# eladb3/SViT

Measured on AMD Instinct MI355X. Metric: clips/sec (fwd+bwd) SViT 16x224^2 bf16, higher is better.
Workload: dtype bf16; 1 GPU; SViT 16x224^2, 8 clips/GPU, 4 object tokens/frame, fwd+CE+bwd+clip+AdamW; global_batch=8, parallelism=dp1, ranks_seen=1, forced_dp=False, launch=hip-graph replay, input=fp32 clips, resident in the replayed step's input buffers, hip_library=svit_amd/lib/libsvit_hip.so

## Files before the change

### include/svit_hip.h

```cpp
#ifndef SVIT_HIP_H
#define SVIT_HIP_H
#include <stdint.h>
#ifdef __cplusplus
extern "C" {
#endif

#define SVIT_HEAD_DIM 96

int svit_version(void);
const char* svit_arch(void);

enum {
  SVIT_EPI_BF16 = 0,
  SVIT_EPI_GELU = 1,
  SVIT_EPI_RESID = 2,
  SVIT_EPI_F32 = 3,
  SVIT_EPI_DGELU = 4,
  SVIT_EPI_RELQ = 5
};
typedef struct {
  const void* A; int32_t lda;
  const void* W; int32_t ldw;
  const float* bias;
  void* out; int32_t ldo;
  void* out2; int32_t ldo2;
  const void* aux; int32_t ldaux;
  const float* row_scale; int32_t rows_per_sample;
  int32_t M, N, K;
  int32_t epilogue; int32_t accumulate;
  int32_t remap_L, remap_N, remap_off;
  const int32_t* relq_map;
  void* relq_out; int32_t relq_ld;
  int32_t relq_extra, relq_rows;
  float relq_scale;
} svit_gemm_args;
int svit_gemm_nt(const svit_gemm_args* args, void* stream);
int svit_gemm_tn(const void* A, int lda, const void* B, int ldb, float* dW, int lddw,
                 int M, int N, int K, int splits, float* dbias ,
                 void* stream);
#define SVIT_TN_GROUP_MAX 16
typedef struct {
  const void* A; const void* B; float* dW; float* dbias;
  int32_t lda, ldb, lddw, M, N, K;
} svit_tn_problem;
int svit_gemm_tn_grouped(const svit_tn_problem* probs, int count, void* stream);
int svit_gemm_tn_grouped_ex(const svit_tn_problem* probs, int count, int ordered, void* stream);
int svit_gemm_tn_grouped_slab(const svit_tn_problem* probs, int count, float* workspace,
                              int64_t workspace_floats, void* stream);
int64_t svit_gemm_tn_grouped_workspace(const svit_tn_problem* probs, int count);
int svit_gemm_tn_grouped_slab_lead(const svit_tn_problem* probs, int count, int launch_count, float* workspace,
                                   int64_t workspace_floats, void* stream);
int svit_colsum_bf16(const void* A, int lda, float* out, int M, int N, void* stream);

int svit_cast_f32_bf16(const float* src, void* dst, int64_t n, void* stream);
int svit_table_interp(const float* M, int rows, int J, const float* tables, float* out32, void* out16, void* stream);
typedef struct svit_table_interp_job {
  const float* M;
  const float* tables;
  float* out32;
  void* out16;
  int32_t rows, J;
} svit_table_interp_job;
int svit_table_interp_batched(const svit_table_interp_job* jobs_dev, int n_jobs, int max_rows, void* stream);
int svit_transpose_cast_batched(const float* src_base, void* dst_base, const int64_t* table,
                                int n_mats, int max_tiles, void* stream);
int svit_transpose_bf16_batched(const void* src_base, void* dst_base, const int64_t* table,
                                int n_mats, int max_tiles, void* stream);
int svit_pad_cast_rows(const float* src, void* dst, int R, int C, int ldd, void* stream);
int svit_scale_cast(const float* src, void* dst, const float* row_scale, int rows_per_sample,
                    int64_t rows, int cols, int gather_L, int gather_N, int gather_off,
                    void* stream);

int svit_reduce_defer(int on, void* stream);
int svit_reduce_flush(void* stream);
int svit_reduce_reset(void* stream);

int svit_layernorm_fwd(const float* x, const float* gamma, const float* beta, void* y_bf16,
                       float* y_f32, float* mean, float* rstd, int64_t rows, int C, float eps,
                       void* stream);
int svit_layernorm_bwd(const void* dy , int dy_is_bf16,
                       const float* x, const float* gamma, const float* mean,
                       const float* rstd, const float* dres, float* dx, void* dx_bf16,
                       const float* row_scale, int rows_per_sample, float* dgamma,
                       float* dbeta, int64_t rows, int C, float* workspace,
                       int64_t workspace_floats, void* stream);

int svit_im2col_patch(const float* video, void* cols, int B, int T, int H, int W, void* stream);
int svit_im2col_patch_u8(const uint8_t* frames, int64_t frames_bytes, const void* lut,
                         const int32_t* crops, void* cols, int B, int T, int Hs, int Ws, int S,
                         void* stream);
int svit_mixup_clips(float* x, const void* mix, int B, int planes, int H, int W, void* stream);
int svit_im2col_patch_u8_mix(const uint8_t* frames, int64_t frames_bytes, const float* lut_f32,
                             const int32_t* crops, const void* mix, void* cols, int B, int T, int Hs,
                             int Ws, int S, void* stream);
int svit_im2col_patch_u8_aug(const uint8_t* frames, int64_t frames_bytes, const float* lut_f32, const void* aug,
                             const void* mix, void* cols, int B, int T, int Hs, int Ws, int S, void* stream);
int svit_im2col_patch_u8_aug_frames(const uint8_t* frames, int64_t frames_bytes, const float* lut_f32, const void* aug,
                                    const void* mix, void* cols, int B, int T, int Hs, int Ws, int S, void* stream);
int svit_u8_clips_render(const uint8_t* frames, int64_t frames_bytes, const float* lut_f32, const void* aug,
                         float* out_f32, int B, int T, int Hs, int Ws, int S, void* stream);
int svit_im2col_patch_u8_aug_ext(const uint8_t* frames, int64_t frames_bytes, const float* lut_f32, const void* aug,
                                 const int32_t* extents, const void* mix, void* cols, int B, int T, int Hs, int Ws, int S,
                                 void* stream);
int svit_im2col_patch_u8_aug_frames_ext(const uint8_t* frames, int64_t frames_bytes, const float* lut_f32, const void* aug,
                                        const int32_t* extents, const void* mix, void* cols, int B, int T, int Hs, int Ws,
                                        int S, void* stream);
int svit_u8_clips_render_ext(const uint8_t* frames, int64_t frames_bytes, const float* lut_f32, const void* aug,
                             const int32_t* extents, float* out_f32, int B, int T, int Hs, int Ws, int S, void* stream);
typedef struct SvitRandAugOp {
  int32_t op, arg_i;
  float arg_f;
  uint32_t bicubic_mask;
  double m[6];
} SvitRandAugOp;
int svit_randaug_stats(const uint8_t* frames, const void* records, int layer, void* workspace, int V, int T, int Hs,
                       int Ws, int N, void* stream);
int svit_randaug_apply(const uint8_t* src, uint8_t* dst, const void* records, int layer, const void* workspace, int V,
                       int T, int Hs, int Ws, int N, void* stream);
int svit_randaug_stats_ext(const uint8_t* frames, const void* records, const int32_t* extents, int layer, void* workspace,
                           int V, int T, int Hs, int Ws, int N, void* stream);
int svit_randaug_apply_ext(const uint8_t* src, uint8_t* dst, const void* records, const int32_t* extents, int layer,
                           const void* workspace, int V, int T, int Hs, int Ws, int N, void* stream);
typedef struct { int64_t src_off; void* dst; int64_t bytes; } svit_feed_seg;
typedef struct {
  const uint8_t* slot; int64_t slot_bytes;
  const int64_t* offsets;
  const int32_t* extents;
  uint8_t* frames;
  int V, T, Hs, Ws, fill, swap_rb, n_seg;
  svit_feed_seg seg[8];
} svit_feed_args;
int svit_feed_unpack(const svit_feed_args* a, void* stream);
int svit_fill_special_tokens(float* x, const float* cls, const float* objq, const float* pos_t,
                             int B, int N, int L, int Tx, int O, int C, int add_pos, void* stream);
int svit_special_token_grads(const float* dx, float* g_cls, float* g_obj, float* g_pos, int B, int N,
                             int L, int Tx, int O, int C, int add_pos, void* stream);

typedef struct {
  const void* qkv; int32_t which;
  const float* conv_w;
  const float* gamma; const float* beta;
  void* out; int32_t ld_out;
  void* pre; float* mean; float* rstd;
  int32_t B, heads, T, H, W, n_obj;
  int32_t stride_hw;
  int32_t mode;
  float eps;
  float out_scale;
  const void* relq_R; const int32_t* relq_map; int32_t relq_lpad; float relq_scale;
} svit_pool_args;
int svit_pool_ln_fwd(const svit_pool_args* a, void* stream);

typedef struct {
  const void* d_main; int32_t main_is_f32; int32_t ld_main;
  const void* d_res; const void* d_extra;
  const void* pre; const float* mean; const float* rstd; const float* gamma;
  void* dpre; float* dgamma; float* dbeta;
  int32_t B, heads, Nout;
  float* workspace; int64_t workspace_floats;
  int32_t main_parts; int64_t main_part_stride;
  int32_t extra_is_bf16;
} svit_pool_ln_bwd_args;
int svit_pool_ln_bwd(const svit_pool_ln_bwd_args* a, void* stream);
typedef struct {
  const void* dpre; const float* conv_w; void* dqkv; int32_t which;
  int32_t B, heads, T, H, W, n_obj, stride_hw;
} svit_pool_dgrad_args;
typedef struct {
  const void* dpre; const void* qkv; int32_t which; float* dw;
  int32_t B, heads, T, H, W, n_obj, stride_hw;
  float* workspace; int64_t workspace_floats;
} svit_pool_wgrad_args;
int svit_pool_ln_fwd_qkv(const svit_pool_args* args3, void* stream);
int svit_pool_weight_sel(const float* src_base, const int64_t* src_off, uint32_t* dst, int n_tables,
                         void* stream);
int svit_pool_ln_fwd_qkv_sel(const svit_pool_args* args3, const uint32_t* const* sel3, void* stream);
int svit_pool_ln_bwd_qkv(const svit_pool_ln_bwd_args* args3, void* stream);
#ifdef SVIT_DIAG_POOL_STREAMING
int svit_pool_conv_dgrad(const svit_pool_dgrad_args* a, void* stream);
int svit_pool_conv_wgrad(const svit_pool_wgrad_args* a, void* stream);
int svit_pool_conv_dgrad_qkv(const svit_pool_dgrad_args* args3, void* stream);
int svit_pool_conv_wgrad_qkv(const svit_pool_wgrad_args* args3, void* stream);
#endif
int svit_pool_conv_bwd_qkv(const svit_pool_dgrad_args* dgrad3, const svit_pool_wgrad_args* wgrad3,
                           void* stream);
int64_t svit_pool_conv_bwd_workspace(const svit_pool_dgrad_args* dgrad3);

typedef struct {
  void* qa; int32_t ld;
  const float* rel_h; const float* rel_w; const float* rel_t;
  const int32_t* idx_h; const int32_t* idx_w; const int32_t* idx_t;
  int32_t B, heads, qt, qh, qw, kt, kh, kw, n_obj;
  float inv_scale;
} svit_relq_args;
int svit_relpos_q_fwd(const svit_relq_args* a, void* stream);
typedef struct {
  const void* qa; const void* dqa; int32_t ld;
  const float* rel_h; const float* rel_w; const float* rel_t;
  const int32_t* idx_h; const int32_t* idx_w; const int32_t* idx_t;
  float* dq_extra;
  float* drel_h; float* drel_w; float* drel_t;
  int32_t rows_h, rows_w, rows_t;
  int32_t B, heads, qt, qh, qw, kt, kh, kw, n_obj;
  float inv_scale;
  float* workspace; int64_t workspace_floats;
} svit_relq_bwd_args;
int svit_relpos_q_bwd(const svit_relq_bwd_args* a, void* stream);
typedef struct {
  const void* P; int32_t ldp; void* qa; int32_t ld;
  const int32_t* idx_h; const int32_t* idx_w; const int32_t* idx_t;
  int32_t row_h, row_w, row_t;
  int32_t B, heads, qt, qh, qw, kt, kh, kw, n_obj;
  float inv_scale;
} svit_relq_gather_args;
int svit_relpos_gather(const svit_relq_gather_args* a, void* stream);
typedef struct {
  const void* dqa; int32_t ld; void* D; int32_t ldd;
  const int32_t* idx_h; const int32_t* idx_w; const int32_t* idx_t;
  int32_t off_h, off_w, off_t;
  int32_t B, heads, qt, qh, qw, kt, kh, kw, n_obj;
  float inv_scale;
} svit_relq_scatter_args;
int svit_relpos_scatter(const svit_relq_scatter_args* a, void* stream);

typedef struct {
  const void* qa; const void* ka; const void* v; void* ctx; float* lse2;
  int32_t B, heads, Nq, Nk, DA; float scale; int32_t bias_cols;
} svit_attn_fwd_args;
int svit_attn_fwd(const svit_attn_fwd_args* a, void* stream);
typedef struct {
  const void* qa; const void* ka; const void* v; const void* ctx; const void* dctx;
  const float* lse2; float* delta;
  void* dqa;
  float* dk; float* dv;
  int32_t B, heads, Nq, Nk, DA, q_splits; float scale;
  int32_t bias_cols;
  void* relD; int32_t relD_ld; const int32_t* relD_map; float relD_scale;
  const void* relR; float* relX;
} svit_attn_bwd_args;
int svit_attn_bwd(const svit_attn_bwd_args* a, void* stream);
int svit_attn_bwd_parts(const svit_attn_bwd_args* a);

int svit_maxpool_fwd(const float* x, float* y, uint8_t* idx, int B, int T, int H, int W,
                     int n_obj, int C, void* stream);
int svit_maxpool_bwd(const float* dy, const uint8_t* idx, float* dx, int B, int T, int H, int W,
                     int n_obj, int C, void* stream);
int svit_maxpool_bwd_bf16(const float* dy, const uint8_t* idx, void* dx_bf16, int B, int T, int H, int W,
                          int n_obj, int C, void* stream);

int svit_sumsq(const float* g, int64_t n, float* sumsq, float* workspace,
               int64_t workspace_floats, void* stream);
int svit_adamw_step(float* p, const float* g, float* m, float* v, int64_t n, const float* sumsq,
                    float max_norm, float lr, float beta1, float beta2, float eps, float wd,
                    int step, float grad_scale, void* stream);

typedef struct {
  float lr[2], weight_decay[2];
  float max_norm, clip_value, grad_scale, reserved;
} svit_step_host;
typedef struct {
  int64_t applied, skipped;
  int32_t consecutive, apply;
  float coef, bc1, bc2_sqrt, sumsq, grad_norm, reserved;
} svit_step_dev;

int svit_tensor_stats_window(void);
int svit_tensor_table_check(const int64_t* table, int64_t Tn, int64_t n);
int64_t svit_tensor_stats_workspace(int64_t n, int64_t Tn);
int svit_tensor_stats(const float* g, const float* p, int64_t n, const int64_t* table_dev, const int64_t* table_host,
                      int64_t Tn, const int64_t* segs, int64_t S, const svit_step_dev* dev_rec, void* ring, int64_t R,
                      int64_t every, void* workspace, int64_t workspace_bytes, void* stream);

#define SVIT_ACT_MAX_SITES 96
#define SVIT_ACT_HEADER_BYTES 48
typedef struct {
  const float* a;
  const float* b;
  int32_t rows, first_window;
} svit_act_site;
int svit_act_stats_window(void);
int64_t svit_act_stats_workspace(int64_t total_windows);
int svit_act_sites_check(const svit_act_site* sites, const int32_t* slots, int64_t n_sites, int64_t n_slots,
                         int64_t* total_windows);
int svit_act_stats(const svit_act_site* sites, const int32_t* slots, int64_t n_sites, int64_t n_slots,
                   const int32_t* geom, const svit_step_dev* dev_rec, void* ring, int64_t R, int64_t* state,
                   void* workspace, int64_t workspace_bytes, void* stream);

int svit_adamw_bias_table(float beta1, float beta2, float* table, int64_t capacity, int64_t* n_entries);

int svit_step_guard(const float* g, int64_t n, const svit_step_host* host_rec, svit_step_dev* dev_rec,
                    const float* bias_table, int64_t table_entries, float* workspace, int64_t workspace_floats,
                    void* stream);
int svit_adamw_step_guarded(float* p, const float* g, float* m, float* v, int64_t n, int64_t n_decay,
                            const svit_step_host* host_rec, const svit_step_dev* dev_rec, float beta1, float beta2,
                            float eps, void* stream);

#define SVIT_MAX_SEGS 64
int svit_step_guard_seg(const float* g, int64_t n, const int64_t* segs, int64_t S, const svit_step_host* host_rec,
                        svit_step_dev* dev_rec, const float* bias_table, int64_t table_entries, float* workspace,
                        int64_t workspace_floats, void* stream);
int svit_adamw_step_guarded_seg(float* p, const float* g, float* m, float* v, int64_t n, int64_t n_decay,
                                const int64_t* segs, int64_t S, const svit_step_host* host_rec,
                                const svit_step_dev* dev_rec, float beta1, float beta2, float eps, void* stream);

int svit_adamw_step_guarded_lr(float* p, const float* g, float* m, float* v, int64_t n, int64_t n_decay,
                               const int64_t* segs, const float* scales, int64_t S, const svit_step_host* host_rec,
                               const svit_step_dev* dev_rec, float beta1, float beta2, float eps, void* stream);

int svit_sgd_step_guarded(float* p, const float* g, float* buf, int64_t n, int64_t n_decay, const int64_t* segs,
                          const float* scales, int64_t S, const svit_step_host* host_rec, const svit_step_dev* dev_rec,
                          float momentum, float dampening, int nesterov, void* stream);
int svit_adam_step_guarded(float* p, const float* g, float* m, float* v, int64_t n, int64_t n_decay,
                           const int64_t* segs, const float* scales, int64_t S, const svit_step_host* host_rec,
                           const svit_step_dev* dev_rec, float beta1, float beta2, float eps, void* stream);

int svit_ema_decay_table(float decay, float* table, int64_t capacity, int64_t* n_entries);
int svit_ema_step_guarded(float* ema, const float* p, int64_t n, const int64_t* segs, int64_t S,
                          const float* decay_table, int64_t table_entries, float decay, const int64_t* ema_rec,
                          const svit_step_dev* dev_rec, void* stream);

typedef struct {
  const float* tokens; int32_t B, N, C, T, O;
  const float* keep;
  const float* w_proj; const float* b_proj; int32_t n_cls;
  const float* w_box; const float* b_box;
  const float* w_bce; const float* b_bce;
  const float* w_con; const float* b_con;
  float* logits; float* boxes; float* contact; float* xobj;
} svit_head_args;
int svit_head_fwd(const svit_head_args* a, void* stream);
typedef struct {
  svit_head_args f;
  const float* dlogits; const float* dboxes; const float* dcontact; const float* dxobj;
  float* dtokens;
  float* gw_proj; float* gb_proj; float* gw_box; float* gb_box; float* gw_bce; float* gb_bce; float* gw_con; float* gb_con;
  int32_t ordered;
} svit_head_bwd_args;
int svit_head_bwd(const svit_head_bwd_args* g, void* stream);
int svit_head_eval(const svit_head_args* a, int act, void* stream);

int svit_haog_loss(const float* pred, const float* tar, const float* contact,
                   const int64_t* contact_tar, float* losses, float* g_l1, float* g_bce,
                   float* g_giou, float* g_contact, int R, int Rc, void* stream);
int svit_haog_loss_bwd(const float* upstream, const float* g_l1, const float* g_bce,
                       const float* g_giou, const float* g_contact, float* dpred,
                       float* dcontact, int R, int Rc, void* stream);

int svit_ce_loss(const float* logits, const int64_t* labels, int B, int C, float* loss, float* dlogits, void* stream);
int svit_ce_loss_soft(const float* logits, const float* target, const int64_t* labels, const void* mix, float on,
                      float off, int B, int C, float* loss, float* dlogits, void* stream);
int svit_step_draws(uint64_t* state, const float* keep, int n_blocks, int per_block, float* scales,
                    int n_drop, float p_drop, float* drop, void* stream);

int svit_ensemble_update(const float* preds, const int64_t* labels, const int64_t* clip_ids,
                         int N, int C, int num_clips, int num_videos, int mode, int repeat,
                         float* video_preds, int64_t* video_labels, int64_t* clip_count,
                         int* err, void* stream);
int svit_topk_correct(const float* video_preds, const int64_t* video_labels, int V, int C,
                      const int* ks, int nk, int* counts, int* err, void* stream);
#define SVIT_METER_MAX_SCALARS 16
int svit_meter_push(float* ring, int W, int K, int64_t* state, const float* const* scalars, int n_scalars,
                    const float* logits, const int64_t* labels, int N, int C, int k0, int k1, void* stream);
int svit_debug_set(int key, int val);
int svit_debug_gemm_nt_plan(int M, int N, int K, int epilogue, int32_t* out, int n_out);
int svit_debug_set_tn(int step_us_x100, int atomic_tbs_x100);
int svit_debug_set_tn_tile(int mode);
int svit_debug_gemm_tn_plan(const svit_tn_problem* probs, int count, int form, int arg, int64_t* out, int n_out);
int svit_debug_set_pool(int key, int val);
int svit_debug_pool_bwd_path(void);
int svit_debug_pool_plan(int kind, int B, int heads, int T, int H, int W, int n_obj, int sq, int sk, int sv, int save_mask,
                         int sel, int relq_lpad, int32_t* out, int n_out);
int svit_attn_debug_set(int key, int val);
int svit_debug_reset(void);
#ifdef __cplusplus
}
#endif
#endif
```

### svit_amd/csrc/common.h

```cpp
#pragma once
#include <hip/hip_runtime.h>
#include <stdint.h>

typedef uint16_t bf16_t;
typedef __bf16 bf16x8_t __attribute__((ext_vector_type(8)));
typedef __bf16 bf16x4_t __attribute__((ext_vector_type(4)));
typedef short s16x4_t __attribute__((ext_vector_type(4)));
typedef short s16x8_t __attribute__((ext_vector_type(8)));
typedef float f32x16_t __attribute__((ext_vector_type(16)));
typedef float f32x4_t __attribute__((ext_vector_type(4)));

#define SVIT_OK 0
#define SVIT_ERR_SHAPE (-2)
#define SVIT_ERR_ALIGN (-3)
#define SVIT_ERR_ARG (-4)

struct SvitOnce {
  unsigned long long mask;
};
static inline int svit_max_lds_once(SvitOnce& once, const void* fn, size_t bytes) {
  int dev = 0;
  if (hipGetDevice(&dev) != hipSuccess) dev = 0;
  const unsigned long long bit = 1ull << (dev & 63);
  if (__atomic_load_n(&once.mask, __ATOMIC_ACQUIRE) & bit) return 0;
  hipError_t e = hipFuncSetAttribute(fn, hipFuncAttributeMaxDynamicSharedMemorySize, (int)bytes);
  if (e != hipSuccess) return (int)e;
  __atomic_fetch_or(&once.mask, bit, __ATOMIC_RELEASE);
  return 0;
}

enum SvitKnob {
  SVIT_K_NT_STAGES = 0,
  SVIT_K_NT_CFG,
  SVIT_K_NT_BK,
  SVIT_K_TN_STEP_US_X100,
  SVIT_K_TN_ATOMIC_TBS_X100,
  SVIT_K_TN_TILE,
  SVIT_K_POOL_FWD,
  SVIT_K_POOL_BWD,
  SVIT_K_POOL_FWD_LARGE,
  SVIT_K_ATTN_DKV_FORM,
  SVIT_K_ATTN_FWD_SHORT,
  SVIT_K_POOL_FRAME,
  SVIT_K_COUNT
};
int svit_knob(int k);
int svit_knob_set(int k, int v);
void svit_knob_reset();

#define SVIT_LAUNCH_CHECK()                       \
  do {                                            \
    hipError_t e__ = hipGetLastError();           \
    if (e__ != hipSuccess) return (int)e__;       \
  } while (0)

__device__ __forceinline__ float bf16_to_f32(bf16_t v) {
  return __uint_as_float(((uint32_t)v) << 16);
}
__device__ __forceinline__ bf16_t f32_to_bf16(float f) {
  __bf16 b = (__bf16)f;
  return __builtin_bit_cast(bf16_t, b);
}
__device__ __forceinline__ uint32_t pack_bf16x2(float lo, float hi) {
  return (uint32_t)f32_to_bf16(lo) | ((uint32_t)f32_to_bf16(hi) << 16);
}
__device__ __forceinline__ float lo_bf16(uint32_t w) { return __uint_as_float(w << 16); }
__device__ __forceinline__ float hi_bf16(uint32_t w) { return __uint_as_float(w & 0xffff0000u); }

__device__ __forceinline__ float wave_sum(float v) {
#pragma unroll
  for (int o = 32; o > 0; o >>= 1) v += __shfl_xor(v, o, 64);
  return v;
}
__device__ __forceinline__ float wave_max(float v) {
#pragma unroll
  for (int o = 32; o > 0; o >>= 1) v = fmaxf(v, __shfl_xor(v, o, 64));
  return v;
}

__device__ __forceinline__ float fast_exp2(float x) { return __builtin_amdgcn_exp2f(x); }

__device__ __forceinline__ f32x16_t mfma32(bf16x8_t a, bf16x8_t b, f32x16_t c) {
  return __builtin_amdgcn_mfma_f32_32x32x16_bf16(a, b, c, 0, 0, 0);
}
__device__ __forceinline__ int acc_row(int r, int lane) {
  return (r & 3) + 8 * (r >> 2) + 4 * (lane >> 5);
}

typedef __attribute__((address_space(3))) s16x4_t lds_s16x4_t;
__device__ __forceinline__ s16x4_t lds_read_tr16(const void* p) {
  return __builtin_amdgcn_ds_read_tr16_b64_v4i16(
      (lds_s16x4_t*)(__attribute__((address_space(3))) void*)p);
}

__device__ __forceinline__ bf16x8_t make_bf16x8(s16x4_t lo, s16x4_t hi) {
  s16x8_t v = {lo[0], lo[1], lo[2], lo[3], hi[0], hi[1], hi[2], hi[3]};
  return __builtin_bit_cast(bf16x8_t, v);
}

__device__ __forceinline__ void gelu_parts(float x, float* cdf, float* pdf_scaled) {
  const float ax = fabsf(x) * 0.70710678118654752f;
  const float e = __expf(-ax * ax);
  const float t = __builtin_amdgcn_rcpf(1.0f + 0.3275911f * ax);
  const float poly = t * (0.254829592f + t * (-0.284496736f + t * (1.421413741f +
                     t * (-1.453152027f + t * 1.061405429f))));
  const float erf_abs = 1.0f - poly * e;
  const float erfv = x < 0.f ? -erf_abs : erf_abs;
  *cdf = 0.5f * (1.0f + erfv);
  *pdf_scaled = 0.39894228040143268f * e;
}
__device__ __forceinline__ float gelu_erf(float x) {
  float cdf, pdf;
  gelu_parts(x, &cdf, &pdf);
  return x * cdf;
}
__device__ __forceinline__ void gelu_fwd_grad(float x, float* y, float* dydx) {
#ifdef SVIT_DIAG_GELU_FREE
  *y = 0.5f * x; *dydx = 0.5f;
  return;
#endif
  float cdf, pdf;
  gelu_parts(x, &cdf, &pdf);
  *y = x * cdf;
  *dydx = cdf + x * pdf;
}
__device__ __forceinline__ float gelu_erf_grad(float x) {
  float cdf, pdf;
  gelu_parts(x, &cdf, &pdf);
  return cdf + x * pdf;
}

__device__ __forceinline__ void philox_round(uint32_t (&c)[4], uint32_t k0, uint32_t k1) {
  const uint64_t p0 = (uint64_t)0xD2511F53u * c[0], p1 = (uint64_t)0xCD9E8D57u * c[2];
  const uint32_t n0 = (uint32_t)(p1 >> 32) ^ c[1] ^ k0, n2 = (uint32_t)(p0 >> 32) ^ c[3] ^ k1;
  c[1] = (uint32_t)p1; c[3] = (uint32_t)p0; c[0] = n0; c[2] = n2;
}
__device__ __forceinline__ void philox4(uint64_t seed, uint64_t draw, uint32_t idx, float (&u)[4]) {
  uint32_t c[4] = {idx, 0u, (uint32_t)draw, (uint32_t)(draw >> 32)};
  uint32_t k0 = (uint32_t)seed, k1 = (uint32_t)(seed >> 32);
#pragma unroll
  for (int r = 0; r < 10; ++r) {
    philox_round(c, k0, k1);
    k0 += 0x9E3779B9u; k1 += 0xBB67AE85u;
  }
#pragma unroll
  for (int i = 0; i < 4; ++i) u[i] = (float)(c[i] >> 8) * (1.0f / 16777216.0f);
}

struct SvitReduceDst {
  float* ptr[6];
  int end[6];
};
void svit_launch_reduce(const float* partial, int nblocks, int n, SvitReduceDst dst, hipStream_t st);

static __global__ void svit_zero_kernel(uint4* __restrict__ p, size_t n16) {
  const size_t stride = (size_t)gridDim.x * blockDim.x;
  for (size_t i = (size_t)blockIdx.x * blockDim.x + threadIdx.x; i < n16; i += stride)
    p[i] = make_uint4(0u, 0u, 0u, 0u);
}
static inline void svit_launch_zero(void* p, size_t bytes, hipStream_t st) {
  const size_t n16 = bytes / 16;
  size_t blocks = (n16 + 255) / 256;
  if (blocks > 2048) blocks = 2048;
  if (blocks == 0) return;
  hipLaunchKernelGGL(svit_zero_kernel, dim3((unsigned)blocks), dim3(256), 0, st, (uint4*)p, n16);
}
```

### svit_amd/csrc/gemm_tn.hip

```cpp
#include <algorithm>
#include <type_traits>
#include <vector>
#include "common.h"
#include "../../include/svit_hip.h"

namespace {

template <int B, int E, typename F>
__device__ __forceinline__ void tn_static_for(F&& f) {
  if constexpr (B < E) {
    f(std::integral_constant<int, B>{});
    tn_static_for<B + 1, E>(f);
  }
}

template <int RB_, int WN_, int WK_, int BM_, int NS_>
struct TnDma {
  static constexpr int RB = RB_, WN = WN_, WK = WK_, BM = BM_, NS = NS_;
  static constexpr int TN = 32 * RB * WN, TK = 96 * WK;
  static constexpr int ROWA = TN * 2, ROWB = TK * 2;
  static constexpr int A_BYTES = BM * ROWA, B_BYTES = BM * ROWB, STAGE = A_BYTES + B_BYTES;
  static constexpr int A_INSTR = A_BYTES / 1024, B_INSTR = B_BYTES / 1024;
  static constexpr int NW = WN * WK, NT = NW * 64;
  static constexpr int PER = (A_INSTR + B_INSTR) / NW;
  static_assert((A_INSTR + B_INSTR) % NW == 0, "every wave issues the same number of pieces");
  __host__ __device__ static constexpr int swz_a(int row) { return row & 3; }
  __host__ __device__ static constexpr int swz_b(int row) { return ROWB == 384 ? ((row >> 1) & 1) : (ROWB % 256 == 0 ? (row & 3) : 0); }
};
using TnSmallD = TnDma<1, 4, 1, 64, 2>;
#ifndef SVIT_TN_BIG_NS
#define SVIT_TN_BIG_NS 3
#endif
#ifndef SVIT_TN_BIG_BM
#define SVIT_TN_BIG_BM 32
#endif
using TnBigD = TnDma<2, 2, 2, SVIT_TN_BIG_BM, SVIT_TN_BIG_NS>;
constexpr int TN_DMA_LDS = 2 * TnSmallD::STAGE > SVIT_TN_BIG_NS * TnBigD::STAGE ? 2 * TnSmallD::STAGE : SVIT_TN_BIG_NS * TnBigD::STAGE;

template <int OFF>
__device__ __forceinline__ void tn_read_tr(s16x4_t& d, unsigned addr) {
  asm volatile("ds_read_b64_tr_b16 %0, %1 offset:%2" : "=&v"(d) : "v"(addr), "i"(OFF) : "memory");
}

template <class C, bool SLAB>
__device__ __forceinline__ void tn_tile_dma(unsigned char* lds, const bf16_t* __restrict__ A, int lda,
                                            const bf16_t* __restrict__ B, int ldb,
                                            float* __restrict__ dW, int lddw, int M, int N, int K, int n0,
                                            int k0, int m_begin, int m_end,
                                            float* __restrict__ dbias, bool bias_tile) {
#if __HIP_DEVICE_COMPILE__
  constexpr int RB = C::RB, BM = C::BM, NS = C::NS, PER = C::PER;
  const int tid = threadIdx.x, lane = tid & 63, wave = __builtin_amdgcn_readfirstlane(tid >> 6);
  const int wn = wave / C::WK, wk = wave % C::WK;
  if (m_begin >= m_end) return;
  constexpr int NW = C::NW, NT = C::NT;
  constexpr int PA = C::A_INSTR / NW;
  static_assert(C::A_INSTR % NW == 0 && C::B_INSTR % NW == 0, "pieces split evenly over the waves");
  unsigned voff[PER];
  const int na8 = (N - n0 + 7) / 8, nb8 = (K - k0 + 7) / 8;
  auto piece = [&](int i, bool a) { return wave + NW * (a ? i : i - PA); };
#pragma unroll
  for (int i = 0; i < PER; ++i) {
    const bool a = i < PA;
    const int o = piece(i, a) * 1024 + lane * 16;
    const int rowb = a ? C::ROWA : C::ROWB;
    const int row = o / rowb, inrow = o % rowb;
    const int pb = inrow >> 6, c16 = (inrow >> 4) & 3;
    const int lb = pb ^ (a ? C::swz_a(row) : C::swz_b(row));
    const int ch = min(lb * 4 + c16, (a ? na8 : nb8) - 1);
    voff[i] = (unsigned)(row * (a ? lda : ldb) + (a ? n0 : k0) + ch * 8) * 2u;
  }
  const auto ars = __builtin_amdgcn_make_buffer_rsrc((void*)A, 0, (int)std::min<size_t>((size_t)M * lda * 2, 0x7fffffffu), 0x00020000);
  const auto brs = __builtin_amdgcn_make_buffer_rsrc((void*)B, 0, (int)std::min<size_t>((size_t)M * ldb * 2, 0x7fffffffu), 0x00020000);
  const int nsteps = (m_end - m_begin + BM - 1) / BM;
  auto issue = [&](int s) {
    unsigned char* st = lds + (s % NS) * C::STAGE;
    const int m0 = m_begin + s * BM;
    const int valid = m_end - m0;
#pragma unroll
    for (int i = 0; i < PER; ++i) {
      const bool a = i < PA;
      unsigned vo = voff[i];
      if (valid < BM) {
        const int row = (piece(i, a) * 1024 + lane * 16) / (a ? C::ROWA : C::ROWB);
        vo -= (unsigned)(row - min(row, valid - 1)) * (a ? lda : ldb) * 2u;
      }
      unsigned char* dst = st + (a ? 0 : C::A_BYTES) + piece(i, a) * 1024;
      if (a)
        __builtin_amdgcn_raw_ptr_buffer_load_lds(ars, (__attribute__((address_space(3))) void*)dst, 16, vo,
                                                 (unsigned)m0 * lda * 2u, 0, 0);
      else
        __builtin_amdgcn_raw_ptr_buffer_load_lds(brs, (__attribute__((address_space(3))) void*)dst, 16, vo,
                                                 (unsigned)m0 * ldb * 2u, 0, 0);
    }
  };
#pragma unroll
  for (int s = 0; s < NS - 1; ++s)
    if (s < nsteps) issue(s);

  f32x16_t acc[RB][3];
#pragma unroll
  for (int i = 0; i < RB; ++i)
#pragma unroll
    for (int j = 0; j < 3; ++j)
#pragma unroll
      for (int r = 0; r < 16; ++r) acc[i][j][r] = 0.f;
  const bool do_bias = (dbias != nullptr) && bias_tile;
  float bsum[8] = {0.f, 0.f, 0.f, 0.f, 0.f, 0.f, 0.f, 0.f};

  const int hh = lane >> 5, cg = (lane >> 4) & 1, ii = lane & 15, q = ii >> 2, pp = ii & 3;
  const unsigned lds0 = (unsigned)(size_t)lds;
  unsigned a_addr[RB], b_addr[3];
#pragma unroll
  for (int i = 0; i < RB; ++i) {
    const int col = wn * 32 * RB + i * 32 + 16 * cg + 4 * pp;
    a_addr[i] = lds0 + (8 * hh + q) * C::ROWA + (((col >> 5) ^ C::swz_a(q)) << 6) + (col & 31) * 2;
  }
#pragma unroll
  for (int j = 0; j < 3; ++j) {
    const int col = wk * 96 + j * 32 + 16 * cg + 4 * pp;
    b_addr[j] = lds0 + C::A_BYTES + (8 * hh + q) * C::ROWB + (((col >> 5) ^ C::swz_b(q)) << 6) + (col & 31) * 2;
  }
  constexpr int KS = BM / 16;
  for (int s = 0; s < nsteps; ++s) {
    if (s + NS - 2 < nsteps - 0 && NS > 2 && s + 1 < nsteps) asm volatile("s_waitcnt vmcnt(%0)" ::"n"((NS - 2) * PER) : "memory");
    else asm volatile("s_waitcnt vmcnt(0)" ::: "memory");
    __builtin_amdgcn_s_barrier();
    if (s + NS - 1 < nsteps) issue(s + NS - 1);
    const unsigned so = (unsigned)((s % NS) * C::STAGE);
    if (m_begin + (s + 1) * BM > m_end) {
      const int valid = m_end - (m_begin + s * BM);
      for (int c = tid; c < (BM - valid) * (C::ROWA / 16); c += NT)
        *(uint4*)(lds + so + valid * C::ROWA + c * 16) = make_uint4(0, 0, 0, 0);
      __syncthreads();
    }
    if (do_bias) {
      constexpr int CPR = C::TN / 8, RP = NT / CPR;
#pragma unroll
      for (int r0 = 0; r0 < BM; r0 += RP) {
        const int row = r0 + tid / CPR, lc = tid % CPR;
        uint4 u;
        asm volatile("ds_read_b128 %0, %1\n\ts_waitcnt lgkmcnt(0)" : "=&v"(u)
                     : "v"(lds0 + so + row * C::ROWA + ((((lc >> 2) ^ C::swz_a(row))) << 6) + (lc & 3) * 16) : "memory");
        bsum[0] += lo_bf16(u.x); bsum[1] += hi_bf16(u.x);
        bsum[2] += lo_bf16(u.y); bsum[3] += hi_bf16(u.y);
        bsum[4] += lo_bf16(u.z); bsum[5] += hi_bf16(u.z);
        bsum[6] += lo_bf16(u.w); bsum[7] += hi_bf16(u.w);
      }
    }
    s16x4_t fl[2][RB + 3], fh[2][RB + 3];
    auto rd = [&](auto KS_, auto BUF_) {
      constexpr int ks = decltype(KS_)::value, buf = decltype(BUF_)::value;
#pragma unroll
      for (int i = 0; i < RB; ++i) {
        tn_read_tr<ks * 16 * C::ROWA>(fl[buf][i], a_addr[i] + so);
        tn_read_tr<(ks * 16 + 4) * C::ROWA>(fh[buf][i], a_addr[i] + so);
      }
#pragma unroll
      for (int j = 0; j < 3; ++j) {
        tn_read_tr<ks * 16 * C::ROWB>(fl[buf][RB + j], b_addr[j] + so);
        tn_read_tr<(ks * 16 + 4) * C::ROWB>(fh[buf][RB + j], b_addr[j] + so);
      }
    };
    rd(std::integral_constant<int, 0>{}, std::integral_constant<int, 0>{});
    tn_static_for<0, KS>([&](auto KS_) {
      constexpr int ks = decltype(KS_)::value, cur = ks & 1;
      if constexpr (ks + 1 < KS) {
        rd(std::integral_constant<int, ks + 1>{}, std::integral_constant<int, (cur ^ 1)>{});
        asm volatile("s_waitcnt lgkmcnt(%0)" ::"n"(2 * (RB + 3)) : "memory");
      } else {
        asm volatile("s_waitcnt lgkmcnt(0)" ::: "memory");
      }
#pragma unroll
      for (int f = 0; f < RB + 3; ++f) asm volatile("" : "+v"(fl[cur][f]), "+v"(fh[cur][f]));
#pragma unroll
      for (int j = 0; j < 3; ++j)
#pragma unroll
        for (int i = 0; i < RB; ++i)
          acc[i][j] = mfma32(make_bf16x8(fl[cur][i], fh[cur][i]), make_bf16x8(fl[cur][RB + j], fh[cur][RB + j]), acc[i][j]);
      __builtin_amdgcn_sched_barrier(0);
    });
  }
  if constexpr (SLAB) {
#pragma unroll
    for (int i = 0; i < RB; ++i)
#pragma unroll
      for (int j = 0; j < 3; ++j) {
        const int tcol = wk * 96 + j * 32 + (lane & 31);
        if (k0 + tcol >= K) continue;
#pragma unroll
        for (int r4 = 0; r4 < 4; ++r4) {
          const int trow = wn * 32 * RB + i * 32 + acc_row(4 * r4, lane);
          if (n0 + trow < N)
            *(float4*)(dW + ((size_t)(trow >> 2) * lddw + tcol) * 4) =
                make_float4(acc[i][j][4 * r4], acc[i][j][4 * r4 + 1], acc[i][j][4 * r4 + 2], acc[i][j][4 * r4 + 3]);
        }
      }
  } else {
#pragma unroll
  for (int i = 0; i < RB; ++i)
#pragma unroll
    for (int j = 0; j < 3; ++j) {
      const int col = k0 + wk * 96 + j * 32 + (lane & 31);
      if (col >= K) continue;
#pragma unroll
      for (int r = 0; r < 16; ++r) {
        const int row = n0 + wn * 32 * RB + i * 32 + acc_row(r, lane);
#ifdef SVIT_TN_FLUSH_PLAIN
        if (row < N) dW[(size_t)row * lddw + col] = acc[i][j][r];
#else
        if (row < N) atomicAdd(dW + (size_t)row * lddw + col, acc[i][j][r]);
#endif
      }
    }
  }
  if (do_bias) {
    constexpr int CPR = C::TN / 8, RP = NT / CPR;
    static_assert(BM % RP == 0, "whole passes over a stage");
    __syncthreads();
    float* red = (float*)lds;
#pragma unroll
    for (int e = 0; e < 8; ++e) red[(tid / CPR) * C::TN + (tid % CPR) * 8 + e] = bsum[e];
    __syncthreads();
    if (tid < C::TN && n0 + tid < N) {
      float sum = 0.f;
#pragma unroll
      for (int g = 0; g < RP; ++g) sum += red[g * C::TN + tid];
      if constexpr (SLAB) dbias[tid] = sum;
      else atomicAdd(dbias + n0 + tid, sum);
    }
  }
#endif
}


__global__ __launch_bounds__(256) void gemm_tn_kernel(const bf16_t* __restrict__ A, int lda,
                                                      const bf16_t* __restrict__ B, int ldb,
                                                      float* __restrict__ dW, int lddw, int M,
                                                      int N, int K, int rows_per_split,
                                                      float* __restrict__ dbias) {
  __shared__ __attribute__((aligned(16))) unsigned char lds[TN_DMA_LDS];
  const int m_begin = blockIdx.z * rows_per_split;
  tn_tile_dma<TnSmallD, false>(lds, A, lda, B, ldb, dW, lddw, M, N, K, blockIdx.x * TnSmallD::TN, blockIdx.y * TnSmallD::TK,
                               m_begin, min(M, m_begin + rows_per_split), dbias, blockIdx.y == 0);
}

struct TnGroup {
  svit_tn_problem p[SVIT_TN_GROUP_MAX];
  int first_block[SVIT_TN_GROUP_MAX + 1];
  int tiles_n[SVIT_TN_GROUP_MAX];
  int tiles[SVIT_TN_GROUP_MAX];
  int rows_per_split[SVIT_TN_GROUP_MAX];
  int big[SVIT_TN_GROUP_MAX];
  int count;
};

struct TnSlabs {
  long long tile_off[SVIT_TN_GROUP_MAX];
  long long bias_off[SVIT_TN_GROUP_MAX];
  int red_first[SVIT_TN_GROUP_MAX + 1];
  int w[SVIT_TN_GROUP_MAX];
};
constexpr int TN_RED_THREADS = 128;
static_assert(TnSmallD::TN == 128 && TnBigD::TN == 128, "slabs and bias partials are 128 rows");

template <bool SLAB>
__device__ __forceinline__ void tn_grouped_workgroup(unsigned char* lds, const TnGroup& g, const TnSlabs* sl, float* ws) {
  const int nwg = gridDim.x, lin = blockIdx.x;
  const int xq = nwg >> 3, xr = nwg & 7, xcd = lin & 7;
  int pi = 0;
  const int bid = (xcd < xr ? xcd * (xq + 1) : xr * (xq + 1) + (xcd - xr) * xq) + (lin >> 3);
#pragma unroll
  for (int i = 1; i < SVIT_TN_GROUP_MAX; ++i)
    if (i < g.count && bid >= g.first_block[i]) pi = i;
  const int local = bid - g.first_block[pi];
  const int tile = local % g.tiles[pi], split = local / g.tiles[pi];
  const svit_tn_problem& p = g.p[pi];
  const int tn = tile % g.tiles_n[pi], tk = tile / g.tiles_n[pi];
  const int m_begin = split * g.rows_per_split[pi];
  float *out, *bias;
  int ld;
  if constexpr (SLAB) {
    ld = sl->w[pi];
    out = ws + sl->tile_off[pi] + (long long)local * (128 * ld);
    bias = p.dbias ? ws + sl->bias_off[pi] + (long long)(split * g.tiles_n[pi] + tn) * 128 : nullptr;
  } else {
    out = p.dW, ld = p.lddw, bias = p.dbias;
  }
  if (g.big[pi])
    tn_tile_dma<TnBigD, SLAB>(lds, (const bf16_t*)p.A, p.lda, (const bf16_t*)p.B, p.ldb, out, ld, p.M, p.N, p.K,
                              tn * TnBigD::TN, tk * TnBigD::TK, m_begin, min(p.M, m_begin + g.rows_per_split[pi]),
                              bias, tk == 0);
  else
    tn_tile_dma<TnSmallD, SLAB>(lds, (const bf16_t*)p.A, p.lda, (const bf16_t*)p.B, p.ldb, out, ld, p.M, p.N, p.K,
                                tn * TnSmallD::TN, tk * TnSmallD::TK, m_begin, min(p.M, m_begin + g.rows_per_split[pi]),
                                bias, tk == 0);
}

#ifndef SVIT_TN_WPE
#define SVIT_TN_WPE 2
#endif
__global__ __launch_bounds__(256, SVIT_TN_WPE) void gemm_tn_grouped_kernel(const TnGroup g) {
  __shared__ __attribute__((aligned(16))) unsigned char lds[TN_DMA_LDS];
  tn_grouped_workgroup<false>(lds, g, nullptr, nullptr);
}

__global__ __launch_bounds__(256, SVIT_TN_WPE) void gemm_tn_grouped_slab_kernel(const TnGroup g, const TnSlabs sl,
                                                                               float* __restrict__ ws) {
  __shared__ __attribute__((aligned(16))) unsigned char lds[TN_DMA_LDS];
  tn_grouped_workgroup<true>(lds, g, &sl, ws);
}

__global__ __launch_bounds__(TN_RED_THREADS) void tn_slab_reduce_kernel(const TnGroup g, const TnSlabs sl,
                                                                        const float* __restrict__ ws) {
#pragma clang fp reassociate(off)
  int pi = 0;
  const int blk = blockIdx.x;
#pragma unroll
  for (int i = 1; i < SVIT_TN_GROUP_MAX; ++i)
    if (i < g.count && blk >= sl.red_first[i]) pi = i;
  const svit_tn_problem& p = g.p[pi];
  const int N = p.N, K = p.K, rg_n = (N + 3) >> 2;
  const int tiles = g.tiles[pi], tiles_n = g.tiles_n[pi];
  const int S = (g.first_block[pi + 1] - g.first_block[pi]) / tiles;
  const long long e = (long long)(blk - sl.red_first[pi]) * TN_RED_THREADS + threadIdx.x;
  const long long nmat = (long long)rg_n * K;
  const float* src;
  long long stride;
  if (e < nmat) {
    const int rg = (int)(e / K), col = (int)(e - (long long)rg * K);
    const int tk_w = g.big[pi] ? TnBigD::TK : TnSmallD::TK, w = sl.w[pi];
    const int tile = (col / tk_w) * tiles_n + rg / 32;
    stride = (long long)tiles * (128 * w);
    src = ws + sl.tile_off[pi] + (long long)tile * (128 * w) + ((long long)(rg % 32) * w + col % tk_w) * 4;
  } else if (p.dbias && e < nmat + rg_n) {
    const int n = (int)(e - nmat) * 4;
    stride = (long long)tiles_n * 128;
    src = ws + sl.bias_off[pi] + (long long)(n / 128) * 128 + n % 128;
  } else {
    return;
  }
  float a0 = 0.f, a1 = 0.f, a2 = 0.f, a3 = 0.f;
  int s = 0;
  for (; s + 8 <= S; s += 8) {
    float4 v[8];
#pragma unroll
    for (int u = 0; u < 8; ++u) v[u] = *(const float4*)(src + (s + u) * stride);
#pragma unroll
    for (int u = 0; u < 8; ++u) { a0 += v[u].x; a1 += v[u].y; a2 += v[u].z; a3 += v[u].w; }
  }
  for (; s < S; ++s) {
    const float4 v = *(const float4*)(src + s * stride);
    a0 += v.x; a1 += v.y; a2 += v.z; a3 += v.w;
  }
  if (e < nmat) {
    const int rg = (int)(e / K), col = (int)(e - (long long)rg * K), row = rg * 4;
    float* d = p.dW + (size_t)row * p.lddw + col;
    d[0] += a0;
    if (row + 1 < N) d[p.lddw] += a1;
    if (row + 2 < N) d[2 * (size_t)p.lddw] += a2;
    if (row + 3 < N) d[3 * (size_t)p.lddw] += a3;
  } else {
    const int n = (int)(e - nmat) * 4;
    float* d = p.dbias + n;
    d[0] += a0;
    if (n + 1 < N) d[1] += a1;
    if (n + 2 < N) d[2] += a2;
    if (n + 3 < N) d[3] += a3;
  }
}

__global__ void colsum_kernel(const bf16_t* __restrict__ A, int lda, float* __restrict__ out,
                              int M, int N, int rows_per_block) {
  const int col = (blockIdx.x * 64 + threadIdx.x) * 2;
  const int r0 = blockIdx.y * rows_per_block;
  const int r1 = min(M, r0 + rows_per_block);
  float s0 = 0.f, s1 = 0.f;
  if (col < N) {
    for (int r = r0 + threadIdx.y; r < r1; r += 4) {
      const uint32_t w = *(const uint32_t*)(A + (size_t)r * lda + col);
      s0 += lo_bf16(w);
      s1 += hi_bf16(w);
    }
  }
  __shared__ float red[4][64][2];
  red[threadIdx.y][threadIdx.x][0] = s0;
  red[threadIdx.y][threadIdx.x][1] = s1;
  __syncthreads();
  if (threadIdx.y == 0 && col < N) {
    for (int k = 1; k < 4; ++k) {
      s0 += red[k][threadIdx.x][0];
      s1 += red[k][threadIdx.x][1];
    }
    atomicAdd(out + col, s0);
    if (col + 1 < N) atomicAdd(out + col + 1, s1);
  }
}

}

struct TnTileDims { int tn, tk, bm; };
static constexpr TnTileDims tn_dims(int big) {
  return big ? TnTileDims{TnBigD::TN, TnBigD::TK, TnBigD::BM} : TnTileDims{TnSmallD::TN, TnSmallD::TK, TnSmallD::BM};
}
static constexpr int tn_ceil(long a, long b) { return (int)((a + b - 1) / b); }

static int tn_check(const svit_tn_problem& p) {
  if (!p.A || !p.B || !p.dW) return SVIT_ERR_ARG;
  if (p.M <= 0 || p.N <= 0 || p.K <= 0) return SVIT_ERR_SHAPE;
  if (p.lda % 8 != 0 || p.ldb % 8 != 0 || p.lda < p.N || p.ldb < p.K || p.lddw < p.K)
    return SVIT_ERR_ALIGN;
  if (((uintptr_t)p.A | (uintptr_t)p.B) & 15) return SVIT_ERR_ALIGN;
  return SVIT_OK;
}
static int tn_check_all(const svit_tn_problem* probs, int count) {
  if (!probs || count <= 0) return SVIT_ERR_ARG;
  for (int i = 0; i < count; ++i) {
    const int rc = tn_check(probs[i]);
    if (rc) return rc;
  }
  return SVIT_OK;
}

struct TnSingle { int tiles_n, tiles_k, splits, rows_per_split; };
static int tn_single_splits(int M, int N, int K) {
  constexpr TnTileDims t = tn_dims(0);
  const int tiles = tn_ceil(N, t.tn) * tn_ceil(K, t.tk);
  const double atom_us = (double)N * K * 4.0 / 0.75e6;
  double best = 1e30;
  int splits = 1;
  static const int cand[] = {1, 2, 3, 4, 6, 8, 12, 16, 24, 32, 48, 64, 96, 128, 192, 256, 384, 512};
  for (int ci = 0; ci < (int)(sizeof(cand) / sizeof(cand[0])); ++ci) {
    const int s = cand[ci];
    const long steps = ((M + s - 1) / s + t.bm - 1) / t.bm;
    if (steps < 2 && s > 1) break;
    const long rounds = ((long)tiles * s + 511) / 512;
    const double time = (double)rounds * steps * 0.85 + s * atom_us;
    if (time < best) { best = time; splits = s; }
  }
  return splits;
}
static TnSingle tn_single_plan(int M, int N, int K, int splits) {
  constexpr TnTileDims t = tn_dims(0);
  if (splits <= 0) splits = tn_single_splits(M, N, K);
  const int rows_per_split = tn_ceil(tn_ceil(M, splits), t.bm) * t.bm;
  return {tn_ceil(N, t.tn), tn_ceil(K, t.tk), tn_ceil(M, rows_per_split), rows_per_split};
}

extern "C" int svit_gemm_tn(const void* A, int lda, const void* B, int ldb, float* dW, int lddw,
                            int M, int N, int K, int splits, float* dbias, void* stream) {
  const svit_tn_problem p = {A, B, dW, dbias, lda, ldb, lddw, M, N, K};
  const int rc = tn_check(p);
  if (rc) return rc;
  const TnSingle s = tn_single_plan(M, N, K, splits);
  hipLaunchKernelGGL(gemm_tn_kernel, dim3(s.tiles_n, s.tiles_k, s.splits), dim3(256), 0, (hipStream_t)stream,
                     (const bf16_t*)A, lda, (const bf16_t*)B, ldb, dW, lddw, M, N, K, s.rows_per_split, dbias);
  SVIT_LAUNCH_CHECK();
  return SVIT_OK;
}


static int tn_tile_rule(const svit_tn_problem& p, int mode) {
  const bool whole = p.K % TnBigD::TK == 0 && p.N >= 128;
  return mode == 1 ? (whole && (p.M <= 4096 || (p.M >= 32768 && p.M < 131072))) : mode == 3 ? whole : (mode == 2);
}

static long tn_chunk_steps(const TnGroup& g, int ordered, double step_us, double atomic_tbs) {
  constexpr long slots = 512;
  long st[SVIT_TN_GROUP_MAX], max_steps = 1;
  for (int i = 0; i < g.count; ++i) {
    st[i] = tn_ceil(g.p[i].M, tn_dims(g.big[i]).bm);
    if (st[i] > max_steps) max_steps = st[i];
  }
  if (ordered) return max_steps;
  double best = 1e30;
  long best_steps = max_steps;
  for (long steps = 2; steps <= max_steps; steps += (steps < 32 ? 1 : steps / 16)) {
    long blocks = 0;
    double flush = 0.0;
    for (int i = 0; i < g.count; ++i) {
      const TnTileDims t = tn_dims(g.big[i]);
      const long nb = (long)g.tiles[i] * ((st[i] + steps - 1) / steps);
      blocks += nb;
      flush += (double)nb * ((double)t.tn * t.tk * 4.0);
    }
    const double time = (double)((blocks + slots - 1) / slots) * steps * step_us + flush / (atomic_tbs * 1e6);
    if (time < best) { best = time; best_steps = steps; }
  }
  return best_steps;
}

static int tn_plan(const svit_tn_problem* probs, int n, int ordered, TnGroup& g) {
  const int mode = svit_knob(SVIT_K_TN_TILE);
  g.count = n;
  for (int i = 0; i < n; ++i) {
    g.p[i] = probs[i];
    g.big[i] = tn_tile_rule(probs[i], mode);
    const TnTileDims t = tn_dims(g.big[i]);
    g.tiles_n[i] = tn_ceil(probs[i].N, t.tn);
    g.tiles[i] = g.tiles_n[i] * tn_ceil(probs[i].K, t.tk);
  }
  const long steps = tn_chunk_steps(g, ordered, svit_knob(SVIT_K_TN_STEP_US_X100) * 0.01,
                                    svit_knob(SVIT_K_TN_ATOMIC_TBS_X100) * 0.01);
  int total = 0;
  for (int i = 0; i < n; ++i) {
    g.rows_per_split[i] = (int)steps * tn_dims(g.big[i]).bm;
    g.first_block[i] = total;
    total += g.tiles[i] * tn_ceil(g.p[i].M, g.rows_per_split[i]);
  }
  for (int i = n; i <= SVIT_TN_GROUP_MAX; ++i) g.first_block[i] = total;
  return total;
}

static int64_t tn_slab_layout(const TnGroup& g, TnSlabs& sl) {
  long long off = 0;
  int red = 0;
  for (int i = 0; i < g.count; ++i) {
    const int tk = tn_dims(g.big[i]).tk, k32 = (g.p[i].K + 31) / 32 * 32;
    sl.w[i] = k32 < tk ? k32 : tk;
    sl.tile_off[i] = off;
    off += (long long)(g.first_block[i + 1] - g.first_block[i]) * (128 * sl.w[i]);
  }
  for (int i = 0; i < g.count; ++i) {
    sl.bias_off[i] = off;
    const int splits = (g.first_block[i + 1] - g.first_block[i]) / g.tiles[i];
    if (g.p[i].dbias) off += (long long)splits * g.tiles_n[i] * 128;
    const long long rg_n = (g.p[i].N + 3) / 4, thr = rg_n * g.p[i].K + (g.p[i].dbias ? rg_n : 0);
    sl.red_first[i] = red;
    red += (int)((thr + TN_RED_THREADS - 1) / TN_RED_THREADS);
  }
  for (int i = g.count; i < SVIT_TN_GROUP_MAX; ++i) sl.tile_off[i] = sl.bias_off[i] = 0, sl.w[i] = 0;
  for (int i = g.count; i <= SVIT_TN_GROUP_MAX; ++i) sl.red_first[i] = red;
  return off;
}

struct TnChunk {
  TnGroup g;
  TnSlabs sl;
  int grid;
  int64_t slab_floats;
};
static int tn_chunks(const svit_tn_problem* probs, int count, int ordered, bool slabs, std::vector<TnChunk>& chunks) {
  const int rc = tn_check_all(probs, count);
  if (rc) return rc;
  chunks.resize((count + SVIT_TN_GROUP_MAX - 1) / SVIT_TN_GROUP_MAX);
  for (size_t c = 0; c < chunks.size(); ++c) {
    const int base = (int)c * SVIT_TN_GROUP_MAX;
    chunks[c].grid = tn_plan(probs + base, std::min(count - base, SVIT_TN_GROUP_MAX), ordered, chunks[c].g);
    chunks[c].slab_floats = slabs ? tn_slab_layout(chunks[c].g, chunks[c].sl) : 0;
  }
  return SVIT_OK;
}
static int64_t tn_slab_need(const std::vector<TnChunk>& chunks) {
  int64_t need = 0;
  for (const TnChunk& c : chunks) need = std::max(need, c.slab_floats);
  return need;
}

extern "C" int svit_gemm_tn_grouped_ex(const svit_tn_problem* probs, int count, int ordered, void* stream) {
  std::vector<TnChunk> chunks;
  const int rc = tn_chunks(probs, count, ordered, false, chunks);
  if (rc) return rc;
  for (const TnChunk& c : chunks) {
    hipLaunchKernelGGL(gemm_tn_grouped_kernel, dim3(c.grid), dim3(256), 0, (hipStream_t)stream, c.g);
    SVIT_LAUNCH_CHECK();
  }
  return SVIT_OK;
}
extern "C" int svit_gemm_tn_grouped(const svit_tn_problem* probs, int count, void* stream) {
  return svit_gemm_tn_grouped_ex(probs, count, 0, stream);
}

extern "C" int64_t svit_gemm_tn_grouped_workspace(const svit_tn_problem* probs, int count) {
  std::vector<TnChunk> chunks;
  const int rc = tn_chunks(probs, count, 0, true, chunks);
  return rc ? rc : tn_slab_need(chunks);
}

extern "C" int svit_gemm_tn_grouped_slab(const svit_tn_problem* probs, int count, float* workspace,
                                         int64_t workspace_floats, void* stream) {
  std::vector<TnChunk> chunks;
  const int rc = tn_chunks(probs, count, 0, true, chunks);
  if (rc) return rc;
  if (!workspace || workspace_floats < tn_slab_need(chunks)) return SVIT_ERR_ARG;
  if ((uintptr_t)workspace & 15) return SVIT_ERR_ALIGN;
  for (const TnChunk& c : chunks) {
    hipLaunchKernelGGL(gemm_tn_grouped_slab_kernel, dim3(c.grid), dim3(256), 0, (hipStream_t)stream, c.g, c.sl, workspace);
    SVIT_LAUNCH_CHECK();
    hipLaunchKernelGGL(tn_slab_reduce_kernel, dim3(c.sl.red_first[SVIT_TN_GROUP_MAX]), dim3(TN_RED_THREADS), 0,
                       (hipStream_t)stream, c.g, c.sl, (const float*)workspace);
    SVIT_LAUNCH_CHECK();
  }
  return SVIT_OK;
}

extern "C" int svit_gemm_tn_grouped_slab_lead(const svit_tn_problem* probs, int count, int launch_count,
                                              float* workspace, int64_t workspace_floats, void* stream) {
  if (launch_count < 1 || launch_count > count) return SVIT_ERR_ARG;
  std::vector<TnChunk> chunks;
  const int rc = tn_chunks(probs, count, 0, true, chunks);
  if (rc) return rc;
  if (!workspace || workspace_floats < tn_slab_need(chunks)) return SVIT_ERR_ARG;
  if ((uintptr_t)workspace & 15) return SVIT_ERR_ALIGN;
  for (size_t i = 0; i < chunks.size(); ++i) {
    const TnChunk& c = chunks[i];
    const int lead = std::min(launch_count - (int)i * SVIT_TN_GROUP_MAX, c.g.count);
    if (lead <= 0) break;
    hipLaunchKernelGGL(gemm_tn_grouped_slab_kernel, dim3(c.g.first_block[lead]), dim3(256), 0, (hipStream_t)stream, c.g,
                       c.sl, workspace);
    SVIT_LAUNCH_CHECK();
    hipLaunchKernelGGL(tn_slab_reduce_kernel, dim3(c.sl.red_first[lead]), dim3(TN_RED_THREADS), 0, (hipStream_t)stream,
                       c.g, c.sl, (const float*)workspace);
    SVIT_LAUNCH_CHECK();
  }
  return SVIT_OK;
}

extern "C" int svit_debug_gemm_tn_plan(const svit_tn_problem* probs, int count, int form, int arg, int64_t* out,
                                       int n_out) {
  if (form < 0 || form > 3 || !out || (form == 3 && count != 1)) return SVIT_ERR_ARG;
  std::vector<TnChunk> chunks;
  const int rc = form == 3 ? tn_check_all(probs, count) : tn_chunks(probs, count, form == 1, form == 2, chunks);
  if (rc) return rc;
  const int groups = form == 3 ? 1 : (int)chunks.size(), n = 2 + 3 * groups + 10 * count;
  if (n_out < n) return SVIT_ERR_ARG;
  int64_t* o = out;
  *o++ = groups;
  *o++ = tn_slab_need(chunks);
  if (form == 3) {
    const TnSingle s = tn_single_plan(probs[0].M, probs[0].N, probs[0].K, arg);
    const int64_t v[13] = {1, (int64_t)s.tiles_n * s.tiles_k * s.splits, 0,
                           0, s.tiles_n, s.tiles_k, s.rows_per_split, s.splits, 0, 0, 0, 0, 0};
    o = std::copy(v, v + 13, o);
  }
  for (const TnChunk& c : chunks) {
    const TnGroup& g = c.g;
    const bool slab = form == 2;
    const int64_t head[3] = {g.count, c.grid, slab ? c.sl.red_first[SVIT_TN_GROUP_MAX] : 0};
    o = std::copy(head, head + 3, o);
    for (int i = 0; i < g.count; ++i) {
      const int64_t v[10] = {g.big[i], g.tiles_n[i], g.tiles[i] / g.tiles_n[i], g.rows_per_split[i],
                             (g.first_block[i + 1] - g.first_block[i]) / g.tiles[i], g.first_block[i],
                             slab ? c.sl.w[i] : 0, slab ? c.sl.tile_off[i] : 0, slab ? c.sl.bias_off[i] : 0,
                             slab ? c.sl.red_first[i] : 0};
      o = std::copy(v, v + 10, o);
    }
  }
  return (int)(o - out);
}

extern "C" int svit_colsum_bf16(const void* A, int lda, float* out, int M, int N, void* stream) {
  if (!A || !out || M <= 0 || N <= 0 || (N & 1) || (lda & 1)) return SVIT_ERR_ARG;
  const int col_groups = (N + 127) / 128;
  int row_chunks = 2048 / col_groups;
  if (row_chunks < 1) row_chunks = 1;
  int rows_per_block = (M + row_chunks - 1) / row_chunks;
  if (rows_per_block < 64) rows_per_block = 64;
  row_chunks = (M + rows_per_block - 1) / rows_per_block;
  hipLaunchKernelGGL(colsum_kernel, dim3(col_groups, row_chunks), dim3(64, 4), 0,
                     (hipStream_t)stream, (const bf16_t*)A, lda, out, M, N, rows_per_block);
  SVIT_LAUNCH_CHECK();
  return SVIT_OK;
}
```

### svit_amd/csrc/misc.hip

```cpp
#include <cstring>
#include <mutex>
#include <unordered_map>
#include "common.h"
#include "../../include/svit_hip.h"

namespace {

__global__ void cast_kernel(const float* __restrict__ src, bf16_t* __restrict__ dst, int64_t n) {
  const int64_t stride = (int64_t)gridDim.x * blockDim.x * 8;
  for (int64_t i = ((int64_t)blockIdx.x * blockDim.x + threadIdx.x) * 8; i < n; i += stride) {
    if (i + 8 <= n) {
      const float4 a = *(const float4*)(src + i), b = *(const float4*)(src + i + 4);
      uint4 o;
      o.x = pack_bf16x2(a.x, a.y); o.y = pack_bf16x2(a.z, a.w);
      o.z = pack_bf16x2(b.x, b.y); o.w = pack_bf16x2(b.z, b.w);
      *(uint4*)(dst + i) = o;
    } else {
      for (int64_t j = i; j < n; ++j) dst[j] = f32_to_bf16(src[j]);
    }
  }
}

__global__ void transpose_cast_kernel(const float* __restrict__ src_base,
                                      bf16_t* __restrict__ dst_base,
// ... 383 lines not shown
}
__global__ void sumsq_final_kernel(const float* __restrict__ partial, int nblocks,
                                   float* __restrict__ out) {
  float s = 0.f;
  for (int i = threadIdx.x; i < nblocks; i += 64) s += partial[i];
  s = wave_sum(s);
  if (threadIdx.x == 0) *out += s;
}

__global__ void adamw_kernel(float* __restrict__ p, const float* __restrict__ g,
                             float* __restrict__ m, float* __restrict__ v, int64_t n,
                             const float* __restrict__ sumsq, float max_norm, float lr, float b1,
                             float b2, float eps, float wd, float bc1, float bc2_sqrt,
                             float grad_scale) {
  float coef = grad_scale;
  if (sumsq && max_norm > 0.f) {
    const float total = sqrtf(*sumsq) * grad_scale;
    coef *= fminf(max_norm / (total + 1e-6f), 1.0f);
  }
  const int64_t stride = (int64_t)gridDim.x * blockDim.x;
  for (int64_t i = (int64_t)blockIdx.x * blockDim.x + threadIdx.x; i < n; i += stride) {
    const float gi = g[i] * coef;
    float w = p[i] * (1.f - lr * wd);
    const float mi = m[i] * b1 + gi * (1.f - b1);
    const float vi = v[i] * b2 + gi * gi * (1.f - b2);
    const float denom = sqrtf(vi) / bc2_sqrt + eps;
    w -= (lr / bc1) * (mi / denom);
    p[i] = w; m[i] = mi; v[i] = vi;
  }
}

__global__ void step_guard_final_kernel(const float* __restrict__ partial, int nblocks,
                                        const svit_step_host* __restrict__ h, svit_step_dev* __restrict__ d,
                                        const float2* __restrict__ table, int64_t entries) {
  float s = 0.f;
  for (int i = threadIdx.x; i < nblocks; i += 64) s += partial[i];
  s = wave_sum(s);
  if (threadIdx.x != 0) return;
  const float max_norm = h->max_norm, grad_scale = h->grad_scale;
  const float total = sqrtf(s) * grad_scale;
  if ((__float_as_uint(total) & 0x7f800000u) != 0x7f800000u) {
    const int64_t step = d->applied + 1;
    float coef = grad_scale;
    if (max_norm > 0.f && !(h->clip_value > 0.f))
      coef *= fminf(max_norm / __builtin_fmaf(sqrtf(s), grad_scale, 1e-6f), 1.0f);
    float2 bc = make_float2(1.f, 1.f);
    if (step >= 1 && step <= entries) bc = table[step - 1];
    d->applied = step;
    d->consecutive = 0;
    d->apply = 1;
    d->coef = coef;
    d->bc1 = bc.x;
    d->bc2_sqrt = bc.y;
    d->sumsq = s;
    d->grad_norm = total;
  } else {
    d->skipped += 1;
    d->consecutive += 1;
    d->apply = 0;
  }
}

template <bool CLAMP>
__device__ __forceinline__ void adamw_guarded_update(float& pw, float gr, float& mo, float& va, float coef, float cv,
                                                     float lr, float wd, float b1, float b2, float eps, float bc1,
                                                     float bc2_sqrt) {
  float gi = gr * coef;
  if (CLAMP) gi = fminf(fmaxf(gi, -cv), cv);
  float w = pw * (1.f - lr * wd);
  const float mi = mo * b1 + gi * (1.f - b1);
  const float vi = va * b2 + gi * gi * (1.f - b2);
  const float denom = sqrtf(vi) / bc2_sqrt + eps;
  w -= (lr / bc1) * (mi / denom);
  pw = w; mo = mi; va = vi;
}

template <bool CLAMP>
__device__ __forceinline__ void adamw_guarded_range(float* __restrict__ p, const float* __restrict__ g,
                                                    float* __restrict__ m, float* __restrict__ v, int64_t n,
                                                    int64_t n_decay, const svit_step_host* __restrict__ h, float coef,
                                                    float bc1, float bc2_sqrt, float b1, float b2, float eps) {
  const float cv = h->clip_value;
  const float lr0 = h->lr[0], lr1 = h->lr[1], wd0 = h->weight_decay[0], wd1 = h->weight_decay[1];
  const int64_t n4 = n >> 2;
  const int64_t stride = (int64_t)gridDim.x * blockDim.x;
  for (int64_t q = (int64_t)blockIdx.x * blockDim.x + threadIdx.x; q < n4; q += stride) {
    const int64_t i = q * 4;
    float4 P = ((const float4*)p)[q], M = ((const float4*)m)[q], V = ((const float4*)v)[q];
    const float4 G = ((const float4*)g)[q];
    const bool d0 = i < n_decay, d1 = i + 1 < n_decay, d2 = i + 2 < n_decay, d3 = i + 3 < n_decay;
    adamw_guarded_update<CLAMP>(P.x, G.x, M.x, V.x, coef, cv, d0 ? lr0 : lr1, d0 ? wd0 : wd1, b1, b2, eps, bc1, bc2_sqrt);
    adamw_guarded_update<CLAMP>(P.y, G.y, M.y, V.y, coef, cv, d1 ? lr0 : lr1, d1 ? wd0 : wd1, b1, b2, eps, bc1, bc2_sqrt);
    adamw_guarded_update<CLAMP>(P.z, G.z, M.z, V.z, coef, cv, d2 ? lr0 : lr1, d2 ? wd0 : wd1, b1, b2, eps, bc1, bc2_sqrt);
    adamw_guarded_update<CLAMP>(P.w, G.w, M.w, V.w, coef, cv, d3 ? lr0 : lr1, d3 ? wd0 : wd1, b1, b2, eps, bc1, bc2_sqrt);
    ((float4*)p)[q] = P; ((float4*)m)[q] = M; ((float4*)v)[q] = V;
  }
  const int64_t i = n4 * 4 + threadIdx.x;
  if (blockIdx.x == 0 && i < n) {
    const bool dec = i < n_decay;
    float pw = p[i], mo = m[i], va = v[i];
    adamw_guarded_update<CLAMP>(pw, g[i], mo, va, coef, cv, dec ? lr0 : lr1, dec ? wd0 : wd1, b1, b2, eps, bc1, bc2_sqrt);
    p[i] = pw; m[i] = mo; v[i] = va;
  }
}

__global__ __launch_bounds__(256) void adamw_guarded_kernel(float* __restrict__ p, const float* __restrict__ g,
                                                            float* __restrict__ m, float* __restrict__ v, int64_t n,
                                                            int64_t n_decay, const svit_step_host* __restrict__ h,
                                                            const svit_step_dev* __restrict__ d, float b1, float b2,
                                                            float eps) {
  if (d->apply == 0) return;
  const float coef = d->coef, bc1 = d->bc1, bc2_sqrt = d->bc2_sqrt;
  if (h->clip_value > 0.f) adamw_guarded_range<true>(p, g, m, v, n, n_decay, h, coef, bc1, bc2_sqrt, b1, b2, eps);
  else adamw_guarded_range<false>(p, g, m, v, n, n_decay, h, coef, bc1, bc2_sqrt, b1, b2, eps);
}

struct SegTable {
  int64_t v[SVIT_MAX_SEGS][2];
  int32_t S;
};
__device__ __forceinline__ bool seg_inside(const SegTable& t, int& k, int64_t lo, int64_t hi, int64_t i) {
  while (k < t.S && t.v[k][1] <= lo) ++k;
  bool in = false;
  for (int j = k; j < t.S && t.v[j][0] < hi; ++j) in |= (i >= t.v[j][0]) & (i < t.v[j][1]);
  return in;
}

__global__ void sumsq_seg_kernel(const float* __restrict__ g, int64_t n, float* __restrict__ partial, const SegTable t) {
  float s = 0.f;
  const int64_t window = (int64_t)blockDim.x * 4, stride = (int64_t)gridDim.x * window;
  int k = 0;
  for (int64_t lo = (int64_t)blockIdx.x * window; lo < n; lo += stride) {
    const int64_t i = lo + (int64_t)threadIdx.x * 4;
    if (seg_inside(t, k, lo, lo + window, i)) {
      const float4 v = *(const float4*)(g + i);
      s += v.x * v.x + v.y * v.y + v.z * v.z + v.w * v.w;
    }
  }
  s = wave_sum(s);
  __shared__ float red[4];
  if ((threadIdx.x & 63) == 0) red[threadIdx.x >> 6] = s;
  __syncthreads();
  if (threadIdx.x == 0) partial[blockIdx.x] = (red[0] + red[1]) + (red[2] + red[3]);
}

template <bool CLAMP>
__device__ __forceinline__ void adamw_guarded_seg_range(float* __restrict__ p, const float* __restrict__ g,
                                                        float* __restrict__ m, float* __restrict__ v, int64_t n,
                                                        int64_t n_decay, const svit_step_host* __restrict__ h,
                                                        float coef, float bc1, float bc2_sqrt, float b1, float b2,
                                                        float eps, const SegTable& t) {
  const float cv = h->clip_value;
  const float lr0 = h->lr[0], lr1 = h->lr[1], wd0 = h->weight_decay[0], wd1 = h->weight_decay[1];
  const int64_t window = (int64_t)blockDim.x * 4, stride = (int64_t)gridDim.x * window;
  int k = 0;
  for (int64_t lo = (int64_t)blockIdx.x * window; lo < n; lo += stride) {
    const int64_t i = lo + (int64_t)threadIdx.x * 4;
    if (!seg_inside(t, k, lo, lo + window, i)) continue;
    const int64_t q = i >> 2;
    float4 P = ((const float4*)p)[q], M = ((const float4*)m)[q], V = ((const float4*)v)[q];
    const float4 G = ((const float4*)g)[q];
    const bool d0 = i < n_decay, d1 = i + 1 < n_decay, d2 = i + 2 < n_decay, d3 = i + 3 < n_decay;
    adamw_guarded_update<CLAMP>(P.x, G.x, M.x, V.x, coef, cv, d0 ? lr0 : lr1, d0 ? wd0 : wd1, b1, b2, eps, bc1, bc2_sqrt);
    adamw_guarded_update<CLAMP>(P.y, G.y, M.y, V.y, coef, cv, d1 ? lr0 : lr1, d1 ? wd0 : wd1, b1, b2, eps, bc1, bc2_sqrt);
    adamw_guarded_update<CLAMP>(P.z, G.z, M.z, V.z, coef, cv, d2 ? lr0 : lr1, d2 ? wd0 : wd1, b1, b2, eps, bc1, bc2_sqrt);
    adamw_guarded_update<CLAMP>(P.w, G.w, M.w, V.w, coef, cv, d3 ? lr0 : lr1, d3 ? wd0 : wd1, b1, b2, eps, bc1, bc2_sqrt);
    ((float4*)p)[q] = P; ((float4*)m)[q] = M; ((float4*)v)[q] = V;
  }
}

__global__ __launch_bounds__(256) void adamw_guarded_seg_kernel(float* __restrict__ p, const float* __restrict__ g,
                                                                float* __restrict__ m, float* __restrict__ v, int64_t n,
                                                                int64_t n_decay, const svit_step_host* __restrict__ h,
                                                                const svit_step_dev* __restrict__ d, float b1, float b2,
                                                                float eps, const SegTable t) {
  if (d->apply == 0) return;
  const float coef = d->coef, bc1 = d->bc1, bc2_sqrt = d->bc2_sqrt;
  if (h->clip_value > 0.f) adamw_guarded_seg_range<true>(p, g, m, v, n, n_decay, h, coef, bc1, bc2_sqrt, b1, b2, eps, t);
  else adamw_guarded_seg_range<false>(p, g, m, v, n, n_decay, h, coef, bc1, bc2_sqrt, b1, b2, eps, t);
}

struct LrTable {
  SegTable t;
  float scale[SVIT_MAX_SEGS];
};
__device__ __forceinline__ float lr_times_scale(float lr, float scale) {
  return __uint_as_float(__builtin_amdgcn_readfirstlane(__float_as_uint(lr * scale)));
}

template <bool CLAMP>
__device__ __forceinline__ void adamw_guarded_lr_range(float* __restrict__ p, const float* __restrict__ g,
                                                       float* __restrict__ m, float* __restrict__ v, int64_t n,
                                                       int64_t n_decay, const svit_step_host* __restrict__ h,
                                                       float coef, float bc1, float bc2_sqrt, float b1, float b2,
                                                       float eps, const LrTable& T) {
  const SegTable& t = T.t;
  const float cv = h->clip_value;
  const float lr0 = h->lr[0], lr1 = h->lr[1], wd0 = h->weight_decay[0], wd1 = h->weight_decay[1];
  const int64_t window = (int64_t)blockDim.x * 4, stride = (int64_t)gridDim.x * window;
  int k = 0;
  for (int64_t lo = (int64_t)blockIdx.x * window; lo < n; lo += stride) {
    const int64_t i = lo + (int64_t)threadIdx.x * 4, hi = lo + window;
    while (k < t.S && t.v[k][1] <= lo) ++k;
    bool in = false;
    float lr = 0.f, wd = 0.f;
    for (int j = k; j < t.S && t.v[j][0] < hi; ++j) {
      const bool dec = t.v[j][0] < n_decay;
      const float le = lr_times_scale(dec ? lr0 : lr1, T.scale[j]);
      const bool here = (i >= t.v[j][0]) & (i < t.v[j][1]);
      in |= here;
      lr = here ? le : lr;
      wd = here ? (dec ? wd0 : wd1) : wd;
    }
    if (!in) continue;
    const int64_t q = i >> 2;
    float4 P = ((const float4*)p)[q], M = ((const float4*)m)[q], V = ((const float4*)v)[q];
    const float4 G = ((const float4*)g)[q];
    adamw_guarded_update<CLAMP>(P.x, G.x, M.x, V.x, coef, cv, lr, wd, b1, b2, eps, bc1, bc2_sqrt);
    adamw_guarded_update<CLAMP>(P.y, G.y, M.y, V.y, coef, cv, lr, wd, b1, b2, eps, bc1, bc2_sqrt);
    adamw_guarded_update<CLAMP>(P.z, G.z, M.z, V.z, coef, cv, lr, wd, b1, b2, eps, bc1, bc2_sqrt);
    adamw_guarded_update<CLAMP>(P.w, G.w, M.w, V.w, coef, cv, lr, wd, b1, b2, eps, bc1, bc2_sqrt);
    ((float4*)p)[q] = P; ((float4*)m)[q] = M; ((float4*)v)[q] = V;
  }
}

__global__ __launch_bounds__(256) void adamw_guarded_lr_kernel(float* __restrict__ p, const float* __restrict__ g,
                                                               float* __restrict__ m, float* __restrict__ v, int64_t n,
                                                               int64_t n_decay, const svit_step_host* __restrict__ h,
                                                               const svit_step_dev* __restrict__ d, float b1, float b2,
                                                               float eps, const LrTable T) {
  if (d->apply == 0) return;
  const float coef = d->coef, bc1 = d->bc1, bc2_sqrt = d->bc2_sqrt;
  if (h->clip_value > 0.f) adamw_guarded_lr_range<true>(p, g, m, v, n, n_decay, h, coef, bc1, bc2_sqrt, b1, b2, eps, T);
  else adamw_guarded_lr_range<false>(p, g, m, v, n, n_decay, h, coef, bc1, bc2_sqrt, b1, b2, eps, T);
}

static int seg_table_take(const int64_t* segs, int64_t S, int64_t n, int64_t n_decay, SegTable* out) {
  if (!segs || S < 1 || S > SVIT_MAX_SEGS) return SVIT_ERR_ARG;
  int64_t prev = 0;
  for (int64_t s = 0; s < S; ++s) {
    const int64_t b = segs[2 * s], e = segs[2 * s + 1];
    if (b < prev || e <= b || e > n) return SVIT_ERR_ARG;
    if (n_decay >= 0 && b < n_decay && e > n_decay) return SVIT_ERR_ARG;
    prev = e;
  }
  for (int64_t s = 0; s < 2 * S; ++s)
    if (segs[s] & 3) return SVIT_ERR_ALIGN;
  for (int64_t s = 0; s < SVIT_MAX_SEGS; ++s) {
    out->v[s][0] = s < S ? segs[2 * s] : 0;
    out->v[s][1] = s < S ? segs[2 * s + 1] : 0;
  }
  out->S = (int32_t)S;
  return SVIT_OK;
}

inline unsigned grid_for(int64_t work_items, int block, unsigned cap = 8192) {
  int64_t b = (work_items + block - 1) / block;
  if (b < 1) b = 1;
  if (b > cap) b = cap;
  return (unsigned)b;
}
__global__ __launch_bounds__(128) void table_interp_kernel(const float* __restrict__ M, int J, const float* __restrict__ T,
                                                           float* __restrict__ out32, bf16_t* __restrict__ out16) {
  const int r = blockIdx.x, c = threadIdx.x;
  if (c >= 96) return;
  const float* m = M + (size_t)r * J;
  float acc = 0.f;
#pragma unroll 8
  for (int j = 0; j < J; ++j) acc += m[j] * T[(size_t)j * 96 + c];
  if (out32) out32[(size_t)r * 96 + c] = acc;
  if (out16) out16[(size_t)r * 96 + c] = f32_to_bf16(acc);
}
__global__ __launch_bounds__(128) void table_interp_batched_kernel(const svit_table_interp_job* __restrict__ jobs) {
  const svit_table_interp_job j = jobs[blockIdx.y];
  const int r = blockIdx.x, c = threadIdx.x;
  if (r >= j.rows || c >= 96) return;
  const float* m = j.M + (size_t)r * j.J;
  float acc = 0.f;
#pragma unroll 8
  for (int k = 0; k < j.J; ++k) acc += m[k] * j.tables[(size_t)k * 96 + c];
  if (j.out32) j.out32[(size_t)r * 96 + c] = acc;
  if (j.out16) ((bf16_t*)j.out16)[(size_t)r * 96 + c] = f32_to_bf16(acc);
}
}

extern "C" int svit_version(void) { return 1; }

extern "C" int svit_table_interp_batched(const svit_table_interp_job* jobs_dev, int n_jobs, int max_rows, void* stream) {
  if (!jobs_dev || n_jobs <= 0 || n_jobs > 65535 || max_rows <= 0) return SVIT_ERR_ARG;
  hipLaunchKernelGGL(table_interp_batched_kernel, dim3(max_rows, n_jobs), dim3(128), 0, (hipStream_t)stream, jobs_dev);
  SVIT_LAUNCH_CHECK();
  return SVIT_OK;
}

extern "C" int svit_table_interp(const float* M, int rows, int J, const float* tables, float* out32, void* out16, void* stream) {
  if (!M || !tables || (!out32 && !out16) || rows <= 0 || J <= 0) return SVIT_ERR_ARG;
  hipLaunchKernelGGL(table_interp_kernel, dim3(rows), dim3(128), 0, (hipStream_t)stream, M, J, tables, out32, (bf16_t*)out16);
  SVIT_LAUNCH_CHECK();
  return SVIT_OK;
}

static const int k_knob_default[SVIT_K_COUNT] = {
     0,  -1,  0,  85,  75,  2,
     2,  1,  1,  0,  1,  2};
static int g_knob[SVIT_K_COUNT] = {0, -1, 0, 85, 75, 2, 2, 1, 1, 0, 1, 2};
int svit_knob(int k) { return __atomic_load_n(&g_knob[k], __ATOMIC_RELAXED); }
int svit_knob_set(int k, int v) {
  if (k < 0 || k >= SVIT_K_COUNT) return SVIT_ERR_ARG;
  __atomic_store_n(&g_knob[k], v, __ATOMIC_RELAXED);
  return SVIT_OK;
}
void svit_knob_reset() {
  for (int k = 0; k < SVIT_K_COUNT; ++k) __atomic_store_n(&g_knob[k], k_knob_default[k], __ATOMIC_RELAXED);
}
extern "C" int svit_debug_set(int key, int val) {
  if (key == 0) return (val == 0 || (val >= 2 && val <= 4)) ? svit_knob_set(SVIT_K_NT_STAGES, val) : SVIT_ERR_ARG;
  if (key == 1) return (val >= -1 && val <= 10) ? svit_knob_set(SVIT_K_NT_CFG, val) : SVIT_ERR_ARG;
  if (key == 2) return (val == 0 || val == 32 || val == 64) ? svit_knob_set(SVIT_K_NT_BK, val) : SVIT_ERR_ARG;
  return SVIT_ERR_ARG;
}
extern "C" int svit_debug_set_tn(int step_us_x100, int atomic_tbs_x100) {
  if (step_us_x100 > 0) svit_knob_set(SVIT_K_TN_STEP_US_X100, step_us_x100);
  if (atomic_tbs_x100 > 0) svit_knob_set(SVIT_K_TN_ATOMIC_TBS_X100, atomic_tbs_x100);
  return SVIT_OK;
}
extern "C" int svit_debug_set_tn_tile(int mode) {
  return (mode >= 0 && mode <= 3) ? svit_knob_set(SVIT_K_TN_TILE, mode) : SVIT_ERR_ARG;
}
extern "C" int svit_debug_set_pool(int key, int val) {
  if (key == 0) return (val >= 0 && val <= 3) ? svit_knob_set(SVIT_K_POOL_FWD, val) : SVIT_ERR_ARG;
  if (key == 1) return (val == 0 || val == 1) ? svit_knob_set(SVIT_K_POOL_BWD, val) : SVIT_ERR_ARG;
  if (key == 2) return (val == 0 || val == 1) ? svit_knob_set(SVIT_K_POOL_FWD_LARGE, val) : SVIT_ERR_ARG;
  if (key == 3) return (val >= 0 && val <= 2) ? svit_knob_set(SVIT_K_POOL_FRAME, val) : SVIT_ERR_ARG;
  return SVIT_ERR_ARG;
}
extern "C" int svit_attn_debug_set(int key, int val) {
  if (key == 0) return (val >= 0 && val <= 2) ? svit_knob_set(SVIT_K_ATTN_DKV_FORM, val) : SVIT_ERR_ARG;
  if (key == 3) return (val == 0 || val == 1) ? svit_knob_set(SVIT_K_ATTN_FWD_SHORT, val) : SVIT_ERR_ARG;
  return SVIT_ERR_ARG;
}
extern "C" int svit_debug_reset(void) { svit_knob_reset(); return SVIT_OK; }
extern "C" const char* svit_arch(void) { return "gfx950"; }

extern "C" int svit_cast_f32_bf16(const float* src, void* dst, int64_t n, void* stream) {
  if (!src || !dst || n <= 0) return SVIT_ERR_ARG;
  if (((uintptr_t)src | (uintptr_t)dst) & 15) return SVIT_ERR_ALIGN;
  hipLaunchKernelGGL(cast_kernel, dim3(grid_for((n + 7) / 8, 256)), dim3(256), 0,
                     (hipStream_t)stream, src, (bf16_t*)dst, n);
  SVIT_LAUNCH_CHECK();
  return SVIT_OK;
}

extern "C" int svit_transpose_cast_batched(const float* src_base, void* dst_base,
                                           const int64_t* table, int n_mats, int max_tiles,
                                           void* stream) {
  if (!src_base || !dst_base || !table || n_mats <= 0) return SVIT_ERR_ARG;
  int gx = max_tiles < 1 ? 1 : (max_tiles > 256 ? 256 : max_tiles);
  hipLaunchKernelGGL(transpose_cast_kernel, dim3(gx, n_mats), dim3(256), 0, (hipStream_t)stream,
                     src_base, (bf16_t*)dst_base, table, n_mats);
  SVIT_LAUNCH_CHECK();
  return SVIT_OK;
}


extern "C" int svit_transpose_bf16_batched(const void* src_base, void* dst_base, const int64_t* table,
                                           int n_mats, int max_tiles, void* stream) {
  if (!src_base || !dst_base || !table || n_mats <= 0) return SVIT_ERR_ARG;
  if (((uintptr_t)src_base | (uintptr_t)dst_base) & 15) return SVIT_ERR_ALIGN;
  int gx = max_tiles < 1 ? 1 : (max_tiles > 256 ? 256 : max_tiles);
  hipLaunchKernelGGL(transpose_bf16_kernel, dim3(gx, n_mats), dim3(256), 0, (hipStream_t)stream,
                     (const bf16_t*)src_base, (bf16_t*)dst_base, table, n_mats);
  SVIT_LAUNCH_CHECK();
  return SVIT_OK;
}

extern "C" int svit_scale_cast(const float* src, void* dst, const float* row_scale,
                               int rows_per_sample, int64_t rows, int cols, int gather_L,
                               int gather_N, int gather_off, void* stream) {
  if (!src || !dst || rows <= 0 || cols <= 0 || cols % 4 != 0) return SVIT_ERR_ARG;
  if (row_scale && rows_per_sample <= 0) return SVIT_ERR_ARG;
  if (gather_L < 0 || (gather_L > 0 && (gather_N < gather_L || gather_off < 0))) return SVIT_ERR_ARG;
  hipLaunchKernelGGL(scale_cast_kernel, dim3(grid_for(rows * (cols / 4), 256)), dim3(256), 0,
                     (hipStream_t)stream, src, (bf16_t*)dst, row_scale, rows_per_sample, rows,
                     cols, gather_L, gather_N, gather_off);
  SVIT_LAUNCH_CHECK();
  return SVIT_OK;
}

extern "C" int svit_pad_cast_rows(const float* src, void* dst, int R, int C, int ldd, void* stream) {
  if (!src || !dst || R <= 0 || C <= 0 || ldd < C) return SVIT_ERR_ARG;
  hipLaunchKernelGGL(pad_cast_rows_kernel, dim3(grid_for((int64_t)R * ldd, 256)), dim3(256), 0,
                     (hipStream_t)stream, src, (bf16_t*)dst, R, C, ldd);
  SVIT_LAUNCH_CHECK();
  return SVIT_OK;
}

extern "C" int svit_im2col_patch(const float* video, void* cols, int B, int T, int H, int W,
                                 void* stream) {
  if (!video || !cols || B <= 0 || T <= 0 || H <= 0 || W <= 0) return SVIT_ERR_ARG;
  const int To = (T + 2 - 3) / 2 + 1, Ho = (H + 6 - 7) / 4 + 1, Wo = (W + 6 - 7) / 4 + 1;
  hipLaunchKernelGGL(im2col_patch_kernel, dim3((unsigned)(B * To * Ho)), dim3(256), 0,
                     (hipStream_t)stream, video, (bf16_t*)cols, B, T, H, W, To, Ho, Wo);
  SVIT_LAUNCH_CHECK();
  return SVIT_OK;
}

extern "C" int svit_fill_special_tokens(float* x, const float* cls, const float* objq,
                                        const float* pos_t, int B, int N, int L, int Tx, int O,
                                        int C, int add_pos, void* stream) {
  if (!x || !cls || !objq || (add_pos && !pos_t)) return SVIT_ERR_ARG;
  if (N != 1 + L + Tx * O) return SVIT_ERR_SHAPE;
  const int64_t total = (int64_t)B * (1 + Tx * O) * C;
  hipLaunchKernelGGL(fill_special_kernel, dim3(grid_for(total, 256)), dim3(256), 0,
                     (hipStream_t)stream, x, cls, objq, pos_t, B, N, L, Tx, O, C, add_pos);
  SVIT_LAUNCH_CHECK();
  return SVIT_OK;
}

extern "C" int svit_special_token_grads(const float* dx, float* g_cls, float* g_obj, float* g_pos, int B, int N,
                                        int L, int Tx, int O, int C, int add_pos, void* stream) {
  if (!dx || !g_cls || !g_obj || (add_pos && !g_pos)) return SVIT_ERR_ARG;
  if (N != 1 + L + Tx * O || B <= 0 || C <= 0) return SVIT_ERR_SHAPE;
  const int n_out = C + O * C + (add_pos ? Tx * C : 0);
  hipLaunchKernelGGL(special_grads_kernel, dim3((n_out * 8 + 255) / 256), dim3(256), 0, (hipStream_t)stream, dx, g_cls,
                     g_obj, g_pos, B, N, L, Tx, O, C, add_pos);
  SVIT_LAUNCH_CHECK();
  return SVIT_OK;
}

extern "C" int svit_maxpool_fwd(const float* x, float* y, uint8_t* idx, int B, int T, int H, int W,
                                int n_obj, int C, void* stream) {
  if (!x || !y || !idx || C % 4 != 0) return SVIT_ERR_ARG;
  const int Ho = (H - 1) / 2 + 1, Wo = (W - 1) / 2 + 1;
  const int64_t per = (int64_t)(1 + T * Ho * Wo + n_obj) * (C / 4);
  if (per >= (1ll << 31) || B > 65535) return SVIT_ERR_SHAPE;
  hipLaunchKernelGGL(maxpool_fwd_kernel, dim3(grid_for(per, 256, 2048), B), dim3(256), 0,
                     (hipStream_t)stream, x, y, idx, B, T, H, W, Ho, Wo, n_obj, C);
  SVIT_LAUNCH_CHECK();
  return SVIT_OK;
}

extern "C" int svit_maxpool_bwd(const float* dy, const uint8_t* idx, float* dx, int B, int T, int H,
                                int W, int n_obj, int C, void* stream) {
  if (!dy || !dx || !idx || C % 4 != 0) return SVIT_ERR_ARG;
  const int Ho = (H - 1) / 2 + 1, Wo = (W - 1) / 2 + 1;
  const int64_t per = (int64_t)(1 + T * H * W + n_obj) * (C / 4);
  if (per >= (1ll << 31) || B > 65535) return SVIT_ERR_SHAPE;
  hipLaunchKernelGGL(maxpool_bwd_kernel<false>, dim3(grid_for(per, 256, 2048), B), dim3(256), 0,
                     (hipStream_t)stream, dy, idx, (void*)dx, B, T, H, W, Ho, Wo, n_obj, C);
  SVIT_LAUNCH_CHECK();
  return SVIT_OK;
}
extern "C" int svit_maxpool_bwd_bf16(const float* dy, const uint8_t* idx, void* dx_bf16, int B, int T, int H,
                                     int W, int n_obj, int C, void* stream) {
  if (!dy || !dx_bf16 || !idx || C % 4 != 0) return SVIT_ERR_ARG;
  const int Ho = (H - 1) / 2 + 1, Wo = (W - 1) / 2 + 1;
  const int64_t per = (int64_t)(1 + T * H * W + n_obj) * (C / 4);
  if (per >= (1ll << 31) || B > 65535) return SVIT_ERR_SHAPE;
  hipLaunchKernelGGL(maxpool_bwd_kernel<true>, dim3(grid_for(per, 256, 2048), B), dim3(256), 0,
                     (hipStream_t)stream, dy, idx, dx_bf16, B, T, H, W, Ho, Wo, n_obj, C);
  SVIT_LAUNCH_CHECK();
  return SVIT_OK;
}

struct ReduceQueue {
  SvitReduceBatch batch;
  bool defer = false;
  ReduceQueue() { batch.count = 0; }
};
static std::mutex g_reduce_mu;
static std::unordered_map<hipStream_t, ReduceQueue> g_reduce_q;

static void reduce_launch(const SvitReduceBatch& b, hipStream_t st) {
  int max_n = 0;
  for (int i = 0; i < b.count; ++i)
    if (b.job[i].n > max_n) max_n = b.job[i].n;
  hipLaunchKernelGGL(svit_reduce_partials_kernel, dim3((max_n + 31) / 32, b.count), dim3(32, 32),
                     0, st, b);
}

void svit_launch_reduce(const float* partial, int nblocks, int n, SvitReduceDst dst, hipStream_t st) {
  SvitReduceJob job = {partial, nblocks, n, dst};
  SvitReduceBatch run;
  run.count = 0;
  {
    std::lock_guard<std::mutex> lk(g_reduce_mu);
    auto it = g_reduce_q.find(st);
    if (it != g_reduce_q.end() && it->second.defer) {
      ReduceQueue& q = it->second;
      if (q.batch.count == SVIT_REDUCE_MAX_JOBS) {
        run = q.batch;
        q.batch.count = 0;
      }
      q.batch.job[q.batch.count++] = job;
      job.partial = nullptr;
    }
  }
  if (run.count) reduce_launch(run, st);
  if (job.partial) {
    SvitReduceBatch one;
    one.job[0] = job;
    one.count = 1;
    reduce_launch(one, st);
  }
}

static void reduce_take(hipStream_t st, int set_defer , bool drop, SvitReduceBatch* out) {
  out->count = 0;
  std::lock_guard<std::mutex> lk(g_reduce_mu);
  auto it = g_reduce_q.find(st);
  if (it == g_reduce_q.end()) {
    if (set_defer != 1) return;
    it = g_reduce_q.emplace(st, ReduceQueue()).first;
  }
  ReduceQueue& q = it->second;
  if (!drop) *out = q.batch;
  q.batch.count = 0;
  if (set_defer >= 0) q.defer = set_defer != 0;
  if (!q.defer) g_reduce_q.erase(it);
}

extern "C" int svit_reduce_defer(int on, void* stream) {
  SvitReduceBatch run;
  reduce_take((hipStream_t)stream, on ? 1 : 0, on != 0, &run);
  if (run.count) reduce_launch(run, (hipStream_t)stream);
  SVIT_LAUNCH_CHECK();
  return SVIT_OK;
}

extern "C" int svit_reduce_flush(void* stream) {
  SvitReduceBatch run;
  reduce_take((hipStream_t)stream, -1, false, &run);
  if (run.count) reduce_launch(run, (hipStream_t)stream);
  SVIT_LAUNCH_CHECK();
  return SVIT_OK;
}

extern "C" int svit_reduce_reset(void* stream) {
  SvitReduceBatch run;
  reduce_take((hipStream_t)stream, 0, true, &run);
  return SVIT_OK;
}

extern "C" int svit_sumsq(const float* g, int64_t n, float* sumsq, float* workspace,
                          int64_t workspace_floats, void* stream) {
  if (!g || !sumsq || !workspace || n <= 0) return SVIT_ERR_ARG;
  unsigned blocks = grid_for((n + 3) / 4, 256, 1024);
  if ((int64_t)blocks > workspace_floats) blocks = (unsigned)workspace_floats;
  if (blocks < 1) return SVIT_ERR_ARG;
  hipLaunchKernelGGL(sumsq_kernel, dim3(blocks), dim3(256), 0, (hipStream_t)stream, g, n, workspace);
  SVIT_LAUNCH_CHECK();
  hipLaunchKernelGGL(sumsq_final_kernel, dim3(1), dim3(64), 0, (hipStream_t)stream, workspace,
                     (int)blocks, sumsq);
  SVIT_LAUNCH_CHECK();
  return SVIT_OK;
}

static inline void adamw_bias_corrections(float beta1, float beta2, int step, float* bc1, float* bc2_sqrt) {
#pragma float_control(precise, on)
  *bc1 = 1.f - powf(beta1, (float)step);
  *bc2_sqrt = sqrtf(1.f - powf(beta2, (float)step));
}

extern "C" int svit_adamw_step(float* p, const float* g, float* m, float* v, int64_t n,
                               const float* sumsq, float max_norm, float lr, float beta1,
                               float beta2, float eps, float wd, int step, float grad_scale,
                               void* stream) {
  if (!p || !g || !m || !v || n <= 0 || step < 1) return SVIT_ERR_ARG;
  float bc1, bc2s;
  adamw_bias_corrections(beta1, beta2, step, &bc1, &bc2s);
  hipLaunchKernelGGL(adamw_kernel, dim3(grid_for(n, 256, 4096)), dim3(256), 0, (hipStream_t)stream,
                     p, g, m, v, n, sumsq, max_norm, lr, beta1, beta2, eps, wd, bc1, bc2s,
                     grad_scale);
  SVIT_LAUNCH_CHECK();
  return SVIT_OK;
}

extern "C" int svit_adamw_bias_table(float beta1, float beta2, float* table, int64_t capacity, int64_t* n_entries) {
  if (!n_entries || (table && capacity < 0)) return SVIT_ERR_ARG;
  constexpr int64_t kMax = 1ll << 20;
  for (int64_t k = 1; k <= kMax; ++k) {
    float bc1, bc2s;
    adamw_bias_corrections(beta1, beta2, (int)k, &bc1, &bc2s);
    if (table) {
      if (k > capacity) return SVIT_ERR_ARG;
      table[2 * (k - 1)] = bc1;
      table[2 * (k - 1) + 1] = bc2s;
    }
    if (bc1 == 1.0f && bc2s == 1.0f) {
      *n_entries = k;
      return SVIT_OK;
    }
  }
  return SVIT_ERR_ARG;
}

extern "C" int svit_step_guard(const float* g, int64_t n, const svit_step_host* host_rec, svit_step_dev* dev_rec,
                               const float* bias_table, int64_t table_entries, float* workspace,
                               int64_t workspace_floats, void* stream) {
  if (!g || !host_rec || !dev_rec || !workspace || n <= 0 || table_entries < 0 || (table_entries > 0 && !bias_table))
    return SVIT_ERR_ARG;
  if (((uintptr_t)host_rec | (uintptr_t)dev_rec | (uintptr_t)bias_table) & 7) return SVIT_ERR_ALIGN;
  unsigned blocks = grid_for((n + 3) / 4, 256, 1024);
  if ((int64_t)blocks > workspace_floats) blocks = (unsigned)workspace_floats;
  if (blocks < 1) return SVIT_ERR_ARG;
  hipLaunchKernelGGL(sumsq_kernel, dim3(blocks), dim3(256), 0, (hipStream_t)stream, g, n, workspace);
  SVIT_LAUNCH_CHECK();
  hipLaunchKernelGGL(step_guard_final_kernel, dim3(1), dim3(64), 0, (hipStream_t)stream, workspace, (int)blocks,
                     host_rec, dev_rec, (const float2*)bias_table, table_entries);
  SVIT_LAUNCH_CHECK();
  return SVIT_OK;
}

extern "C" int svit_adamw_step_guarded(float* p, const float* g, float* m, float* v, int64_t n, int64_t n_decay,
                                       const svit_step_host* host_rec, const svit_step_dev* dev_rec, float beta1,
                                       float beta2, float eps, void* stream) {
  if (!p || !g || !m || !v || !host_rec || !dev_rec || n <= 0 || n_decay < 0 || n_decay > n) return SVIT_ERR_ARG;
  if (((uintptr_t)p | (uintptr_t)g | (uintptr_t)m | (uintptr_t)v) & 15) return SVIT_ERR_ALIGN;
  if (((uintptr_t)host_rec | (uintptr_t)dev_rec) & 7) return SVIT_ERR_ALIGN;
  hipLaunchKernelGGL(adamw_guarded_kernel, dim3(grid_for(n >> 2, 256, 4096)), dim3(256), 0, (hipStream_t)stream,
                     p, g, m, v, n, n_decay, host_rec, dev_rec, beta1, beta2, eps);
  SVIT_LAUNCH_CHECK();
  return SVIT_OK;
}

extern "C" int svit_step_guard_seg(const float* g, int64_t n, const int64_t* segs, int64_t S,
                                   const svit_step_host* host_rec, svit_step_dev* dev_rec, const float* bias_table,
                                   int64_t table_entries, float* workspace, int64_t workspace_floats, void* stream) {
  if (!g || !host_rec || !dev_rec || !workspace || n <= 0 || table_entries < 0 || (table_entries > 0 && !bias_table))
    return SVIT_ERR_ARG;
// ... 54 lines not shown
```

### svit_amd/engine.py

```python
import math

import torch

from . import arch, hip, ops
from .augment import AugClips
from .input import FramesView, U8Clips

HD = arch.HEAD_DIM
F32, BF16 = torch.float32, torch.bfloat16
SCALE = HD ** -0.5
LOG2E = 1.4426950408889634
K_SCALE = SCALE * LOG2E


def _align(n, a=8):
    return (n + a - 1) // a * a


class FlatParams:

    @staticmethod
    def layout(shapes, decay_of, rank_of):
        names = list(shapes)
        depth = 1 + max([int(n.split(".")[1]) for n in names if n.startswith("blocks.")] or [0])
# ... 197 lines not shown
                q_thw = (cur[0], arch.pooled(cur[1], sq), arch.pooled(cur[2], sq))
                k_thw = (cur[0], arch.pooled(cur[1], skv), arch.pooled(cur[2], skv))
                _, _, mcat, _ = self._rel(blk, q_thw, k_thw)
                if mcat is not None:
                    r32 = torch.empty((mcat.shape[0], HD), device=self.dev, dtype=F32) if save else None
                    r16 = torch.empty((mcat.shape[0], HD), device=self.dev, dtype=BF16)
                    entries.append((mcat, self.flat.rel_tables32("blocks.%d." % blk.index), r32, r16))
                    outs[blk.index] = (r32, r16)
                cur = q_thw
            jobs = ops.table_interp_jobs(entries, self.dev) if entries else None
            ent = (jobs, max((e[0].shape[0] for e in entries), default=0), outs, entries)
            self._interp_cache[key] = ent
        jobs, max_rows, outs, _ = ent
        if jobs is not None:
            ops.table_interp_batched(jobs, max_rows)
        self._interp_out = outs

    def _relq_map(self, blk, q_thw, k_thw, idx, rows_off, n_obj, extra):
        key = (blk.index, q_thw, k_thw, tuple(rows_off), n_obj, extra)
        m = self._relq_cache.get(key)
        if m is None:
            qt, qh, qw = q_thw
            kt, kh, kw = k_thw
            ih, iw, it = (t.cpu().view(n, k) for t, n, k in zip(idx, (qh, qw, qt), (kh, kw, kt)))
            Lq = qt * qh * qw
            body = torch.full((qt, qh, qw, extra), -1, dtype=torch.int32)
            body[..., :kh] = (rows_off[0] + ih).view(1, qh, 1, kh)
            body[..., kh:kh + kw] = (rows_off[1] + iw).view(1, 1, qw, kw)
            body[..., kh + kw:kh + kw + kt] = (rows_off[2] + it).view(qt, 1, 1, kt)
            m = torch.full((1 + Lq + n_obj, extra), -1, dtype=torch.int32)
            m[1:1 + Lq] = body.view(Lq, extra)
            m = m.contiguous().to(self.dev)
            self._relq_cache[key] = m
        return m

    def _tables(self, pre, mats):
        names = (pre + "attn.rel_pos_h", pre + "attn.rel_pos_w", pre + "attn.rel_pos_t")
        out = []
        for n, m in zip(names, mats):
            t = self.flat.p(n)
            out.append(t if m is None else (m @ t).contiguous())
        return out

    def forward(self, video, drop_scales=None, save=True, cut=0):
        plan, f = self.plan, self.flat
        if isinstance(video, U8Clips):
            cols, (To, Ho, Wo) = ops.im2col_patch_u8(video)
        elif isinstance(video, AugClips):
            cols, (To, Ho, Wo) = ops.im2col_patch_u8_aug(video)
        elif isinstance(video, FramesView):
            cols, (To, Ho, Wo) = ops.im2col_patch_u8_aug_frames(video)
        else:
            if video.dim() == 4:
                video = video.unsqueeze(2)
            video = video.contiguous().to(F32)
            cols, (To, Ho, Wo) = ops.im2col_patch(video)
        B, _, Tx = video.shape[:3]
        T = plan.num_frames // plan.patch_stride[0] if Tx > 1 else Tx
        if To != T:
            raise hip.SvitHipError("clip has %d frames but cfg.DATA.NUM_FRAMES=%d" % (Tx, plan.num_frames))
        L, n_obj, C = To * Ho * Wo, Tx * plan.objects, plan.embed_dim
        N = 1 + L + n_obj
        x = torch.empty((B, N, C), device=self.dev, dtype=F32)
        ops.gemm_nt(cols, self.patch_w16, f.p("patch_embed.proj.bias"), hip.EPI_F32,
                    out=x.view(B * N, C), remap=(L, N, 1))
        ops.fill_special_tokens(x, f.p("cls_token"), f.p("object_queries"),
                                f.p("pos_embed_temporal"), L, Tx, plan.objects, Tx > 1)
        st = {"B": B, "Tx": Tx, "n_obj": n_obj, "L0": L, "cols": cols if save and cut == 0 else None,
              "blocks": [], "cut": cut}
        thw = (T, Ho, Wo)
        self._interp_tables(thw, save)
        hip.mark("stem")
        for blk in plan.blocks:
            ds = drop_scales[blk.index] if drop_scales is not None else None
            keep = save and 1 + blk.index >= cut
            shapes = (self._tn_shapes(blk, x.shape[0], x.shape[1], thw, n_obj)
                      if save and not keep and self.reproducible and not self.deterministic else None)
            x, thw, sv = self._block_fwd(blk, x, thw, n_obj, ds, keep)
            if shapes is not None:
                sv = {"tn_shapes": shapes}
            st["blocks"].append(sv)
            hip.mark("fwd%d" % blk.index)
        y16, y32, mean, rstd = ops.layernorm_fwd(x, f.p("norm.weight"), f.p("norm.bias"),
                                                 want_f32=True, want_bf16=False, save_stats=save)
        st.update(x_last=x if save else None, mean=mean, rstd=rstd, thw=thw, thw0=(T, Ho, Wo))
        if save and self.act_monitor is not None:
            self.act_monitor.enqueue(st)
        self._interp_out = {}
        return y32, st

    def _tn_shapes(self, blk, B, N, thw, n_obj):
        f = self.flat
        pre = "blocks.%d." % blk.index
        sq, skv = blk.stride_q[1], blk.stride_kv[1]
        q_thw = (thw[0], arch.pooled(thw[1], sq), arch.pooled(thw[2], sq))
        k_thw = (thw[0], arch.pooled(thw[1], skv), arch.pooled(thw[2], skv))
        Nq = 1 + q_thw[0] * q_thw[1] * q_thw[2] + n_obj
        hid, Co = f.slots[pre + "mlp.fc1.weight"][2]
        C = f.slots[pre + "attn.qkv.weight"][2][1]
        M, Mq = B * N, B * Nq
        out = [(Mq, Co, hid, True), (Mq, hid, Co, True), (Mq, Co, Co, True)]
        for a, m in zip("hwt", self._rel(blk, q_thw, k_thw)[1]):
            if m is None:
                out.append((B * blk.heads * Nq, f.slots[pre + "attn.rel_pos_" + a][2][0], HD, False))
        out.append((M, 3 * Co, C, True))
        if blk.has_proj:
            out.append((M, Co, C, True))
        return out

    def _block_fwd(self, blk, x, thw, n_obj, ds, save):
        f = self.flat
        pre = "blocks.%d." % blk.index
        B, N, C = x.shape
        Co, h = blk.dim_out, blk.heads
        sq, skv = blk.stride_q[1], blk.stride_kv[1]
        q_thw = (thw[0], arch.pooled(thw[1], sq), arch.pooled(thw[2], sq))
        k_thw = (thw[0], arch.pooled(thw[1], skv), arch.pooled(thw[2], skv))
        Nq = 1 + q_thw[0] * q_thw[1] * q_thw[2] + n_obj
        J = k_thw[0] + k_thw[1] + k_thw[2]
        DA = HD + 32 if J <= 32 else HD + 64
        if J > 64:
            raise hip.SvitHipError("key grid %s too large for the in-MFMA rel-pos bias" % (k_thw,))
        xn, _, mean1, rstd1 = ops.layernorm_fwd(x, f.p(pre + "norm1.weight"), f.p(pre + "norm1.bias"),
                                                save_stats=save)
        xn2d = xn.view(B * N, C)
        qkv = ops.gemm_nt(xn2d, f.w(pre + "attn.qkv.weight"), f.p(pre + "attn.qkv.bias"), hip.EPI_BF16)
        idx, mats, mcat, need = self._rel(blk, q_thw, k_thw)
        if mcat is None:
            tabs = self._tables(pre, mats)
            rcat, rows_off = f.rel_cat(pre)
        else:
            if blk.index in self._interp_out:
                r32, rcat = self._interp_out[blk.index]
            else:
                r32, rcat = ops.table_interp(mcat, f.rel_tables32(pre), want_f32=save)
            rows_off = (0, need[0], need[0] + need[1])
            tabs = None if r32 is None else [r32[rows_off[0]:rows_off[0] + need[0]], r32[rows_off[1]:rows_off[1] + need[1]],
                                             r32[rows_off[2]:rows_off[2] + need[2]]]
        pools = ops.pool_ln_fwd_qkv(
            qkv, [f.p(pre + "attn.pool_%s.weight" % r).view(HD, 27) for r in "qkv"],
            [f.p(pre + "attn.norm_%s.weight" % r) for r in "qkv"],
            [f.p(pre + "attn.norm_%s.bias" % r) for r in "qkv"],
            B, h, thw, n_obj, (sq, skv, skv), (DA, DA, HD), (0, 1, 0), save=save, out_scales=(1.0, K_SCALE, 1.0),
            sels=f.sels(pre) if (thw[1] * thw[2] >= f.TILED_MIN_PLANE or thw[1] * thw[2] <= f.SLAB_MAX_PLANE)
            else None,
            relq=(rcat.contiguous(), self._relq_map(blk, q_thw, k_thw, idx, rows_off, n_obj, DA - HD), LOG2E))
        qa, ka, v = pools[0][0], pools[1][0], pools[2][0]
        ctx, lse2 = ops.attn_fwd(qa, ka, v, SCALE, bias_cols=J)
        pool_idx = None
        if blk.has_proj:
            skip = ops.gemm_nt(xn2d, f.w(pre + "proj.weight"), f.p(pre + "proj.bias"), hip.EPI_F32)
            skip = skip.view(B, N, Co)
        else:
            skip = x
        if blk.pools_q:
            skip, pool_idx = ops.maxpool_fwd(skip, thw, n_obj)
        dpa, dpm = ds if ds is not None else (None, None)
        x1 = ops.gemm_nt(ctx.view(B * Nq, Co), f.w(pre + "attn.proj.weight"), f.p(pre + "attn.proj.bias"),
                         hip.EPI_RESID, aux=skip.view(B * Nq, Co), row_scale=dpa, rows_per_sample=Nq)
        x1 = x1.view(B, Nq, Co)
        xn2, _, mean2, rstd2 = ops.layernorm_fwd(x1, f.p(pre + "norm2.weight"), f.p(pre + "norm2.bias"),
                                                 save_stats=save)
        act, dact = ops.gemm_nt(xn2.view(B * Nq, Co), f.w(pre + "mlp.fc1.weight"),
                                f.p(pre + "mlp.fc1.bias"), hip.EPI_GELU, save=save)
        x2 = ops.gemm_nt(act, f.w(pre + "mlp.fc2.weight"), f.p(pre + "mlp.fc2.bias"), hip.EPI_RESID,
                         aux=x1.view(B * Nq, Co), row_scale=dpm, rows_per_sample=Nq).view(B, Nq, Co)
        sv = None
        if save:
            sv = dict(x=x, thw=thw, q_thw=q_thw, k_thw=k_thw, mean1=mean1, rstd1=rstd1, xn=xn2d,
                      qkv=qkv, pools=pools, tabs=tabs, idx=idx, mats=mats, ctx=ctx, lse2=lse2,
                      pool_idx=pool_idx, x1=x1, mean2=mean2, rstd2=rstd2, xn2=xn2, act=act,
                      dact=dact, dpa=dpa, dpm=dpm, Nq=Nq)
        return x2, q_thw, sv

    def backward(self, st, dy, on_ready=None, ready_ranks=None):
        def ready(rank):
            if on_ready is not None:
                if ready_ranks is None or rank in ready_ranks:
                    ops.reduce_flush()
                    self._flush_tn()
                    self._join()
                on_ready(rank)
        plan, f = self.plan, self.flat
        depth = len(plan.blocks)
        cut = st.get("cut", 0)
        lo = max(cut - 1, 0)
        if cut > depth:
            if cut == depth + 1:
                ops.layernorm_bwd(dy.contiguous(), st["x_last"], f.p("norm.weight"), st["mean"], st["rstd"],
                                  f.g("norm.weight"), f.g("norm.bias"), want_bf16=False,
                                  rows_per_sample=st["x_last"].shape[1])
            for rank in range(depth + 2):
                ready(rank)
            return
        last = st["blocks"][depth - 1]
        dx, dx16 = ops.layernorm_bwd(dy.contiguous(), st["x_last"], f.p("norm.weight"), st["mean"],
                                     st["rstd"], f.g("norm.weight"), f.g("norm.bias"),
                                     want_bf16=True, row_scale=last["dpm"],
                                     rows_per_sample=st["x_last"].shape[1])
        ready(0)
        hip.mark("bwd_norm")
        for blk in reversed(plan.blocks[lo:]):
            below = st["blocks"][blk.index - 1] if blk.index > lo else None
            try:
                G = self.RED_GROUP
                dx, dx16 = self._block_bwd(blk, st["blocks"][blk.index], dx, dx16, st["n_obj"], below,
                                           red_begin=blk.index % G == G - 1 or blk.index == depth - 1,
                                           red_end=blk.index % G == 0 or blk.index == lo, red_slot=blk.index % G)
            except BaseException:
                ops.reduce_reset()
                self._tn = []
                raise
            hip.mark("bwd%d" % blk.index)
            ready(1 + (depth - 1 - blk.index))
        if cut > 0:
            behind = []
            if self._tn and self.reproducible and not self.deterministic:
                for j in range(lo - 1, -1, -1):
                    behind += st["blocks"][j]["tn_shapes"]
                    if len(self._tn) + len(behind) > 8:
                        break
            self._flush_tn(behind=behind)
            self._join()
            for rank in range(1 + (depth - lo), depth + 2):
                ready(rank)
            return
        B, Tx, L, O, C = st["B"], st["Tx"], st["L0"], plan.objects, plan.embed_dim
        ops.special_token_grads(dx, f.g("cls_token"), f.g("object_queries"),
                                f.g("pos_embed_temporal") if Tx > 1 else None, L, Tx, O, Tx > 1)
        dtok = ops.scale_cast(dx, gather=(L, 1))
        self._gemm_tn(dtok, st["cols"], f.g("patch_embed.proj.weight").view(C, 441), f.g("patch_embed.proj.bias"))
        self._flush_tn()
        self._join()
        ready(depth + 1)

    def _rws(self, key):
        a, b = self._red_regions[key]
        o = self._red_slot * 18 * 1024 * 1024
        return self._red_ws[o + a:o + b]

    def _wgrad_ws(self, B, h, thw, n_obj, strides):
        key = (B, h, tuple(thw), n_obj, tuple(strides))
        need = self._wgrad_need.get(key)
        if need is None:
            need = self._wgrad_need[key] = ops.pool_conv_bwd_workspace(B, h, thw, n_obj, strides)
        ws = self._rws("wgrad")
        if need <= ws.numel():
            return ws
        big = self._wgrad_big.get(self._red_slot)
        if big is None or big.numel() < need:
            big = self._wgrad_big[self._red_slot] = torch.empty(need, device=self.dev, dtype=F32)
        return big

    def _fork(self, fn, keep):
        if not self.overlap_wgrad:
            fn()
            return
        if self._capture_fork is not None:
            self._capture_fork(fn)
            self._side_active = True
            return
        main = torch.cuda.current_stream(self.dev)
        if self._side is None:
            self._side = torch.cuda.Stream(device=self.dev)
        self._side.wait_stream(main)
        with torch.cuda.stream(self._side):
            fn()
        self._side_keep.append(keep)
        self._side_active = True

    def _join(self):
        if self._side_active and self._capture_join is not None:
            self._capture_join()
            self._side_active = False
            return
        if self._side_active:
            torch.cuda.current_stream(self.dev).wait_stream(self._side)
            self._side_keep.clear()
            self._side_active = False

    def _flush_tn(self, force=True, behind=()):
        if not force and len(self._tn) <= 8:
            return
        q, self._tn = self._tn, []
        if not q:
            return
        det = self.deterministic
        if self.reproducible and not det:
            if behind:
                self._fork(lambda: ops.gemm_tn_grouped_slab_lead(q, behind, tag="tn_slab_queue"), q)
            else:
                self._fork(lambda: ops.gemm_tn_grouped_slab(q, tag="tn_slab_queue"), q)
            return
        self._fork(lambda: ops.gemm_tn_grouped(q, ordered=det), q)

    def _gemm_tn(self, a, b, dw, dbias=None):
        if self.deterministic:
            ops.gemm_tn(a, b, dw, splits=1, dbias=dbias)
        elif self.reproducible:
            ops.gemm_tn_grouped_slab([(a, b, dw, dbias)], tag="tn_slab_main")
        else:
            ops.gemm_tn(a, b, dw, splits=0, dbias=dbias)

    def _linear_bwd(self, dy16, x16, wname, bname, need_dx, out=None, accumulate=False,
                    epilogue=hip.EPI_F32, aux=None):
        f = self.flat
        self._tn.append((dy16, x16, f.g(wname), f.g(bname)))
        if not need_dx:
            return None
        return ops.gemm_nt(dy16, f.wt(wname), None, epilogue, out=out, aux=aux, accumulate=accumulate)

    def _block_bwd(self, blk, sv, dx2, dy, n_obj, below, red_begin=True, red_end=True, red_slot=0):
        f = self.flat
        pre = "blocks.%d." % blk.index
        B, Nq, Co = dx2.shape
        x = sv["x"]
        N, C, h = x.shape[1], x.shape[2], blk.heads
        M, Mq = B * N, B * Nq
        sq, skv = blk.stride_q[1], blk.stride_kv[1]
        thw, q_thw, k_thw = sv["thw"], sv["q_thw"], sv["k_thw"]
        self._red_slot = red_slot
        if red_begin:
            ops.reduce_defer(True)
        dy = dy.view(Mq, Co)
        dh = self._linear_bwd(dy, sv["act"], pre + "mlp.fc2.weight", pre + "mlp.fc2.bias", True,
                              epilogue=hip.EPI_DGELU, aux=sv["dact"])
        dxn2 = self._linear_bwd(dh, sv["xn2"].view(Mq, Co), pre + "mlp.fc1.weight",
                                pre + "mlp.fc1.bias", True, epilogue=hip.EPI_BF16)
        dx1, dy = ops.layernorm_bwd(dxn2, sv["x1"], f.p(pre + "norm2.weight"), sv["mean2"],
                                    sv["rstd2"], f.g(pre + "norm2.weight"), f.g(pre + "norm2.bias"),
                                    dres=dx2, want_bf16=True, row_scale=sv["dpa"], rows_per_sample=Nq,
                                    ws=self._rws("ln2"))
        dy = dy.view(Mq, Co)
        dctx = self._linear_bwd(dy, sv["ctx"].view(Mq, Co), pre + "attn.proj.weight",
                                pre + "attn.proj.bias", True, epilogue=hip.EPI_BF16)
        (qa, preq, mq, rq), (ka, prek, mk, rk), (v, prev, mv, rv) = sv["pools"]
        tabs, mats = sv["tabs"], sv["mats"]
        names = (pre + "attn.rel_pos_h", pre + "attn.rel_pos_w", pre + "attn.rel_pos_t")
        if all(m is None for m in mats):
            rcat_t, lpad, offs = f.rel_cat_t(pre)
        else:
            offs, lpad = rel_sections([t.shape[0] for t in tabs])
            rcat = torch.zeros((lpad, HD), device=self.dev, dtype=F32)
            for o, t in zip(offs, tabs):
                rcat[o:o + t.shape[0]] = t
            rcat_t = rcat.t().contiguous().to(BF16)
        if self.fused_scatter:
            dmap = self._relq_map(blk, q_thw, k_thw, sv["idx"], offs, n_obj, qa.shape[-1] - HD)
            dqa, dk, dv, D, dq_extra = ops.attn_bwd(
                qa, ka, v, sv["ctx"], dctx.view(B, Nq, Co), sv["lse2"], SCALE,
                q_splits=1 if self.deterministic else self.attn_q_splits, bias_cols=sum(sv["k_thw"]),
                reld=(dmap, lpad, LOG2E, rcat_t if rcat_t.is_contiguous() else None, "fold"))
        else:
            dqa, dk, dv = ops.attn_bwd(qa, ka, v, sv["ctx"], dctx.view(B, Nq, Co), sv["lse2"], SCALE,
                                       q_splits=1 if self.deterministic else self.attn_q_splits,
                                       bias_cols=sum(sv["k_thw"]))
            D = ops.relpos_scatter(dqa, sv["idx"], offs, lpad, B, h, q_thw, k_thw, n_obj, LOG2E)
            dq_extra = None
        qa2 = qa.view(B * h * Nq, qa.shape[-1])
        for n, m, t, o in zip(names, mats, tabs, offs):
            rows = t.shape[0]
            if m is None:
                self._tn.append((D[:, o:o + rows], qa2[:, :HD], f.g(n), None))
            else:
                d = torch.zeros_like(t)
                self._gemm_tn(D[:, o:o + rows], qa2[:, :HD], d)
                f.g(n).add_(m.t() @ d)
        if dq_extra is None:
            dq_extra = ops.gemm_nt(D, rcat_t, None, hip.EPI_BF16)
        elif isinstance(dq_extra, str):
            dq_extra = None
        Nk = ka.shape[2]
        dqkv = torch.empty_like(sv["qkv"])
        entries = []
        for r, pre_t, mean, rstd, nout, kw in (
                ("q", preq, mq, rq, Nq, dict(d_main=dqa, ld_main=qa.shape[-1], d_res=dctx,
                                             d_extra=dq_extra)),
                ("k", prek, mk, rk, Nk, dict(d_main=dk, ld_main=HD)),
                ("v", prev, mv, rv, Nk, dict(d_main=dv, ld_main=HD))):
            entries.append(((pre_t, mean, rstd, f.p(pre + "attn.norm_%s.weight" % r),
                             f.g(pre + "attn.norm_%s.weight" % r),
                             f.g(pre + "attn.norm_%s.bias" % r), B, h, nout), kw))
        dpres = ops.pool_ln_bwd_qkv(entries, ws=self._rws("pln"))
        strides = (sq, skv, skv)
        ops.pool_conv_bwd_qkv(dpres, [f.p(pre + "attn.pool_%s.weight" % r).view(HD, 27) for r in "qkv"],
                              dqkv, sv["qkv"],
                              [f.g(pre + "attn.pool_%s.weight" % r).view(HD, 27) for r in "qkv"],
                              B, h, thw, n_obj, strides, ws=self._wgrad_ws(B, h, thw, n_obj, strides))
        dxn = self._linear_bwd(dqkv, sv["xn"], pre + "attn.qkv.weight", pre + "attn.qkv.bias", True,
                               epilogue=hip.EPI_F32 if blk.has_proj else hip.EPI_BF16)
        dskip = dx1
        if blk.pools_q:
            dskip = ops.maxpool_bwd(dskip, sv["pool_idx"], thw, n_obj, bf16=blk.has_proj)
        if blk.has_proj:
            ds16 = dskip.view(M, Co) if blk.pools_q else ops.scale_cast(dskip.view(M, Co))
            self._linear_bwd(ds16, sv["xn"], pre + "proj.weight", pre + "proj.bias", True, out=dxn,
                             accumulate=True)
            dskip = None
        res = ops.layernorm_bwd(dxn, x, f.p(pre + "norm1.weight"), sv["mean1"], sv["rstd1"],
                                f.g(pre + "norm1.weight"), f.g(pre + "norm1.bias"), dres=dskip,
                                want_bf16=below is not None,
                                row_scale=below["dpm"] if below is not None else None,
                                rows_per_sample=N, ws=self._rws("ln1"))
        if red_end:
            ops.reduce_defer(False)
        self._flush_tn(force=False)
        if below is None:
            return res.view(B, N, C), None
        return res[0].view(B, N, C), res[1]
```

### svit_amd/hip.py

```python
import ctypes as C
import os

import torch

_HERE = os.path.dirname(os.path.abspath(__file__))
LIB_PATH = os.environ.get("SVIT_HIP_LIB") or os.path.join(_HERE, "lib", "libsvit_hip.so")
_lib = None

vp, i32, i64, f32 = C.c_void_p, C.c_int32, C.c_int64, C.c_float

EPI_BF16, EPI_GELU, EPI_RESID, EPI_F32, EPI_DGELU, EPI_RELQ = 0, 1, 2, 3, 4, 5


class TnProblem(C.Structure):
    _fields_ = [("A", vp), ("B", vp), ("dW", vp), ("dbias", vp), ("lda", i32), ("ldb", i32),
                ("lddw", i32), ("M", i32), ("N", i32), ("K", i32)]


class GemmArgs(C.Structure):
    _fields_ = [("A", vp), ("lda", i32), ("W", vp), ("ldw", i32), ("bias", vp), ("out", vp),
                ("ldo", i32), ("out2", vp), ("ldo2", i32), ("aux", vp), ("ldaux", i32),
                ("row_scale", vp), ("rows_per_sample", i32), ("M", i32), ("N", i32), ("K", i32),
                ("epilogue", i32), ("accumulate", i32), ("remap_L", i32), ("remap_N", i32),
                ("remap_off", i32), ("relq_map", vp), ("relq_out", vp), ("relq_ld", i32),
                ("relq_extra", i32), ("relq_rows", i32), ("relq_scale", f32)]


class PoolArgs(C.Structure):
    _fields_ = [("qkv", vp), ("which", i32), ("conv_w", vp), ("gamma", vp), ("beta", vp),
                ("out", vp), ("ld_out", i32), ("pre", vp), ("mean", vp), ("rstd", vp),
                ("B", i32), ("heads", i32), ("T", i32), ("H", i32), ("W", i32), ("n_obj", i32),
                ("stride_hw", i32), ("mode", i32), ("eps", f32), ("out_scale", f32),
                ("relq_R", vp), ("relq_map", vp), ("relq_lpad", i32), ("relq_scale", f32)]


class PoolLnBwdArgs(C.Structure):
    _fields_ = [("d_main", vp), ("main_is_f32", i32), ("ld_main", i32), ("d_res", vp),
                ("d_extra", vp), ("pre", vp), ("mean", vp), ("rstd", vp), ("gamma", vp),
                ("dpre", vp), ("dgamma", vp), ("dbeta", vp), ("B", i32), ("heads", i32),
                ("Nout", i32), ("workspace", vp), ("workspace_floats", i64), ("main_parts", i32),
                ("main_part_stride", i64), ("extra_is_bf16", i32)]


class PoolDgradArgs(C.Structure):
    _fields_ = [("dpre", vp), ("conv_w", vp), ("dqkv", vp), ("which", i32), ("B", i32),
                ("heads", i32), ("T", i32), ("H", i32), ("W", i32), ("n_obj", i32),
                ("stride_hw", i32)]


class PoolWgradArgs(C.Structure):
    _fields_ = [("dpre", vp), ("qkv", vp), ("which", i32), ("dw", vp), ("B", i32), ("heads", i32),
                ("T", i32), ("H", i32), ("W", i32), ("n_obj", i32), ("stride_hw", i32),
                ("workspace", vp), ("workspace_floats", i64)]


class RelqArgs(C.Structure):
    _fields_ = [("qa", vp), ("ld", i32), ("rel_h", vp), ("rel_w", vp), ("rel_t", vp),
                ("idx_h", vp), ("idx_w", vp), ("idx_t", vp), ("B", i32), ("heads", i32),
                ("qt", i32), ("qh", i32), ("qw", i32), ("kt", i32), ("kh", i32), ("kw", i32),
                ("n_obj", i32), ("inv_scale", f32)]


class RelqBwdArgs(C.Structure):
    _fields_ = [("qa", vp), ("dqa", vp), ("ld", i32), ("rel_h", vp), ("rel_w", vp), ("rel_t", vp),
                ("idx_h", vp), ("idx_w", vp), ("idx_t", vp), ("dq_extra", vp), ("drel_h", vp),
                ("drel_w", vp), ("drel_t", vp), ("rows_h", i32), ("rows_w", i32), ("rows_t", i32),
                ("B", i32), ("heads", i32), ("qt", i32), ("qh", i32), ("qw", i32), ("kt", i32),
                ("kh", i32), ("kw", i32), ("n_obj", i32), ("inv_scale", f32),
                ("workspace", vp), ("workspace_floats", i64)]


class RelqGatherArgs(C.Structure):
    _fields_ = [("P", vp), ("ldp", i32), ("qa", vp), ("ld", i32), ("idx_h", vp), ("idx_w", vp),
                ("idx_t", vp), ("row_h", i32), ("row_w", i32), ("row_t", i32), ("B", i32),
                ("heads", i32), ("qt", i32), ("qh", i32), ("qw", i32), ("kt", i32), ("kh", i32),
                ("kw", i32), ("n_obj", i32), ("inv_scale", f32)]


class RelqScatterArgs(C.Structure):
    _fields_ = [("dqa", vp), ("ld", i32), ("D", vp), ("ldd", i32), ("idx_h", vp), ("idx_w", vp),
                ("idx_t", vp), ("off_h", i32), ("off_w", i32), ("off_t", i32), ("B", i32),
                ("heads", i32), ("qt", i32), ("qh", i32), ("qw", i32), ("kt", i32), ("kh", i32),
                ("kw", i32), ("n_obj", i32), ("inv_scale", f32)]


class AttnFwdArgs(C.Structure):
    _fields_ = [("qa", vp), ("ka", vp), ("v", vp), ("ctx", vp), ("lse2", vp), ("B", i32),
                ("heads", i32), ("Nq", i32), ("Nk", i32), ("DA", i32), ("scale", f32),
                ("bias_cols", i32)]


class AttnBwdArgs(C.Structure):
    _fields_ = [("qa", vp), ("ka", vp), ("v", vp), ("ctx", vp), ("dctx", vp), ("lse2", vp),
                ("delta", vp), ("dqa", vp), ("dk", vp), ("dv", vp), ("B", i32), ("heads", i32),
                ("Nq", i32), ("Nk", i32), ("DA", i32), ("q_splits", i32), ("scale", f32),
                ("bias_cols", i32), ("relD", vp), ("relD_ld", i32), ("relD_map", vp), ("relD_scale", f32),
                ("relR", vp), ("relX", vp)]


class HeadArgs(C.Structure):
    _fields_ = [("tokens", vp), ("B", i32), ("N", i32), ("C", i32), ("T", i32), ("O", i32), ("keep", vp),
                ("w_proj", vp), ("b_proj", vp), ("n_cls", i32), ("w_box", vp), ("b_box", vp),
                ("w_bce", vp), ("b_bce", vp), ("w_con", vp), ("b_con", vp),
                ("logits", vp), ("boxes", vp), ("contact", vp), ("xobj", vp)]


class HeadBwdArgs(C.Structure):
    _fields_ = [("f", HeadArgs), ("dlogits", vp), ("dboxes", vp), ("dcontact", vp), ("dxobj", vp), ("dtokens", vp),
                ("gw_proj", vp), ("gb_proj", vp), ("gw_box", vp), ("gb_box", vp), ("gw_bce", vp), ("gb_bce", vp),
                ("gw_con", vp), ("gb_con", vp), ("ordered", i32)]


class FeedSeg(C.Structure):
    _fields_ = [("src_off", i64), ("dst", vp), ("bytes", i64)]


class FeedArgs(C.Structure):
    _fields_ = [("slot", vp), ("slot_bytes", i64), ("offsets", vp), ("extents", vp), ("frames", vp),
                ("V", i32), ("T", i32), ("Hs", i32), ("Ws", i32), ("fill", i32), ("swap_rb", i32), ("n_seg", i32),
                ("seg", FeedSeg * 8)]


class ActSite(C.Structure):
    _fields_ = [("a", vp), ("b", vp), ("rows", i32), ("first_window", i32)]


class StepHost(C.Structure):
    _fields_ = [("lr", f32 * 2), ("weight_decay", f32 * 2), ("max_norm", f32), ("clip_value", f32),
                ("grad_scale", f32), ("reserved", f32)]


class StepDev(C.Structure):
    _fields_ = [("applied", i64), ("skipped", i64), ("consecutive", i32), ("apply", i32), ("coef", f32),
                ("bc1", f32), ("bc2_sqrt", f32), ("sumsq", f32), ("grad_norm", f32), ("reserved", f32)]


_SIGS = {
    "svit_version": (i32, []),
    "svit_arch": (C.c_char_p, []),
    "svit_gemm_nt": (i32, [C.POINTER(GemmArgs), vp]),
    "svit_gemm_tn": (i32, [vp, i32, vp, i32, vp, i32, i32, i32, i32, i32, vp, vp]),
    "svit_gemm_tn_grouped": (i32, [C.POINTER(TnProblem), i32, vp]),
    "svit_gemm_tn_grouped_ex": (i32, [C.POINTER(TnProblem), i32, i32, vp]),
    "svit_gemm_tn_grouped_slab": (i32, [C.POINTER(TnProblem), i32, vp, i64, vp]),
    "svit_gemm_tn_grouped_workspace": (i64, [C.POINTER(TnProblem), i32]),
    "svit_gemm_tn_grouped_slab_lead": (i32, [C.POINTER(TnProblem), i32, i32, vp, i64, vp]),
    "svit_colsum_bf16": (i32, [vp, i32, vp, i32, i32, vp]),
    "svit_cast_f32_bf16": (i32, [vp, vp, i64, vp]),
    "svit_table_interp": (i32, [vp, i32, i32, vp, vp, vp, vp]),
    "svit_table_interp_batched": (i32, [vp, i32, i32, vp]),
    "svit_transpose_cast_batched": (i32, [vp, vp, vp, i32, i32, vp]),
    "svit_transpose_bf16_batched": (i32, [vp, vp, vp, i32, i32, vp]),
    "svit_scale_cast": (i32, [vp, vp, vp, i32, i64, i32, i32, i32, i32, vp]),
    "svit_pad_cast_rows": (i32, [vp, vp, i32, i32, i32, vp]),
    "svit_reduce_defer": (i32, [i32, vp]),
    "svit_reduce_flush": (i32, [vp]),
    "svit_reduce_reset": (i32, [vp]),
    "svit_layernorm_fwd": (i32, [vp, vp, vp, vp, vp, vp, vp, i64, i32, f32, vp]),
    "svit_layernorm_bwd": (i32, [vp, i32, vp, vp, vp, vp, vp, vp, vp, vp, i32, vp, vp, i64, i32, vp,
                                 i64, vp]),
    "svit_im2col_patch": (i32, [vp, vp, i32, i32, i32, i32, vp]),
    "svit_im2col_patch_u8": (i32, [vp, i64, vp, vp, vp, i32, i32, i32, i32, i32, vp]),
    "svit_im2col_patch_u8_mix": (i32, [vp, i64, vp, vp, vp, vp, i32, i32, i32, i32, i32, vp]),
    "svit_im2col_patch_u8_aug": (i32, [vp, i64, vp, vp, vp, vp, i32, i32, i32, i32, i32, vp]),
    "svit_im2col_patch_u8_aug_frames": (i32, [vp, i64, vp, vp, vp, vp, i32, i32, i32, i32, i32, vp]),
    "svit_u8_clips_render": (i32, [vp, i64, vp, vp, vp, i32, i32, i32, i32, i32, vp]),
    "svit_im2col_patch_u8_aug_ext": (i32, [vp, i64, vp, vp, vp, vp, vp, i32, i32, i32, i32, i32, vp]),
    "svit_im2col_patch_u8_aug_frames_ext": (i32, [vp, i64, vp, vp, vp, vp, vp, i32, i32, i32, i32, i32, vp]),
    "svit_u8_clips_render_ext": (i32, [vp, i64, vp, vp, vp, vp, i32, i32, i32, i32, i32, vp]),
    "svit_mixup_clips": (i32, [vp, vp, i32, i32, i32, i32, vp]),
    "svit_randaug_stats": (i32, [vp, vp, i32, vp, i32, i32, i32, i32, i32, vp]),
    "svit_randaug_apply": (i32, [vp, vp, vp, i32, vp, i32, i32, i32, i32, i32, vp]),
    "svit_randaug_stats_ext": (i32, [vp, vp, vp, i32, vp, i32, i32, i32, i32, i32, vp]),
    "svit_randaug_apply_ext": (i32, [vp, vp, vp, vp, i32, vp, i32, i32, i32, i32, i32, vp]),
    "svit_feed_unpack": (i32, [C.POINTER(FeedArgs), vp]),
    "svit_fill_special_tokens": (i32, [vp, vp, vp, vp, i32, i32, i32, i32, i32, i32, i32, vp]),
    "svit_special_token_grads": (i32, [vp, vp, vp, vp, i32, i32, i32, i32, i32, i32, i32, vp]),
    "svit_pool_ln_fwd": (i32, [C.POINTER(PoolArgs), vp]),
    "svit_pool_ln_bwd": (i32, [C.POINTER(PoolLnBwdArgs), vp]),
    "svit_pool_ln_fwd_qkv": (i32, [C.POINTER(PoolArgs), vp]),
    "svit_pool_ln_fwd_qkv_sel": (i32, [C.POINTER(PoolArgs), C.POINTER(vp), vp]),
    "svit_pool_weight_sel": (i32, [vp, vp, vp, i32, vp]),
    "svit_pool_ln_bwd_qkv": (i32, [C.POINTER(PoolLnBwdArgs), vp]),
    "svit_pool_conv_bwd_qkv": (i32, [C.POINTER(PoolDgradArgs), C.POINTER(PoolWgradArgs), vp]),
    "svit_pool_conv_bwd_workspace": (i64, [C.POINTER(PoolDgradArgs)]),
    "svit_relpos_q_fwd": (i32, [C.POINTER(RelqArgs), vp]),
    "svit_relpos_q_bwd": (i32, [C.POINTER(RelqBwdArgs), vp]),
    "svit_relpos_scatter": (i32, [C.POINTER(RelqScatterArgs), vp]),
    "svit_relpos_gather": (i32, [C.POINTER(RelqGatherArgs), vp]),
    "svit_attn_fwd": (i32, [C.POINTER(AttnFwdArgs), vp]),
    "svit_attn_bwd": (i32, [C.POINTER(AttnBwdArgs), vp]),
    "svit_attn_bwd_parts": (i32, [C.POINTER(AttnBwdArgs)]),
    "svit_maxpool_fwd": (i32, [vp, vp, vp, i32, i32, i32, i32, i32, i32, vp]),
    "svit_maxpool_bwd": (i32, [vp, vp, vp, i32, i32, i32, i32, i32, i32, vp]),
    "svit_maxpool_bwd_bf16": (i32, [vp, vp, vp, i32, i32, i32, i32, i32, i32, vp]),
    "svit_sumsq": (i32, [vp, i64, vp, vp, i64, vp]),
    "svit_adamw_step": (i32, [vp, vp, vp, vp, i64, vp, f32, f32, f32, f32, f32, f32, i32, f32, vp]),
    "svit_adamw_bias_table": (i32, [f32, f32, vp, i64, C.POINTER(i64)]),
    "svit_step_guard": (i32, [vp, i64, vp, vp, vp, i64, vp, i64, vp]),
    "svit_adamw_step_guarded": (i32, [vp, vp, vp, vp, i64, i64, vp, vp, f32, f32, f32, vp]),
    "svit_step_guard_seg": (i32, [vp, i64, vp, i64, vp, vp, vp, i64, vp, i64, vp]),
    "svit_adamw_step_guarded_seg": (i32, [vp, vp, vp, vp, i64, i64, vp, i64, vp, vp, f32, f32, f32, vp]),
    "svit_adamw_step_guarded_lr": (i32, [vp, vp, vp, vp, i64, i64, vp, vp, i64, vp, vp, f32, f32, f32, vp]),
    "svit_sgd_step_guarded": (i32, [vp, vp, vp, i64, i64, vp, vp, i64, vp, vp, f32, f32, i32, vp]),
    "svit_adam_step_guarded": (i32, [vp, vp, vp, vp, i64, i64, vp, vp, i64, vp, vp, f32, f32, f32, vp]),
    "svit_ema_decay_table": (i32, [f32, vp, i64, C.POINTER(i64)]),
    "svit_ema_step_guarded": (i32, [vp, vp, i64, vp, i64, vp, i64, f32, vp, vp, vp]),
    "svit_tensor_stats_window": (i32, []),
    "svit_tensor_table_check": (i32, [vp, i64, i64]),
    "svit_tensor_stats_workspace": (i64, [i64, i64]),
    "svit_tensor_stats": (i32, [vp, vp, i64, vp, vp, i64, vp, i64, vp, vp, i64, i64, vp, i64, vp]),
    "svit_act_stats_window": (i32, []),
    "svit_act_stats_workspace": (i64, [i64]),
    "svit_act_sites_check": (i32, [C.POINTER(ActSite), vp, i64, i64, C.POINTER(i64)]),
    "svit_act_stats": (i32, [C.POINTER(ActSite), vp, i64, i64, vp, vp, vp, i64, vp, vp, i64, vp]),
    "svit_head_fwd": (i32, [C.POINTER(HeadArgs), vp]),
    "svit_head_bwd": (i32, [C.POINTER(HeadBwdArgs), vp]),
    "svit_head_eval": (i32, [C.POINTER(HeadArgs), i32, vp]),
    "svit_haog_loss": (i32, [vp, vp, vp, vp, vp, vp, vp, vp, vp, i32, i32, vp]),
    "svit_haog_loss_bwd": (i32, [vp, vp, vp, vp, vp, vp, vp, i32, i32, vp]),
    "svit_ce_loss": (i32, [vp, vp, i32, i32, vp, vp, vp]),
    "svit_ce_loss_soft": (i32, [vp, vp, vp, vp, f32, f32, i32, i32, vp, vp, vp]),
    "svit_step_draws": (i32, [vp, vp, i32, i32, vp, i32, C.c_float, vp, vp]),
    "svit_ensemble_update": (i32, [vp, vp, vp, i32, i32, i32, i32, i32, i32, vp, vp, vp, vp, vp]),
    "svit_topk_correct": (i32, [vp, vp, i32, i32, vp, i32, vp, vp, vp]),
    "svit_meter_push": (i32, [vp, i32, i32, vp, vp, i32, vp, vp, i32, i32, i32, i32, vp]),
    "svit_debug_set": (i32, [i32, i32]),
    "svit_debug_set_tn": (i32, [i32, i32]),
    "svit_debug_set_tn_tile": (i32, [i32]),
    "svit_debug_set_pool": (i32, [i32, i32]),
    "svit_attn_debug_set": (i32, [i32, i32]),
    "svit_debug_reset": (i32, []),
    "svit_debug_pool_bwd_path": (i32, []),
    "svit_debug_pool_plan": (i32, [i32] * 13 + [C.POINTER(C.c_int32), i32]),
    "svit_debug_gemm_nt_plan": (i32, [i32] * 4 + [C.POINTER(C.c_int32), i32]),
    "svit_debug_gemm_tn_plan": (i32, [C.POINTER(TnProblem), i32, i32, i32, C.POINTER(i64), i32]),
}
EXPORTS = tuple(sorted(_SIGS))


class SvitHipError(RuntimeError):
    pass


def load():
    global _lib
    if _lib is None:
        if not os.path.exists(LIB_PATH):
            raise SvitHipError(
                "libsvit_hip.so not found at %s -- run `python -m svit_amd.build` "
                "(the SViT HIP path has no PyTorch/CPU fallback)" % LIB_PATH)
        if os.environ.get("SVIT_HIP_LIB"):
            import warnings
            warnings.warn("SVIT_HIP_LIB is set: loading the SViT HIP library from %s instead of the "
                          "in-tree build" % LIB_PATH)
        lib = C.CDLL(LIB_PATH)
        for name, (res, args) in _SIGS.items():
            fn = getattr(lib, name)
            fn.restype, fn.argtypes = res, args
        _lib = lib
    return _lib


_raw_stream = torch._C._cuda_getCurrentRawStream
_cur_device = torch._C._cuda_getDevice


def stream():
    return C.c_void_p(_raw_stream(_cur_device()))


def ptr(t):
    if t is None:
        return None
    return t.data_ptr()


def check(rc, what):
    if rc != 0:
        kind = {-2: "bad shape", -3: "bad alignment/stride", -4: "bad argument"}.get(
            rc, "hipError_t %d" % rc)
        raise SvitHipError("%s failed: %s" % (what, kind))


_trace = None


def start_trace():
    global _trace
    _trace = []


def stop_trace():
    global _trace
    t, _trace = _trace, None
    return t


def mark(label):
    if _trace is not None:
        e = torch.cuda.Event(enable_timing=True)
        e.record()
        _trace.append(("mark:" + label, e, e, None))


def call(name, *args, meta=None):
    if _trace is None:
        rc = getattr(load(), name)(*args, stream())
        check(rc, name)
        return
    e0 = torch.cuda.Event(enable_timing=True)
    e1 = torch.cuda.Event(enable_timing=True)
    e0.record()
    rc = getattr(load(), name)(*args, stream())
    e1.record()
    check(rc, name)
    _trace.append((name, e0, e1, meta))
```

### svit_amd/ops.py

```python
import ctypes as C

import torch

from . import hip
from .hip import ptr

BF16 = torch.bfloat16
F32 = torch.float32
HD = 96
_scratch = {}


def scratch(device, floats=8 * 1024 * 1024, tag="main"):
    key = (device.index, floats, tag)
    buf = _scratch.get(key)
    if buf is None:
        buf = torch.empty(floats, device=device, dtype=F32)
        _scratch[key] = buf
    return buf


def _chk_rows(*ts):
    for t in ts:
        if not t.is_cuda or t.dim() != 2 or t.stride(1) != 1:
            raise hip.SvitHipError("svit_amd GEMM operands must be 2-D device tensors with unit inner stride")


def _chk_dev(*ts):
    for t in ts:
        if t is not None and not t.is_cuda:
            raise hip.SvitHipError("svit_amd ops need device tensors (got %s)" % t.device)
        if t is not None and not t.is_contiguous():
            raise hip.SvitHipError("svit_amd ops need contiguous tensors")


def gemm_nt(a, w, bias=None, epilogue=hip.EPI_BF16, out=None, out2=None, aux=None,
            row_scale=None, rows_per_sample=0, accumulate=False, remap=None, save=True, relq=None):
    _chk_rows(a)
    _chk_dev(w, bias, out, out2, aux, row_scale)
    M, K = a.shape
    N = w.shape[0]
    assert w.shape[1] == K and a.dtype == BF16 and w.dtype == BF16
    if epilogue == hip.EPI_RELQ:
        cmap, qa, scale = relq
        _chk_dev(cmap, qa)
        extra = qa.shape[-1] - 96
        assert cmap.dtype == torch.int32 and cmap.is_contiguous() and cmap.shape == (qa.shape[-2], extra)
        assert qa.is_contiguous() and qa.numel() == M * qa.shape[-1] and bias is None
        g = hip.GemmArgs()
        g.A, g.lda, g.W, g.ldw = ptr(a), a.stride(0), ptr(w), w.stride(0)
        g.M, g.N, g.K, g.epilogue = M, N, K, epilogue
        g.relq_map, g.relq_out, g.relq_ld = ptr(cmap), ptr(qa), qa.shape[-1]
        g.relq_extra, g.relq_rows, g.relq_scale = extra, qa.shape[-2], scale
        hip.call("svit_gemm_nt", C.byref(g), meta=("mnk", M, N, K, epilogue, 2 * M * K + 2 * N * K + 2 * M * extra))
        return qa
    if out is None:
        dt = F32 if epilogue in (hip.EPI_RESID, hip.EPI_F32) else BF16
        out = torch.empty((M, N), device=a.device, dtype=dt)
    if epilogue == hip.EPI_GELU and out2 is None and save:
        out2 = torch.empty((M, N), device=a.device, dtype=BF16)
    g = hip.GemmArgs()
    g.A, g.lda, g.W, g.ldw = ptr(a), a.stride(0), ptr(w), w.stride(0)
    g.bias = ptr(bias)
    g.out, g.ldo = ptr(out), out.stride(-2)
    g.out2, g.ldo2 = ptr(out2), (out2.stride(-2) if out2 is not None else 0)
    g.aux, g.ldaux = ptr(aux), (aux.stride(-2) if aux is not None else 0)
    g.row_scale, g.rows_per_sample = ptr(row_scale), rows_per_sample
    g.M, g.N, g.K = M, N, K
    g.epilogue, g.accumulate = epilogue, int(accumulate)
    if remap is not None:
        g.remap_L, g.remap_N, g.remap_off = remap
    osz = out.element_size()
    nbytes = 2 * M * K + 2 * N * K + M * N * osz
    if out2 is not None:
        nbytes += 2 * M * N
    if aux is not None:
        nbytes += M * N * aux.element_size()
    if accumulate:
        nbytes += M * N * osz
    hip.call("svit_gemm_nt", C.byref(g), meta=("mnk", M, N, K, epilogue, nbytes))
    return (out, out2) if epilogue == hip.EPI_GELU else out


NT_FAMILIES = ("v2", "ring")
NT_RULES = ("forced", "ring_few_long_tiles", "ring_long_k_narrow", "bk64_narrow_long_k", "one_round_160x256",
            "one_round_192x192", "square_128x128", "big_128x192", "default_128x96")
_NT_PLAN_FIELDS = ("RB", "NB", "WM", "WN", "NL", "stages", "BK", "gx", "gy", "block", "lds")


def gemm_nt_plan(M, N, K, epilogue=hip.EPI_BF16):
    out = (C.c_int32 * 13)()
    n = hip.load().svit_debug_gemm_nt_plan(M, N, K, epilogue, out, 13)
    hip.check(min(n, 0), "svit_debug_gemm_nt_plan")
    plan = dict(zip(_NT_PLAN_FIELDS, out[1:12]))
    plan.update(family=NT_FAMILIES[out[0]], rule=NT_RULES[out[12]])
    return plan


def gemm_tn(a, b, dw, splits=0, dbias=None):
    _chk_rows(a, b)
    _chk_dev(dw)
    M, N = a.shape
    K = dw.shape[-1]
    assert b.shape[0] == M and b.shape[1] >= K and dw.shape[-2] == N and dw.dtype == F32
    hip.call("svit_gemm_tn", ptr(a), a.stride(0), ptr(b), b.stride(0), ptr(dw), dw.stride(-2),
             M, N, K, splits, ptr(dbias), meta=("mnk", M, N, K))
    return dw


def _tn_problem_array(problems):
    arr = (hip.TnProblem * len(problems))()
    flop = 0.0
    for t, (a, b, dw, dbias) in zip(arr, problems):
        _chk_rows(a, b, dw)
        _chk_dev(dbias)
        M, N = a.shape
        K = dw.shape[1]
        assert b.shape[0] == M and b.shape[1] >= K and dw.shape[0] == N and dw.dtype == F32
        t.A, t.B, t.dW, t.dbias = ptr(a), ptr(b), ptr(dw), ptr(dbias)
        t.lda, t.ldb, t.lddw, t.M, t.N, t.K = a.stride(0), b.stride(0), dw.stride(0), M, N, K
        flop += 2.0 * M * N * K
    return arr, flop


def gemm_tn_grouped(problems, ordered=False):
    if not problems:
        return
    arr, flop = _tn_problem_array(problems)
    if ordered:
        hip.call("svit_gemm_tn_grouped_ex", arr, len(problems), 1, meta=("flop", flop))
    else:
        hip.call("svit_gemm_tn_grouped", arr, len(problems), meta=("flop", flop))


TN_FORMS = ("atomic", "ordered", "slab", "single")
_TN_PLAN_FIELDS = ("tile_kind", "tiles_n", "tiles_k", "rows_per_split", "splits", "first_block", "w", "tile_off", "bias_off",
                   "red_first")


def gemm_tn_plan(problems, form="atomic", splits=0):
    form = TN_FORMS.index(form) if isinstance(form, str) else form
    n = len(problems)
    if n and isinstance(problems[0][0], int):
        arr = (hip.TnProblem * n)()
        for t, (M, N, K, has_bias) in zip(arr, problems):
            t.A, t.B, t.dW, t.dbias = 1 << 20, 2 << 20, 3 << 20, (4 << 20) if has_bias else None
            t.lda, t.ldb, t.lddw, t.M, t.N, t.K = -(-N // 8) * 8, -(-K // 8) * 8, K, M, N, K
    else:
        arr = _tn_problem_array(problems)[0]
    size = 2 + 3 * (n // 16 + 1) + 10 * n
    out = (C.c_int64 * size)()
    got = hip.load().svit_debug_gemm_tn_plan(arr, n, form, splits, out, size)
    hip.check(min(got, 0), "svit_debug_gemm_tn_plan")
    vals, groups = iter(out[2:got]), []
    for _ in range(out[0]):
        count, grid, reduce_grid = next(vals), next(vals), next(vals)
        groups.append(dict(grid=grid, reduce_grid=reduce_grid,
                           problems=[dict(zip(_TN_PLAN_FIELDS, vals)) for _ in range(count)]))
    return dict(form=TN_FORMS[form], workspace_floats=out[1], groups=groups)


_tn_slab_need = {}
_tn_slab_ws = {}


def gemm_tn_slab_workspace(arr, n, fresh=False):
    key = tuple((t.M, t.N, t.K, t.dbias is not None) for t in arr)
    need = None if fresh else _tn_slab_need.get(key)
    if need is None:
        need = hip.load().svit_gemm_tn_grouped_workspace(arr, n)
        if need < 0:
            hip.check(need, "svit_gemm_tn_grouped_workspace")
        _tn_slab_need[key] = need
    return need


def _tn_slab_buffer(dev, tag, need):
    key = (dev.index, tag)
    ws = _tn_slab_ws.get(key)
    if ws is None or ws.numel() < need:
        if ws is not None:
            torch.cuda.synchronize(dev)
        ws = _tn_slab_ws[key] = torch.empty(max(need, 1), device=dev, dtype=F32)
    return ws


def gemm_tn_grouped_slab(problems, ws=None, tag="tn_slab"):
    n = len(problems)
    if n == 0:
        return
    arr, flop = _tn_problem_array(problems)
    if ws is not None:
        _chk_dev(ws)
        assert ws.dtype == F32
        hip.call("svit_gemm_tn_grouped_slab", arr, n, ptr(ws), ws.numel(), meta=("flop", flop))
        return
    dev = problems[0][2].device
    ws = _tn_slab_buffer(dev, tag, gemm_tn_slab_workspace(arr, n))
    try:
        hip.call("svit_gemm_tn_grouped_slab", arr, n, ptr(ws), ws.numel(), meta=("flop", flop))
    except hip.SvitHipError:
        need = gemm_tn_slab_workspace(arr, n, fresh=True)
        if need <= ws.numel():
            raise
        ws = _tn_slab_buffer(dev, tag, need)
        hip.call("svit_gemm_tn_grouped_slab", arr, n, ptr(ws), ws.numel(), meta=("flop", flop))


def gemm_tn_grouped_slab_lead(problems, shapes_behind, tag="tn_slab"):
    n, m = len(problems), len(shapes_behind)
    if m == 0:
        return gemm_tn_grouped_slab(problems, tag=tag)
    real, flop = _tn_problem_array(problems)
    arr = (hip.TnProblem * (n + m))()
    for i in range(n):
        arr[i] = real[i]
    for j, (M, N, K, has_bias) in enumerate(shapes_behind):
        t = arr[n + j]
        t.A, t.B, t.dW, t.dbias = 1 << 20, 2 << 20, 3 << 20, (4 << 20) if has_bias else None
        t.lda, t.ldb, t.lddw, t.M, t.N, t.K = -(-N // 8) * 8, -(-K // 8) * 8, K, M, N, K
    ws = _tn_slab_buffer(problems[0][2].device, tag, gemm_tn_slab_workspace(arr, n + m))
    hip.call("svit_gemm_tn_grouped_slab_lead", arr, n + m, n, ptr(ws), ws.numel(), meta=("flop", flop))


def reduce_defer(on):
    hip.call("svit_reduce_defer", int(on))


def reduce_flush():
    hip.call("svit_reduce_flush")


def reduce_reset():
    hip.call("svit_reduce_reset")


def colsum(a, out):
    _chk_dev(a, out)
    hip.call("svit_colsum_bf16", ptr(a), a.stride(0), ptr(out), a.shape[0], a.shape[1])
    return out


def cast_bf16(src, dst=None):
    _chk_dev(src, dst)
    if dst is None:
        dst = torch.empty(src.shape, device=src.device, dtype=BF16)
    hip.call("svit_cast_f32_bf16", ptr(src), ptr(dst), src.numel())
    return dst


def transpose_cast_batched(src_flat, dst_flat, table, n_mats, max_tiles):
    hip.call("svit_transpose_cast_batched", ptr(src_flat), ptr(dst_flat), ptr(table), n_mats,
             max_tiles)


def transpose_bf16_batched(src16_flat, dst_flat, table, n_mats, max_tiles):
    _chk_dev(src16_flat, dst_flat, table)
    assert src16_flat.dtype == BF16 and dst_flat.dtype == BF16
    hip.call("svit_transpose_bf16_batched", ptr(src16_flat), ptr(dst_flat), ptr(table), n_mats,
             max_tiles)


def table_interp(mcat, tables, want_f32=True):
    _chk_dev(mcat, tables)
    assert mcat.dtype == F32 and tables.dtype == F32 and mcat.is_contiguous() and tables.is_contiguous()
    assert mcat.shape[1] == tables.shape[0] and tables.shape[1] == HD
    r32 = torch.empty((mcat.shape[0], HD), device=mcat.device, dtype=F32) if want_f32 else None
    r16 = torch.empty((mcat.shape[0], HD), device=mcat.device, dtype=BF16)
    hip.call("svit_table_interp", ptr(mcat), mcat.shape[0], mcat.shape[1], ptr(tables), ptr(r32), ptr(r16))
    return r32, r16


def table_interp_jobs(entries, device):
    import struct
    raw = b"".join(struct.pack("<QQQQii", ptr(m), ptr(t), ptr(o32) or 0, ptr(o16) or 0, m.shape[0], m.shape[1])
                   for m, t, o32, o16 in entries)
    return torch.frombuffer(bytearray(raw), dtype=torch.uint8).view(len(entries), 40).to(device)


def table_interp_batched(jobs, max_rows):
    hip.call("svit_table_interp_batched", ptr(jobs), jobs.shape[0], max_rows)


def pad_cast_rows(src, dst):
    _chk_dev(src, dst)
    hip.call("svit_pad_cast_rows", ptr(src), ptr(dst), src.shape[0], src.shape[1], dst.shape[1])
    return dst


def scale_cast(src, row_scale=None, rows_per_sample=0, dst=None, gather=None):
    _chk_dev(src, row_scale, dst)
    cols = src.shape[-1]
    if gather is None:
        rows, gl, gn, go = src.shape[:-1].numel(), 0, 0, 0
        shape = src.shape
    else:
        gl, go = gather
        gn = src.shape[-2]
        rows = src.shape[0] * gl
        shape = (rows, cols)
    if dst is None:
        dst = torch.empty(shape, device=src.device, dtype=BF16)
    hip.call("svit_scale_cast", ptr(src), ptr(dst), ptr(row_scale), rows_per_sample, rows, cols,
             gl, gn, go)
    return dst


def layernorm_fwd(x, gamma, beta, eps=1e-6, want_f32=False, want_bf16=True, save_stats=True):
    _chk_dev(x, gamma, beta)
    C_ = x.shape[-1]
    rows = x.numel() // C_
    y16 = torch.empty(x.shape, device=x.device, dtype=BF16) if want_bf16 else None
    y32 = torch.empty(x.shape, device=x.device, dtype=F32) if want_f32 else None
    mean = torch.empty(rows, device=x.device, dtype=F32) if save_stats else None
    rstd = torch.empty(rows, device=x.device, dtype=F32) if save_stats else None
    hip.call("svit_layernorm_fwd", ptr(x), ptr(gamma), ptr(beta), ptr(y16), ptr(y32), ptr(mean),
             ptr(rstd), rows, C_, eps)
    return y16, y32, mean, rstd


def layernorm_bwd(dy, x, gamma, mean, rstd, dgamma, dbeta, dres=None, dx=None, want_bf16=False,
                  row_scale=None, rows_per_sample=0, ws=None):
    _chk_dev(dy, x, gamma, mean, rstd, dgamma, dbeta, dres, dx, row_scale)
    C_ = x.shape[-1]
    rows = x.numel() // C_
    if dx is None:
        dx = torch.empty(x.shape, device=x.device, dtype=F32)
    dx16 = torch.empty(x.shape, device=x.device, dtype=BF16) if want_bf16 else None
    ws = scratch(x.device) if ws is None else ws
    assert dy.dtype in (F32, BF16)
    hip.call("svit_layernorm_bwd", ptr(dy), int(dy.dtype == BF16), ptr(x), ptr(gamma), ptr(mean),
             ptr(rstd), ptr(dres),
             ptr(dx), ptr(dx16), ptr(row_scale), rows_per_sample, ptr(dgamma), ptr(dbeta), rows, C_,
             ptr(ws), ws.numel())
    return (dx, dx16) if want_bf16 else dx


def im2col_patch(video):
    _chk_dev(video)
    B, Cin, T, H, W = video.shape
    assert Cin == 3 and video.dtype == F32
    To, Ho, Wo = (T - 1) // 2 + 1, (H - 1) // 4 + 1, (W - 1) // 4 + 1
    cols = torch.empty((B * To * Ho * Wo, 448), device=video.device, dtype=BF16)
    hip.call("svit_im2col_patch", ptr(video), ptr(cols), B, T, H, W)
    return cols, (To, Ho, Wo)


def _chk_extents(extents, fr):
    if extents is None:
        return "", ()
    if (extents.dtype != torch.int32 or tuple(extents.shape) != (fr.shape[0], 2) or not extents.is_contiguous()
            or extents.device != fr.device):
        raise hip.SvitHipError("the extents must be contiguous int32 [%d,2] on %s (got %s %s on %s)"
                               % (fr.shape[0], fr.device, extents.dtype, tuple(extents.shape), extents.device))
    return "_ext", (ptr(extents),)


def _im2col_u8(name, fr, lut, table, S, mix=(), frames_pass=False, extents=None):
    _chk_dev(fr)
    V, T, Hs, Ws, _ = fr.shape
    B = table.shape[0]
    n, To = (B * T, 1) if frames_pass else (B, (T - 1) // 2 + 1)
    Ho = Wo = (S - 1) // 4 + 1
    cols = torch.empty((n * To * Ho * Wo, 448), device=fr.device, dtype=BF16)
    for m in mix:
        if m is not None:
            _chk_mix(m, fr.device)
    suffix, ext = _chk_extents(extents, fr)
    hip.call(name + suffix, ptr(fr), fr.numel(), ptr(lut), ptr(table), *ext, *[ptr(m) for m in mix], ptr(cols),
             B, T, Hs, Ws, S)
    return cols, (To, Ho, Wo)


def im2col_patch_u8(clips):
    mix = getattr(clips, "mix", None)
    if mix is not None:
        return _im2col_u8("svit_im2col_patch_u8_mix", clips.frames, clips.lut_f32, clips.crops, clips.size, (mix,))
    return _im2col_u8("svit_im2col_patch_u8", clips.frames, clips.lut, clips.crops, clips.size)


def _chk_aug(fr, rec, lut):
    _chk_dev(fr, rec, lut)
    if rec.dtype != torch.int32 or rec.dim() != 2 or rec.shape[1] != 16 or not rec.is_contiguous() or rec.device != fr.device:
        raise hip.SvitHipError("the augmentation records must be contiguous int32 [B,16] on %s (got %s %s on %s)"
                               % (fr.device, rec.dtype, tuple(rec.shape), rec.device))
    if lut.dtype != F32 or lut.numel() != 768 or lut.device != fr.device:
        raise hip.SvitHipError("the normalisation table must be f32 [3,256] on %s" % (fr.device,))


def im2col_patch_u8_aug(clips):
    _chk_aug(clips.frames, clips.records, clips.lut_f32)
    clips.run_randaug()
    return _im2col_u8("svit_im2col_patch_u8_aug", clips.frames, clips.lut_f32, clips.records, clips.size,
                      (getattr(clips, "mix", None),), extents=clips.extents)


def im2col_patch_u8_aug_frames(view):
    clips = view.clips
    if not view.fresh and hasattr(clips, "run_randaug"):
        clips.run_randaug()
    fr, rec, lut = view.frames, view.device_records(), view.lut_f32
    _chk_aug(fr, rec, lut)
    return _im2col_u8("svit_im2col_patch_u8_aug_frames", fr, lut, rec, view.size, (view.mix,), frames_pass=True,
                      extents=view.extents)


def u8_clips_render(clips):
    _chk_aug(clips.frames, clips.records, clips.lut_f32)
    clips.run_randaug()
    fr = clips.frames
    V, T, Hs, Ws, _ = fr.shape
    B, S = clips.records.shape[0], clips.size
    out = torch.empty((B, 3, T, S, S), device=fr.device, dtype=F32)
    suffix, ext = _chk_extents(clips.extents, fr)
    hip.call("svit_u8_clips_render" + suffix, ptr(fr), fr.numel(), ptr(clips.lut_f32), ptr(clips.records), *ext,
             ptr(out), B, T, Hs, Ws, S)
    return out


def feed_args(slot, frames, offsets=None, extents=None, fill=0, swap_rb=False, segments=(), slot_bytes=None):
    _chk_dev(slot, frames, offsets, extents)
    if slot.dtype != torch.uint8 or frames.dtype != torch.uint8 or frames.dim() != 5 or frames.shape[-1] != 3:
        raise hip.SvitHipError("feed_unpack takes a uint8 slot and uint8 [V,T,Hs,Ws,3] frames, got %s and %s %s"
                               % (slot.dtype, frames.dtype, tuple(frames.shape)))
    V, T, Hs, Ws, _ = frames.shape
    if offsets is not None and (offsets.dtype != torch.int64 or tuple(offsets.shape) != (V,) or offsets.device != frames.device):
        raise hip.SvitHipError("the offsets must be int64 [%d] on %s" % (V, frames.device))
    if extents is not None:
        _chk_extents(extents, frames)
    a = hip.FeedArgs()
    a.slot, a.slot_bytes = ptr(slot), slot.numel() if slot_bytes is None else int(slot_bytes)
    if a.slot_bytes > slot.numel():
        raise hip.SvitHipError("slot_bytes %d exceeds the slot tensor's %d bytes" % (a.slot_bytes, slot.numel()))
    a.offsets, a.extents, a.frames = ptr(offsets), ptr(extents), ptr(frames)
    a.V, a.T, a.Hs, a.Ws, a.fill, a.swap_rb = V, T, Hs, Ws, int(fill), int(bool(swap_rb))
    if len(segments) > 8:
        raise hip.SvitHipError("feed_unpack carries at most 8 segments, got %d" % len(segments))
    a.n_seg = len(segments)
    for s, sg in enumerate(segments):
        dst = sg[1]
        _chk_dev(dst)
        if dst.device != frames.device:
            raise hip.SvitHipError("segment %d lives on %s, the frames on %s" % (s, dst.device, frames.device))
        full = dst.numel() * dst.element_size()
        nbytes = full if len(sg) < 3 else int(sg[2])
        if nbytes > full:
            raise hip.SvitHipError("segment %d: %d bytes into a tensor of %d" % (s, nbytes, full))
        a.seg[s].src_off, a.seg[s].dst, a.seg[s].bytes = int(sg[0]), ptr(dst), nbytes
    return a

# ... 672 lines not shown
```

Baseline: 697.1 clips/s.

## Skip drop-path-dead sample rows in grouped weight-gradient GEMMs

Passes the per-sample drop-path scale into the grouped TN weight-gradient GEMM so K-steps (M-row blocks) belonging to samples whose scale is zero are not loaded or multiplied. These rows have zero gradient anyway, so they contribute nothing to dW. The pipelined loop is reworked to walk only live steps, with adjusted waitcnt and tail-zeroing logic. It also adds an XCD-aware block-to-tile remap, off by default, and debug hooks for it. The skip is data-dependent and only saves work when stochastic depth actually drops samples; it adds per-block bitmask overhead and risks load imbalance across blocks.

```diff
diff --git a/include/svit_hip.h b/include/svit_hip.h
--- a/include/svit_hip.h
+++ b/include/svit_hip.h
@@ -42,6 +42,8 @@
 typedef struct {
   const void* A; const void* B; float* dW; float* dbias;
   int32_t lda, ldb, lddw, M, N, K;
+  const float* row_scale;
+  int32_t rows_per_sample;
 } svit_tn_problem;
 int svit_gemm_tn_grouped(const svit_tn_problem* probs, int count, void* stream);
 int svit_gemm_tn_grouped_ex(const svit_tn_problem* probs, int count, int ordered, void* stream);
@@ -366,6 +368,8 @@
 int svit_debug_set_tn(int step_us_x100, int atomic_tbs_x100);
 int svit_debug_set_tn_tile(int mode);
 int svit_debug_gemm_tn_plan(const svit_tn_problem* probs, int count, int form, int arg, int64_t* out, int n_out);
+int svit_debug_set_tn_skip(int key, int val);
+int svit_debug_gemm_tn_map(const svit_tn_problem* probs, int count, int form, int32_t* out, int n_out);
 int svit_debug_set_pool(int key, int val);
 int svit_debug_pool_bwd_path(void);
 int svit_debug_pool_plan(int kind, int B, int heads, int T, int H, int W, int n_obj, int sq, int sk, int sv, int save_mask,
diff --git a/svit_amd/csrc/common.h b/svit_amd/csrc/common.h
--- a/svit_amd/csrc/common.h
+++ b/svit_amd/csrc/common.h
@@ -42,6 +42,8 @@
   SVIT_K_ATTN_DKV_FORM,
   SVIT_K_ATTN_FWD_SHORT,
   SVIT_K_POOL_FRAME,
+  SVIT_K_TN_SKIP,
+  SVIT_K_TN_MAP,
   SVIT_K_COUNT
 };
 int svit_knob(int k);
diff --git a/svit_amd/csrc/gemm_tn.hip b/svit_amd/csrc/gemm_tn.hip
--- a/svit_amd/csrc/gemm_tn.hip
+++ b/svit_amd/csrc/gemm_tn.hip
@@ -42,17 +42,49 @@
   asm volatile("ds_read_b64_tr_b16 %0, %1 offset:%2" : "=&v"(d) : "v"(addr), "i"(OFF) : "memory");
 }
 
-template <class C, bool SLAB>
+template <class C, bool SLAB, bool SKIP = false>
 __device__ __forceinline__ void tn_tile_dma(unsigned char* lds, const bf16_t* __restrict__ A, int lda,
                                             const bf16_t* __restrict__ B, int ldb,
                                             float* __restrict__ dW, int lddw, int M, int N, int K, int n0,
                                             int k0, int m_begin, int m_end,
-                                            float* __restrict__ dbias, bool bias_tile) {
+                                            float* __restrict__ dbias, bool bias_tile,
+                                            const float* __restrict__ row_scale = nullptr, int rps = 1) {
 #if __HIP_DEVICE_COMPILE__
   constexpr int RB = C::RB, BM = C::BM, NS = C::NS, PER = C::PER;
   const int tid = threadIdx.x, lane = tid & 63, wave = __builtin_amdgcn_readfirstlane(tid >> 6);
   const int wn = wave / C::WK, wk = wave % C::WK;
   if (m_begin >= m_end) return;
+  const int nsteps = (m_end - m_begin + BM - 1) / BM;
+  unsigned long long dead = 0;
+  int walk_s = 0, walk_end = 0;
+  if constexpr (SKIP) {
+    const int s0 = m_begin / rps, ns = min(64, (m_end - 1) / rps - s0 + 1);
+    for (int i = 0; i < ns; ++i)
+      if (row_scale[s0 + i] == 0.f) dead |= 1ull << i;
+    walk_end = (s0 + 1) * rps;
+  }
+  auto next_live = [&](int t) {
+    if constexpr (SKIP) {
+      while (t < nsteps) {
+        const int r0 = m_begin + t * BM, r1 = min(r0 + BM, m_end) - 1;
+        while (r0 >= walk_end) ++walk_s, walk_end += rps;
+        int s = walk_s, e = walk_end;
+        bool run = s < 64 && ((dead >> s) & 1);
+        while (run && e <= r1) {
+          ++s, e += rps;
+          run = s < 64 && ((dead >> s) & 1);
+        }
+        if (!run) return t;
+        t = max(t + 1, (e - m_begin) / BM);
+      }
+      return nsteps;
+    } else {
+      return t;
+    }
+  };
+  int t_next = next_live(0);
+  if constexpr (SKIP && !SLAB)
+    if (t_next >= nsteps) return;
   constexpr int NW = C::NW, NT = C::NT;
   constexpr int PA = C::A_INSTR / NW;
   static_assert(C::A_INSTR % NW == 0 && C::B_INSTR % NW == 0, "pieces split evenly over the waves");
@@ -72,10 +104,11 @@
   }
   const auto ars = __builtin_amdgcn_make_buffer_rsrc((void*)A, 0, (int)std::min<size_t>((size_t)M * lda * 2, 0x7fffffffu), 0x00020000);
   const auto brs = __builtin_amdgcn_make_buffer_rsrc((void*)B, 0, (int)std::min<size_t>((size_t)M * ldb * 2, 0x7fffffffu), 0x00020000);
-  const int nsteps = (m_end - m_begin + BM - 1) / BM;
-  auto issue = [&](int s) {
-    unsigned char* st = lds + (s % NS) * C::STAGE;
-    const int m0 = m_begin + s * BM;
+  int issued = 0;
+  bool has_tail = false;
+  auto issue = [&]() {
+    unsigned char* st = lds + (issued % NS) * C::STAGE;
+    const int m0 = m_begin + t_next * BM;
     const int valid = m_end - m0;
 #pragma unroll
     for (int i = 0; i < PER; ++i) {
@@ -93,10 +126,13 @@
         __builtin_amdgcn_raw_ptr_buffer_load_lds(brs, (__attribute__((address_space(3))) void*)dst, 16, vo,
                                                  (unsigned)m0 * ldb * 2u, 0, 0);
     }
+    has_tail |= t_next == nsteps - 1;
+    ++issued;
+    t_next = next_live(t_next + 1);
   };
 #pragma unroll
   for (int s = 0; s < NS - 1; ++s)
-    if (s < nsteps) issue(s);
+    if (t_next < nsteps) issue();
 
   f32x16_t acc[RB][3];
 #pragma unroll
@@ -122,14 +158,14 @@
     b_addr[j] = lds0 + C::A_BYTES + (8 * hh + q) * C::ROWB + (((col >> 5) ^ C::swz_b(q)) << 6) + (col & 31) * 2;
   }
   constexpr int KS = BM / 16;
-  for (int s = 0; s < nsteps; ++s) {
-    if (s + NS - 2 < nsteps - 0 && NS > 2 && s + 1 < nsteps) asm volatile("s_waitcnt vmcnt(%0)" ::"n"((NS - 2) * PER) : "memory");
+  for (int s = 0; s < issued; ++s) {
+    if (NS > 2 && issued == s + NS - 1) asm volatile("s_waitcnt vmcnt(%0)" ::"n"((NS - 2) * PER) : "memory");
     else asm volatile("s_waitcnt vmcnt(0)" ::: "memory");
     __builtin_amdgcn_s_barrier();
-    if (s + NS - 1 < nsteps) issue(s + NS - 1);
+    if (t_next < nsteps) issue();
     const unsigned so = (unsigned)((s % NS) * C::STAGE);
-    if (m_begin + (s + 1) * BM > m_end) {
-      const int valid = m_end - (m_begin + s * BM);
+    if (s + 1 == issued && has_tail && ((m_end - m_begin) & (BM - 1))) {
+      const int valid = (m_end - m_begin) & (BM - 1);
       for (int c = tid; c < (BM - valid) * (C::ROWA / 16); c += NT)
         *(uint4*)(lds + so + valid * C::ROWA + c * 16) = make_uint4(0, 0, 0, 0);
       __syncthreads();
@@ -253,7 +289,34 @@
   int rows_per_split[SVIT_TN_GROUP_MAX];
   int big[SVIT_TN_GROUP_MAX];
   int count;
+  int map_count;
+  int map_row_first[9];
+  int map_pre[8][SVIT_TN_GROUP_MAX];
+  int map_cls[8];
+  int map_start[8];
+  int map_rot[SVIT_TN_GROUP_MAX];
 };
+
+__host__ __device__ __forceinline__ int tn_block_to_logical(const TnGroup& g, int nwg, int lin) {
+  const int xq = nwg >> 3, xr = nwg & 7, xcd = lin & 7;
+  const int v = (xcd < xr ? xcd * (xq + 1) : xr * (xq + 1) + (xcd - xr) * xq) + (lin >> 3);
+  const int n = g.map_count;
+  if (n == 0) return v;
+  int r = 0;
+#pragma unroll
+  for (int i = 1; i < 8; ++i)
+    if (v >= g.map_row_first[i]) r = i;
+  int k = v - g.map_row_first[r], j = 0;
+#pragma unroll
+  for (int i = 1; i < SVIT_TN_GROUP_MAX; ++i)
+    if (i < n && k >= g.map_pre[r][i]) j = i;
+  k -= g.map_pre[r][j];
+  int pi = j + g.map_start[r];
+  if (pi >= n) pi -= n;
+  const int tiles = g.tiles[pi];
+  const int split = ((g.map_cls[r] - g.map_rot[pi]) & 7) + 8 * (k / tiles);
+  return g.first_block[pi] + split * tiles + k % tiles;
+}
 
 struct TnSlabs {
   long long tile_off[SVIT_TN_GROUP_MAX];
@@ -266,10 +329,8 @@
 
 template <bool SLAB>
 __device__ __forceinline__ void tn_grouped_workgroup(unsigned char* lds, const TnGroup& g, const TnSlabs* sl, float* ws) {
-  const int nwg = gridDim.x, lin = blockIdx.x;
-  const int xq = nwg >> 3, xr = nwg & 7, xcd = lin & 7;
   int pi = 0;
-  const int bid = (xcd < xr ? xcd * (xq + 1) : xr * (xq + 1) + (xcd - xr) * xq) + (lin >> 3);
+  const int bid = tn_block_to_logical(g, gridDim.x, blockIdx.x);
 #pragma unroll
   for (int i = 1; i < SVIT_TN_GROUP_MAX; ++i)
     if (i < g.count && bid >= g.first_block[i]) pi = i;
@@ -287,14 +348,20 @@
   } else {
     out = p.dW, ld = p.lddw, bias = p.dbias;
   }
-  if (g.big[pi])
-    tn_tile_dma<TnBigD, SLAB>(lds, (const bf16_t*)p.A, p.lda, (const bf16_t*)p.B, p.ldb, out, ld, p.M, p.N, p.K,
-                              tn * TnBigD::TN, tk * TnBigD::TK, m_begin, min(p.M, m_begin + g.rows_per_split[pi]),
-                              bias, tk == 0);
-  else
-    tn_tile_dma<TnSmallD, SLAB>(lds, (const bf16_t*)p.A, p.lda, (const bf16_t*)p.B, p.ldb, out, ld, p.M, p.N, p.K,
-                                tn * TnSmallD::TN, tk * TnSmallD::TK, m_begin, min(p.M, m_begin + g.rows_per_split[pi]),
-                                bias, tk == 0);
+  auto body = [&](auto C_, auto SKIP_) {
+    using C = decltype(C_);
+    tn_tile_dma<C, SLAB, decltype(SKIP_)::value>(lds, (const bf16_t*)p.A, p.lda, (const bf16_t*)p.B, p.ldb, out, ld, p.M, p.N,
+                                                 p.K, tn * C::TN, tk * C::TK, m_begin,
+                                                 min(p.M, m_begin + g.rows_per_split[pi]), bias, tk == 0, p.row_scale,
+                                                 p.rows_per_sample);
+  };
+  if (g.big[pi]) {
+    if (p.row_scale) body(TnBigD{}, std::true_type{});
+    else body(TnBigD{}, std::false_type{});
+  } else {
+    if (p.row_scale) body(TnSmallD{}, std::true_type{});
+    else body(TnSmallD{}, std::false_type{});
+  }
 }
 
 #ifndef SVIT_TN_WPE
@@ -418,6 +485,7 @@
   for (int i = 0; i < count; ++i) {
     const int rc = tn_check(probs[i]);
     if (rc) return rc;
+    if (probs[i].row_scale && probs[i].rows_per_sample <= 0) return SVIT_ERR_ARG;
   }
   return SVIT_OK;
 }
@@ -490,11 +558,80 @@
   return best_steps;
 }
 
+static void tn_map_build(TnGroup& g, int n, int grid) {
+  g.map_count = 0;
+  if (!svit_knob(SVIT_K_TN_MAP) || n <= 0 || grid < 8) return;
+  int S[SVIT_TN_GROUP_MAX];
+  long size[8] = {0, 0, 0, 0, 0, 0, 0, 0};
+  auto units = [&](int i, int rot, int c) {
+    const int s0 = (c - rot) & 7;
+    return s0 < S[i] ? (S[i] - s0 + 7) / 8 : 0;
+  };
+  for (int i = 0; i < n; ++i) {
+    S[i] = (g.first_block[i + 1] - g.first_block[i]) / g.tiles[i];
+    double best = 1e300;
+    for (int rot = 0; rot < 8; ++rot) {
+      double sq = 0.0;
+      for (int c = 0; c < 8; ++c) {
+        const double v = (double)(size[c] + (long)g.tiles[i] * units(i, rot, c));
+        sq += v * v;
+      }
+      if (sq < best) best = sq, g.map_rot[i] = rot;
+    }
+    for (int c = 0; c < 8; ++c) size[c] += (long)g.tiles[i] * units(i, g.map_rot[i], c);
+  }
+  bool used[8] = {false, false, false, false, false, false, false, false};
+  long d = 0, d_end[8];
+  for (int r = 0; r < 8; ++r) {
+    const long len = grid / 8 + (r < grid % 8 ? 1 : 0);
+    int pick = -1, largest = -1;
+    for (int c = 0; c < 8; ++c) {
+      if (used[c]) continue;
+      if (largest < 0 || size[c] > size[largest]) largest = c;
+      if (d + size[c] - len >= 0 && (pick < 0 || size[c] < size[pick])) pick = c;
+    }
+    if (pick < 0) pick = largest;
+    used[pick] = true;
+    g.map_cls[r] = pick;
+    d += size[pick] - len;
+    d_end[r] = d;
+  }
+  for (int r = 0; r < 8; ++r) {
+    const int want = (r * n / 8 + n - 1) % n;
+    int last = -1, fattest = -1, best_dist = 0;
+    for (int i = 0; i < n; ++i) {
+      if (!units(i, g.map_rot[i], g.map_cls[r])) continue;
+      if (fattest < 0 || g.tiles[i] > g.tiles[fattest]) fattest = i;
+      const int dist = std::min((i - want + n) % n, (want - i + n) % n);
+      if (g.tiles[i] > d_end[r] && (last < 0 || dist < best_dist)) last = i, best_dist = dist;
+    }
+    if (last < 0) last = fattest < 0 ? n - 1 : fattest;
+    g.map_start[r] = (last + 1) % n;
+  }
+  int pos = 0;
+  for (int r = 0; r < 8; ++r) {
+    g.map_row_first[r] = pos;
+    int acc = 0;
+    for (int j = 0; j < SVIT_TN_GROUP_MAX; ++j) {
+      g.map_pre[r][j] = acc;
+      if (j < n) {
+        const int pi = (j + g.map_start[r]) % n;
+        acc += g.tiles[pi] * units(pi, g.map_rot[pi], g.map_cls[r]);
+      }
+    }
+    pos += acc;
+  }
+  g.map_row_first[8] = pos;
+  g.map_count = n;
+}
+
 static int tn_plan(const svit_tn_problem* probs, int n, int ordered, TnGroup& g) {
   const int mode = svit_knob(SVIT_K_TN_TILE);
+  const bool skip = svit_knob(SVIT_K_TN_SKIP) != 0;
   g.count = n;
   for (int i = 0; i < n; ++i) {
     g.p[i] = probs[i];
+    if (!skip) g.p[i].row_scale = nullptr;
     g.big[i] = tn_tile_rule(probs[i], mode);
     const TnTileDims t = tn_dims(g.big[i]);
     g.tiles_n[i] = tn_ceil(probs[i].N, t.tn);
@@ -509,6 +646,7 @@
     total += g.tiles[i] * tn_ceil(g.p[i].M, g.rows_per_split[i]);
   }
   for (int i = n; i <= SVIT_TN_GROUP_MAX; ++i) g.first_block[i] = total;
+  tn_map_build(g, n, total);
   return total;
 }
 
@@ -603,9 +741,10 @@
   if (!workspace || workspace_floats < tn_slab_need(chunks)) return SVIT_ERR_ARG;
   if ((uintptr_t)workspace & 15) return SVIT_ERR_ALIGN;
   for (size_t i = 0; i < chunks.size(); ++i) {
-    const TnChunk& c = chunks[i];
+    TnChunk& c = chunks[i];
     const int lead = std::min(launch_count - (int)i * SVIT_TN_GROUP_MAX, c.g.count);
     if (lead <= 0) break;
+    if (lead < c.g.count) tn_map_build(c.g, lead, c.g.first_block[lead]);
     hipLaunchKernelGGL(gemm_tn_grouped_slab_kernel, dim3(c.g.first_block[lead]), dim3(256), 0, (hipStream_t)stream, c.g,
                        c.sl, workspace);
     SVIT_LAUNCH_CHECK();
@@ -649,6 +788,22 @@
   return (int)(o - out);
 }
 
+extern "C" int svit_debug_gemm_tn_map(const svit_tn_problem* probs, int count, int form, int32_t* out, int n_out) {
+  if (form < 0 || form > 2 || !out) return SVIT_ERR_ARG;
+  std::vector<TnChunk> chunks;
+  const int rc = tn_chunks(probs, count, form == 1, form == 2, chunks);
+  if (rc) return rc;
+  long n = 0;
+  for (const TnChunk& c : chunks) n += 1 + c.grid;
+  if (n_out < n) return SVIT_ERR_ARG;
+  int32_t* o = out;
+  for (const TnChunk& c : chunks) {
+    *o++ = c.grid;
+    for (int b = 0; b < c.grid; ++b) *o++ = tn_block_to_logical(c.g, c.grid, b);
+  }
+  return (int)(o - out);
+}
+
 extern "C" int svit_colsum_bf16(const void* A, int lda, float* out, int M, int N, void* stream) {
   if (!A || !out || M <= 0 || N <= 0 || (N & 1) || (lda & 1)) return SVIT_ERR_ARG;
   const int col_groups = (N + 127) / 128;
diff --git a/svit_amd/csrc/misc.hip b/svit_amd/csrc/misc.hip
--- a/svit_amd/csrc/misc.hip
+++ b/svit_amd/csrc/misc.hip
@@ -709,8 +709,9 @@
 
 static const int k_knob_default[SVIT_K_COUNT] = {
      0,  -1,  0,  85,  75,  2,
-     2,  1,  1,  0,  1,  2};
-static int g_knob[SVIT_K_COUNT] = {0, -1, 0, 85, 75, 2, 2, 1, 1, 0, 1, 2};
+     2,  1,  1,  0,  1,  2,
+     1,  0};
+static int g_knob[SVIT_K_COUNT] = {0, -1, 0, 85, 75, 2, 2, 1, 1, 0, 1, 2, 1, 0};
 int svit_knob(int k) { return __atomic_load_n(&g_knob[k], __ATOMIC_RELAXED); }
 int svit_knob_set(int k, int v) {
   if (k < 0 || k >= SVIT_K_COUNT) return SVIT_ERR_ARG;
@@ -733,6 +734,11 @@
 }
 extern "C" int svit_debug_set_tn_tile(int mode) {
   return (mode >= 0 && mode <= 3) ? svit_knob_set(SVIT_K_TN_TILE, mode) : SVIT_ERR_ARG;
+}
+extern "C" int svit_debug_set_tn_skip(int key, int val) {
+  if (key == 0) return (val == 0 || val == 1) ? svit_knob_set(SVIT_K_TN_SKIP, val) : SVIT_ERR_ARG;
+  if (key == 1) return (val == 0 || val == 1) ? svit_knob_set(SVIT_K_TN_MAP, val) : SVIT_ERR_ARG;
+  return SVIT_ERR_ARG;
 }
 extern "C" int svit_debug_set_pool(int key, int val) {
   if (key == 0) return (val >= 0 && val <= 3) ? svit_knob_set(SVIT_K_POOL_FWD, val) : SVIT_ERR_ARG;
diff --git a/svit_amd/engine.py b/svit_amd/engine.py
--- a/svit_amd/engine.py
+++ b/svit_amd/engine.py
@@ -523,10 +523,14 @@
         else:
             ops.gemm_tn(a, b, dw, splits=0, dbias=dbias)
 
+    @staticmethod
+    def _dead(scale, rows_per_sample):
+        return None if scale is None else (scale, rows_per_sample)
+
     def _linear_bwd(self, dy16, x16, wname, bname, need_dx, out=None, accumulate=False,
-                    epilogue=hip.EPI_F32, aux=None):
+                    epilogue=hip.EPI_F32, aux=None, dead=None):
         f = self.flat
-        self._tn.append((dy16, x16, f.g(wname), f.g(bname)))
+        self._tn.append((dy16, x16, f.g(wname), f.g(bname), dead))
         if not need_dx:
             return None
         return ops.gemm_nt(dy16, f.wt(wname), None, epilogue, out=out, aux=aux, accumulate=accumulate)
@@ -544,17 +548,18 @@
         if red_begin:
             ops.reduce_defer(True)
         dy = dy.view(Mq, Co)
+        dead_m, dead_a = self._dead(sv["dpm"], Nq), self._dead(sv["dpa"], Nq)
         dh = self._linear_bwd(dy, sv["act"], pre + "mlp.fc2.weight", pre + "mlp.fc2.bias", True,
-                              epilogue=hip.EPI_DGELU, aux=sv["dact"])
+                              epilogue=hip.EPI_DGELU, aux=sv["dact"], dead=dead_m)
         dxn2 = self._linear_bwd(dh, sv["xn2"].view(Mq, Co), pre + "mlp.fc1.weight",
-                                pre + "mlp.fc1.bias", True, epilogue=hip.EPI_BF16)
+                                pre + "mlp.fc1.bias", True, epilogue=hip.EPI_BF16, dead=dead_m)
         dx1, dy = ops.layernorm_bwd(dxn2, sv["x1"], f.p(pre + "norm2.weight"), sv["mean2"],
                                     sv["rstd2"], f.g(pre + "norm2.weight"), f.g(pre + "norm2.bias"),
                                     dres=dx2, want_bf16=True, row_scale=sv["dpa"], rows_per_sample=Nq,
                                     ws=self._rws("ln2"))
         dy = dy.view(Mq, Co)
         dctx = self._linear_bwd(dy, sv["ctx"].view(Mq, Co), pre + "attn.proj.weight",
-                                pre + "attn.proj.bias", True, epilogue=hip.EPI_BF16)
+                                pre + "attn.proj.bias", True, epilogue=hip.EPI_BF16, dead=dead_a)
         (qa, preq, mq, rq), (ka, prek, mk, rk), (v, prev, mv, rv) = sv["pools"]
         tabs, mats = sv["tabs"], sv["mats"]
         names = (pre + "attn.rel_pos_h", pre + "attn.rel_pos_w", pre + "attn.rel_pos_t")
@@ -582,7 +587,7 @@
         for n, m, t, o in zip(names, mats, tabs, offs):
             rows = t.shape[0]
             if m is None:
-                self._tn.append((D[:, o:o + rows], qa2[:, :HD], f.g(n), None))
+                self._tn.append((D[:, o:o + rows], qa2[:, :HD], f.g(n), None, self._dead(sv["dpa"], h * Nq)))
             else:
                 d = torch.zeros_like(t)
                 self._gemm_tn(D[:, o:o + rows], qa2[:, :HD], d)
@@ -609,7 +614,7 @@
                               [f.g(pre + "attn.pool_%s.weight" % r).view(HD, 27) for r in "qkv"],
                               B, h, thw, n_obj, strides, ws=self._wgrad_ws(B, h, thw, n_obj, strides))
         dxn = self._linear_bwd(dqkv, sv["xn"], pre + "attn.qkv.weight", pre + "attn.qkv.bias", True,
-                               epilogue=hip.EPI_F32 if blk.has_proj else hip.EPI_BF16)
+                               epilogue=hip.EPI_F32 if blk.has_proj else hip.EPI_BF16, dead=self._dead(sv["dpa"], N))
         dskip = dx1
         if blk.pools_q:
             dskip = ops.maxpool_bwd(dskip, sv["pool_idx"], thw, n_obj, bf16=blk.has_proj)
diff --git a/svit_amd/hip.py b/svit_amd/hip.py
--- a/svit_amd/hip.py
+++ b/svit_amd/hip.py
@@ -14,7 +14,7 @@
 
 class TnProblem(C.Structure):
     _fields_ = [("A", vp), ("B", vp), ("dW", vp), ("dbias", vp), ("lda", i32), ("ldb", i32),
-                ("lddw", i32), ("M", i32), ("N", i32), ("K", i32)]
+                ("lddw", i32), ("M", i32), ("N", i32), ("K", i32), ("row_scale", vp), ("rows_per_sample", i32)]
 
 
 class GemmArgs(C.Structure):
@@ -228,6 +228,7 @@
     "svit_debug_set": (i32, [i32, i32]),
     "svit_debug_set_tn": (i32, [i32, i32]),
     "svit_debug_set_tn_tile": (i32, [i32]),
+    "svit_debug_set_tn_skip": (i32, [i32, i32]),
     "svit_debug_set_pool": (i32, [i32, i32]),
     "svit_attn_debug_set": (i32, [i32, i32]),
     "svit_debug_reset": (i32, []),
@@ -235,6 +236,7 @@
     "svit_debug_pool_plan": (i32, [i32] * 13 + [C.POINTER(C.c_int32), i32]),
     "svit_debug_gemm_nt_plan": (i32, [i32] * 4 + [C.POINTER(C.c_int32), i32]),
     "svit_debug_gemm_tn_plan": (i32, [C.POINTER(TnProblem), i32, i32, i32, C.POINTER(i64), i32]),
+    "svit_debug_gemm_tn_map": (i32, [C.POINTER(TnProblem), i32, i32, C.POINTER(C.c_int32), i32]),
 }
 EXPORTS = tuple(sorted(_SIGS))
 
diff --git a/svit_amd/ops.py b/svit_amd/ops.py
--- a/svit_amd/ops.py
+++ b/svit_amd/ops.py
@@ -111,9 +111,14 @@
 def _tn_problem_array(problems):
     arr = (hip.TnProblem * len(problems))()
     flop = 0.0
-    for t, (a, b, dw, dbias) in zip(arr, problems):
+    for t, (a, b, dw, dbias, *dead) in zip(arr, problems):
         _chk_rows(a, b, dw)
         _chk_dev(dbias)
+        if dead and dead[0] is not None:
+            scale, rps = dead[0]
+            _chk_dev(scale)
+            assert scale.dtype == F32 and scale.is_contiguous() and rps > 0 and scale.numel() * rps >= a.shape[0]
+            t.row_scale, t.rows_per_sample = ptr(scale), rps
         M, N = a.shape
         K = dw.shape[1]
         assert b.shape[0] == M and b.shape[1] >= K and dw.shape[0] == N and dw.dtype == F32
@@ -133,6 +138,31 @@
         hip.call("svit_gemm_tn_grouped", arr, len(problems), meta=("flop", flop))
 
 
+def gemm_tn_map(problems, form="atomic"):
+    plan = gemm_tn_plan(problems, form=form)
+    form = TN_FORMS.index(form) if isinstance(form, str) else form
+    arr = _tn_shape_array(problems) if isinstance(problems[0][0], int) else _tn_problem_array(problems)[0]
+    size = sum(1 + g["grid"] for g in plan["groups"])
+    out = (C.c_int32 * size)()
+    got = hip.load().svit_debug_gemm_tn_map(arr, len(problems), form, out, size)
+    hip.check(min(got, 0), "svit_debug_gemm_tn_map")
+    assert got == size
+    maps, o = [], 0
+    for g in plan["groups"]:
+        assert out[o] == g["grid"]
+        maps.append(list(out[o + 1:o + 1 + g["grid"]]))
+        o += 1 + g["grid"]
+    return maps
+
+
+def _tn_shape_array(shapes):
+    arr = (hip.TnProblem * len(shapes))()
+    for t, (M, N, K, has_bias) in zip(arr, shapes):
+        t.A, t.B, t.dW, t.dbias = 1 << 20, 2 << 20, 3 << 20, (4 << 20) if has_bias else None
+        t.lda, t.ldb, t.lddw, t.M, t.N, t.K = -(-N // 8) * 8, -(-K // 8) * 8, K, M, N, K
+    return arr
+
+
 TN_FORMS = ("atomic", "ordered", "slab", "single")
 _TN_PLAN_FIELDS = ("tile_kind", "tiles_n", "tiles_k", "rows_per_split", "splits", "first_block", "w", "tile_off", "bias_off",
                    "red_first")
@@ -142,10 +172,7 @@
     form = TN_FORMS.index(form) if isinstance(form, str) else form
     n = len(problems)
     if n and isinstance(problems[0][0], int):
-        arr = (hip.TnProblem * n)()
-        for t, (M, N, K, has_bias) in zip(arr, problems):
-            t.A, t.B, t.dW, t.dbias = 1 << 20, 2 << 20, 3 << 20, (4 << 20) if has_bias else None
-            t.lda, t.ldb, t.lddw, t.M, t.N, t.K = -(-N // 8) * 8, -(-K // 8) * 8, K, M, N, K
+        arr = _tn_shape_array(problems)
     else:
         arr = _tn_problem_array(problems)[0]
     size = 2 + 3 * (n // 16 + 1) + 10 * n
```

New measurement: 701.4 clips/s, median of 6. About the same (+0.6%).
